# vpc-ccg/tksm

Hardware: AMD Instinct MI355X
Metric: sequenced reads/s (higher is better)
Workload: dtype u8; 1 GPU; Bulk molecules, Badread error+qual model (nanopore2020, identity 84,99,5.5), 24 x 128 Mb random genome, FASTQ; kind=bulk, mean_len=1000, length_distribution=normal(1000, 200), compute_qual=True, contexts_in_flight_per_gpu=3

## Files before the change

### tksm_amd/csrc/api.cpp

```cpp
#include "../../include/tksmseq.h"

#include <hip/hip_runtime.h>

#include <algorithm>
#include <cstdio>
#include <cstring>
#include <cstdlib>
#include <memory>
#include <string>

#include "ctx.h"
#include "loop_filter.h"

static thread_local std::string g_create_error;
void set_contextless_error(const std::string& e) { g_create_error = e; }


template <class T>
static int upload(tksmseq_ctx* ctx, DevBuf& b, const std::vector<T>& v) {
    HIPCHK(ctx, b.ensure(v.size() * sizeof(T) + 16));
    if (!v.empty()) HIPCHK(ctx, hipMemcpyAsync(b.p, v.data(), v.size() * sizeof(T), hipMemcpyHostToDevice, ctx->stream));
    HIPCHK(ctx, hipStreamSynchronize(ctx->stream));
    return TKSMSEQ_OK;
}

extern "C" {

const char* tksmseq_version(void) { return "tksm-amd seq 0.1 (gfx950)"; }

int tksmseq_create(int device, tksmseq_ctx** out) {
    if (!out) return TKSMSEQ_EINVAL;
    *out = nullptr;
    int n = 0;
    hipError_t e = hipGetDeviceCount(&n);
    if (e != hipSuccess || n <= 0) { g_create_error = "no HIP device available (this library has no CPU fallback)"; return TKSMSEQ_EDEVICE; }
    if (device < 0 || device >= n) { g_create_error = "device index out of range"; return TKSMSEQ_EINVAL; }
    e = hipSetDevice(device);
    if (e != hipSuccess) { g_create_error = hipGetErrorString(e); return TKSMSEQ_EDEVICE; }
    std::unique_ptr<tksmseq_ctx> c(new tksmseq_ctx());
    c->device = device;
    if (const char* fs = getenv("TKSMSEQ_FORCE_SLOW")) c->force_slow = fs[0] == '1';
    if (const char* tc = getenv("TKSMSEQ_TAIL_CUT")) c->tail_cut = (uint32_t)atoi(tc);
    if (const char* tc = getenv("TKSMSEQ_SMALL_ALN")) c->small_aln = (uint32_t)atoi(tc);
    if (const char* fr = getenv("TKSMSEQ_FULL_ROWS_CAP")) c->full_rows_cap = (uint32_t)std::max(0, atoi(fr));
    if (const char* tc = getenv("TKSMSEQ_WAVE_LOOP")) c->wave_loop = (uint32_t)atoi(tc);
    if (const char* tc = getenv("TKSMSEQ_TAIL_WAVE")) c->tail_wave = (uint32_t)atoi(tc);
    if (const char* tc = getenv("TKSMSEQ_TAIL_WCAP")) c->tail_wcap = atoi(tc);
    if (const char* tc = getenv("TKSMSEQ_EARLY_TAIL")) c->early_tail = (uint32_t)std::min(4096, std::max(0, atoi(tc)));
    if (const char* hl = getenv("TKSMSEQ_HBM_STATE_LEN")) c->hbm_state_len = atoi(hl);
    if (const char* dl = getenv("TKSMSEQ_DEFER_LEN")) c->defer_len = atoi(dl);
    if (const char* fp = getenv("TKSMSEQ_FULL_POOL_MB")) c->full_pool_bytes = (unsigned long long)atoll(fp) << 20;
    if (const char* nbk = getenv("TKSMSEQ_BUCKETS")) c->n_buckets = (uint32_t)std::max(1, atoi(nbk));
    hipDeviceProp_t prop;
    if (hipGetDeviceProperties(&prop, device) == hipSuccess) c->n_cus = prop.multiProcessorCount;
    e = hipStreamCreateWithFlags(&c->stream, hipStreamNonBlocking);
    if (e != hipSuccess) { g_create_error = hipGetErrorString(e); return TKSMSEQ_EDEVICE; }
    c->own_stream = true;
    for (auto& ev : c->ev) (void)hipEventCreate(&ev);
    *out = c.release();
    DevCache::get().context_created();
    return TKSMSEQ_OK;
}

int tksmseq_clone(const tksmseq_ctx* src, tksmseq_ctx** out) {
    if (!src || !out) return TKSMSEQ_EINVAL;
    int rc = tksmseq_create(src->device, out);
    if (rc != TKSMSEQ_OK) return rc;
    tksmseq_ctx* c = *out;
    c->contig_names = src->contig_names; c->contig_index = src->contig_index; c->contigs = src->contigs;
    c->total_alloc = src->total_alloc; c->total_bases = src->total_bases; c->pool_blocks = src->pool_blocks;
    c->contig_declared = src->contig_declared; c->n_declared = src->n_declared;
    c->tsb = src->tsb;
    c->d_packed.borrow(src->d_packed); c->d_blocktab.borrow(src->d_blocktab); c->d_pool.borrow(src->d_pool); c->d_contigs.borrow(src->d_contigs);
    c->em = src->em; c->qm = src->qm; c->idm = src->idm; c->em_uniform = src->em_uniform; c->em_alt0 = src->em_alt0;
    c->d_pself.borrow(src->d_pself); c->d_pseg.borrow(src->d_pseg); c->d_pt0.borrow(src->d_pt0); c->d_pt0b.borrow(src->d_pt0b); c->d_cdf32.borrow(src->d_cdf32); c->d_cdf.borrow(src->d_cdf); c->d_alts.borrow(src->d_alts); c->d_altenc.borrow(src->d_altenc);
    c->d_nalts.borrow(src->d_nalts); c->d_qkeys.borrow(src->d_qkeys); c->d_qoff.borrow(src->d_qoff); c->d_qcnt.borrow(src->d_qcnt);
    c->d_qcdf.borrow(src->d_qcdf); c->d_qq.borrow(src->d_qq); c->d_qtab.borrow(src->d_qtab); c->d_qent.borrow(src->d_qent);
    c->d_qpairs.borrow(src->d_qpairs); c->d_qguide.borrow(src->d_qguide);
    c->tail = src->tail; c->tail_version = src->tail_version; c->host_threads = src->host_threads;
    c->d_tail_lx.borrow(src->d_tail_lx); c->d_tail_ly.borrow(src->d_tail_ly); c->d_tail_cdf.borrow(src->d_tail_cdf); c->d_tail_chain.borrow(src->d_tail_chain);
    return TKSMSEQ_OK;
}

int tksmseq_host_alloc(uint64_t bytes, void** out) {
    if (!out) return TKSMSEQ_EINVAL;
    *out = nullptr;
    return hipHostMalloc(out, bytes ? bytes : 1, hipHostMallocDefault) == hipSuccess ? TKSMSEQ_OK : TKSMSEQ_ENOMEM;
}

void tksmseq_host_free(void* p) { if (p) (void)hipHostFree(p); }

int tksmseq_device_alloc(tksmseq_ctx* ctx, uint64_t bytes, void** out) {
    if (!ctx || !out) return TKSMSEQ_EINVAL;
    *out = nullptr;
    HIPCHK(ctx, hipSetDevice(ctx->device));
    HIPCHK(ctx, hipMalloc(out, bytes ? bytes : 1));
    return TKSMSEQ_OK;
}
void tksmseq_device_free(tksmseq_ctx* ctx, void* p) { if (ctx && p) { (void)hipSetDevice(ctx->device); (void)hipFree(p); } }
int tksmseq_copy_to_host(tksmseq_ctx* ctx, void* dst_host, const void* src_device, uint64_t bytes, int async) {
    if (!ctx || ((!dst_host || !src_device) && bytes)) return TKSMSEQ_EINVAL;
    HIPCHK(ctx, hipSetDevice(ctx->device));
    if (bytes) HIPCHK(ctx, hipMemcpyAsync(dst_host, src_device, bytes, hipMemcpyDeviceToHost, ctx->stream));
    if (!async) HIPCHK(ctx, hipStreamSynchronize(ctx->stream));
    return TKSMSEQ_OK;
}

void tksmseq_destroy(tksmseq_ctx* ctx) {
    if (!ctx) return;
    (void)hipSetDevice(ctx->device);
    (void)hipStreamSynchronize(ctx->stream);
    for (auto& ev : ctx->ev) if (ev) (void)hipEventDestroy(ev);
    for (auto& ev : ctx->evpool) (void)hipEventDestroy(ev);
    if (ctx->own_stream && ctx->stream) (void)hipStreamDestroy(ctx->stream);
    delete ctx;
    DevCache::get().context_destroyed();
}

const char* tksmseq_last_error(const tksmseq_ctx* ctx) { return ctx ? ctx->err.c_str() : g_create_error.c_str(); }

int tksmseq_set_stream(tksmseq_ctx* ctx, void* s) {
    if (!ctx) return TKSMSEQ_EINVAL;
    HIPCHK(ctx, hipStreamSynchronize(ctx->stream));
    if (ctx->own_stream && ctx->stream) (void)hipStreamDestroy(ctx->stream);
    if (s) { ctx->stream = (hipStream_t)s; ctx->own_stream = false; }
    else { HIPCHK(ctx, hipStreamCreateWithFlags(&ctx->stream, hipStreamNonBlocking)); ctx->own_stream = true; }
    return TKSMSEQ_OK;
}

int tksmseq_synchronize(tksmseq_ctx* ctx) {
    if (!ctx) return TKSMSEQ_EINVAL;
    HIPCHK(ctx, hipStreamSynchronize(ctx->stream));
    return TKSMSEQ_OK;
}

int tksmseq_set_host_threads(tksmseq_ctx* ctx, int n) { if (!ctx || n < 1) return TKSMSEQ_EINVAL; ctx->host_threads = std::min(n, 64); return TKSMSEQ_OK; }

int tksmseq_model_available(const char* name, const char* kind) { return (name && kind && model_available(name, kind)) ? 1 : 0; }

int tksmseq_set_timing(tksmseq_ctx* ctx, int enable) { if (!ctx) return TKSMSEQ_EINVAL; ctx->timing = enable != 0; return TKSMSEQ_OK; }

int tksmseq_reference_add_contig(tksmseq_ctx* ctx, const char* name, const uint8_t* ascii, uint64_t len, int on_device) {
    if (!ctx || !name || (!ascii && len)) return TKSMSEQ_EINVAL;
    HIPCHK(ctx, hipSetDevice(ctx->device));
    const uint64_t BLK = 1ull << tk::BLOCK_SHIFT;
    const uint64_t gstart = ctx->total_alloc;
    const uint64_t nblk = (len + BLK - 1) / BLK;
    if (gstart + nblk * BLK > (1ull << 44)) { ctx->err = "reference larger than 2^44 bases"; return TKSMSEQ_ELIMIT; }
    HIPCHK(ctx, ctx->d_packed.ensure(((gstart + nblk * BLK) >> 4) * 4 + 64, true, ctx->stream));
    HIPCHK(ctx, ctx->d_blocktab.ensure(((gstart >> tk::BLOCK_SHIFT) + nblk) * 4 + 64, true, ctx->stream));
    uint32_t* blocktab = ctx->d_blocktab.as<uint32_t>() + (gstart >> tk::BLOCK_SHIFT);
    const uint64_t CH = 64ull << 20;
    std::vector<uint32_t> flags;
    for (uint64_t off = 0; off < len; off += CH) {
        const uint64_t n = std::min(CH, len - off);
        const uint64_t cb = (n + BLK - 1) / BLK;
        const uint8_t* dsrc;
        if (on_device) dsrc = ascii + off;
        else {
            HIPCHK(ctx, ctx->d_stage.ensure(CH));
            HIPCHK(ctx, hipMemcpyAsync(ctx->d_stage.p, ascii + off, n, hipMemcpyHostToDevice, ctx->stream));
            dsrc = ctx->d_stage.as<uint8_t>();
        }
        uint32_t* bt = blocktab + (off >> tk::BLOCK_SHIFT);
        HIPCHK(ctx, hipMemsetAsync(bt, 0, cb * 4, ctx->stream));
        HIPCHK(ctx, tk::launch_pack(dsrc, n, gstart + off, ctx->d_packed.as<uint32_t>(), ctx->d_blocktab.as<uint32_t>(), ctx->stream));
        flags.resize(cb);
        HIPCHK(ctx, hipMemcpyAsync(flags.data(), bt, cb * 4, hipMemcpyDeviceToHost, ctx->stream));
        HIPCHK(ctx, hipStreamSynchronize(ctx->stream));
        uint32_t newblocks = 0;
        for (auto& f : flags) { if (f) { f = ctx->pool_blocks + newblocks; newblocks++; } else f = tk::NO_BLOCK; }
        HIPCHK(ctx, hipMemcpyAsync(bt, flags.data(), cb * 4, hipMemcpyHostToDevice, ctx->stream));
        if (newblocks) {
            HIPCHK(ctx, ctx->d_pool.ensure((uint64_t)(ctx->pool_blocks + newblocks) * BLK, true, ctx->stream));
            HIPCHK(ctx, tk::launch_fill_pool(dsrc, n, gstart + off, ctx->d_blocktab.as<uint32_t>(), ctx->d_pool.as<uint8_t>(), ctx->stream));
            ctx->pool_blocks += newblocks;
        }
        HIPCHK(ctx, hipStreamSynchronize(ctx->stream));
    }
    std::string nm(name);
    auto it = ctx->contig_index.find(nm);
    if (it == ctx->contig_index.end()) {
        ctx->contig_index[nm] = (int)ctx->contig_names.size();
        ctx->contig_names.push_back(nm);
        ctx->contigs.push_back(gstart); ctx->contigs.push_back(len);
        ctx->contig_declared.push_back(0);
    } else {
        ctx->total_bases -= ctx->contigs[2 * it->second + 1];
        ctx->contigs[2 * it->second] = gstart; ctx->contigs[2 * it->second + 1] = len;
        if (ctx->contig_declared[(size_t)it->second]) { ctx->contig_declared[(size_t)it->second] = 0; ctx->n_declared--; }
    }
    ctx->total_alloc = gstart + nblk * BLK;
    ctx->total_bases += len;
    ctx->ref_version++;
    HIPCHK(ctx, ctx->d_contigs.ensure(ctx->contigs.size() * 8 + 16));
    HIPCHK(ctx, hipMemcpyAsync(ctx->d_contigs.p, ctx->contigs.data(), ctx->contigs.size() * 8, hipMemcpyHostToDevice, ctx->stream));
    HIPCHK(ctx, hipStreamSynchronize(ctx->stream));
    return TKSMSEQ_OK;
}

int tksmseq_reference_declare_contig(tksmseq_ctx* ctx, const char* name, uint64_t len) {
    if (!ctx || !name) return TKSMSEQ_EINVAL;
    HIPCHK(ctx, hipSetDevice(ctx->device));
    if (len > (1ull << 44)) { ctx->err = "reference larger than 2^44 bases"; return TKSMSEQ_ELIMIT; }
    std::string nm(name);
    auto it = ctx->contig_index.find(nm);
    if (it == ctx->contig_index.end()) {
        ctx->contig_index[nm] = (int)ctx->contig_names.size();
        ctx->contig_names.push_back(nm);
        ctx->contigs.push_back(ctx->total_alloc); ctx->contigs.push_back(len);
        ctx->contig_declared.push_back(1);
        ctx->n_declared++;
    } else {
        ctx->total_bases -= ctx->contigs[2 * it->second + 1];
        ctx->contigs[2 * it->second + 1] = len;
        if (!ctx->contig_declared[(size_t)it->second]) { ctx->contig_declared[(size_t)it->second] = 1; ctx->n_declared++; }
    }
    ctx->total_bases += len;
    ctx->ref_version++;
    HIPCHK(ctx, ctx->d_contigs.ensure(ctx->contigs.size() * 8 + 16));
    HIPCHK(ctx, hipMemcpyAsync(ctx->d_contigs.p, ctx->contigs.data(), ctx->contigs.size() * 8, hipMemcpyHostToDevice, ctx->stream));
    HIPCHK(ctx, hipStreamSynchronize(ctx->stream));
    return TKSMSEQ_OK;
}

int tksmseq_reference_add_fasta(tksmseq_ctx* ctx, const char* path) {
    if (!ctx || !path) return TKSMSEQ_EINVAL;
    std::vector<FastaRecord> recs;
    if (!read_fasta(path, recs, ctx->err)) return TKSMSEQ_EIO;
    for (auto& r : recs) {
        int rc = tksmseq_reference_add_contig(ctx, r.name.c_str(), (const uint8_t*)r.seq.data(), r.seq.size(), 0);
        if (rc) return rc;
    }
    return TKSMSEQ_OK;
}

int tksmseq_reference_contig_id(const tksmseq_ctx* ctx, const char* name) { return (!ctx || !name) ? -1 : ctx->find(name); }

int tksmseq_reference_info(const tksmseq_ctx* ctx, uint64_t* n_contigs, uint64_t* total_bases, uint64_t* device_bytes) {
    if (!ctx) return TKSMSEQ_EINVAL;
    if (n_contigs) *n_contigs = ctx->contig_names.size();
    if (total_bases) *total_bases = ctx->total_bases;
    if (device_bytes) *device_bytes = (ctx->total_alloc >> 2) + (ctx->total_alloc >> tk::BLOCK_SHIFT) * 4 + ((uint64_t)ctx->pool_blocks << tk::BLOCK_SHIFT);
    return TKSMSEQ_OK;
}

int tksmseq_load_error_model(tksmseq_ctx* ctx, const char* name_or_path) {
    if (!ctx || !name_or_path) return TKSMSEQ_EINVAL;
    HIPCHK(ctx, hipSetDevice(ctx->device));
    ErrorModelHost m;
    if (!load_error_model(name_or_path, m, ctx->err)) return TKSMSEQ_EIO;
    ctx->em = std::move(m);
    ctx->em_alt0 = ctx->em.type == 1;
    for (size_t i = 0; i < ctx->em.nalts.size() && ctx->em_alt0; i++)
        if (ctx->em.nalts[i] && !(ctx->em.alts[i * (size_t)ctx->em.max_alts] >> 63)) ctx->em_alt0 = false;
    ctx->em_uniform = ctx->em.type == 1;
    for (uint8_t v : ctx->em.nalts) if ((int)v != ctx->em.max_alts) { ctx->em_uniform = false; break; }
    int rc;
    if ((rc = upload(ctx, ctx->d_cdf, ctx->em.cdf))) return rc;
    {
        if (ctx->em.max_alts > 32) { ctx->err = "error models with more than 32 alternatives per k-mer are not supported"; return TKSMSEQ_ELIMIT; }
        const size_t nk = ctx->em.nalts.size(), A = (size_t)ctx->em.max_alts;
        std::vector<uint32_t> c32(nk * 32, 0xFFFFFFFFu);
        for (size_t i = 0; i < nk; i++) for (size_t a = 0; a < A; a++) c32[i * 32 + a] = ctx->em.cdf[i * A + a];
        if (ctx->em.type == 0) std::fill(c32.begin(), c32.end(), 0u);
        if ((rc = upload(ctx, ctx->d_cdf32, c32))) return rc;
        std::vector<uint32_t> ps(nk * 2);
        for (size_t i = 0; i < nk; i++) { ps[2 * i] = c32[i * 32]; ps[2 * i + 1] = ctx->em.nalts[i] ? c32[i * 32 + ctx->em.nalts[i] - 1] : 0u; }
        if ((rc = upload(ctx, ctx->d_pself, ps))) return rc;
        std::vector<uint32_t> sg(nk * 4);
        for (size_t i = 0; i < nk; i++) for (int q = 0; q < 4; q++) sg[4 * i + q] = c32[i * 32 + 8 * q];
        if ((rc = upload(ctx, ctx->d_pseg, sg))) return rc;
        std::vector<uint32_t> t0(nk);
        for (size_t i = 0; i < nk; i++) t0[i] = c32[i * 32];
        if ((rc = upload(ctx, ctx->d_pt0, t0))) return rc;
        std::vector<uint16_t> t0b(tklf::LOOP_FILTER_KEYS);
        tklf::loop_filter_build(t0.data(), nk, t0b.data());
        if ((rc = upload(ctx, ctx->d_pt0b, t0b))) return rc;
    }
    if ((rc = upload(ctx, ctx->d_alts, ctx->em.alts))) return rc;
    {
        const size_t nk = ctx->em.nalts.size(), A = (size_t)ctx->em.max_alts;
        const int k = ctx->em.k;
        std::vector<uint32_t> enc(nk * A * 4, 0u);
        for (size_t i = 0; i < nk && ctx->em.type == 1; i++)
            for (size_t a = 0; a < A; a++) {
                const uint64_t alt = ctx->em.alts[i * A + a];
                uint32_t e[8] = {0, 0, 0, 0, 0, 0, 0, 0};
                int boff = 0;
                for (int j = 0; j < k; j++) {
                    const uint32_t kc = (uint32_t)(i >> (2 * (k - 1 - j))) & 3u;
                    if (alt >> 63) { e[j] = (1u << 12) | (kc & 1u) | ((kc >> 1) << 5); continue; }
                    const uint32_t len = (uint32_t)(alt >> (3 * j)) & 7u;
                    const uint32_t codes = (uint32_t)(alt >> (24 + 2 * boff)) & ((1u << (2 * len)) - 1u);
                    boff += (int)len;
                    uint32_t planar = 0;
                    for (uint32_t x = 0; x < len && x < 5; x++) planar |= (((codes >> (2 * x)) & 1u) << x) | (((codes >> (2 * x + 1)) & 1u) << (5 + x));
                    e[j] = ((len == 1 && codes == kc) ? 0u : 0x8000u) | (len << 12) | planar;
                }
                for (int q = 0; q < 4; q++) enc[(i * A + a) * 4 + q] = e[2 * q] | (e[2 * q + 1] << 16);
            }
        if ((rc = upload(ctx, ctx->d_altenc, enc))) return rc;
    }
    return upload(ctx, ctx->d_nalts, ctx->em.nalts);
}

int tksmseq_load_qscore_model(tksmseq_ctx* ctx, const char* name_or_path) {
    if (!ctx || !name_or_path) return TKSMSEQ_EINVAL;
    HIPCHK(ctx, hipSetDevice(ctx->device));
    QScoreModelHost m;
    if (!load_qscore_model(name_or_path, m, ctx->err)) return TKSMSEQ_EIO;
    ctx->qm = std::move(m);
    int rc;
    if ((rc = upload(ctx, ctx->d_qkeys, ctx->qm.keys))) return rc;
    if ((rc = upload(ctx, ctx->d_qoff, ctx->qm.row_off))) return rc;
    if ((rc = upload(ctx, ctx->d_qcnt, ctx->qm.row_cnt))) return rc;
    if ((rc = upload(ctx, ctx->d_qcdf, ctx->qm.cdf_pool))) return rc;
    if ((rc = upload(ctx, ctx->d_qq, ctx->qm.q_pool))) return rc;
    {
        const QScoreModelHost& m2 = ctx->qm;
        const size_t ns = (size_t)m2.n_slots;
        std::vector<uint32_t> ent(ns * 4, 0), pairs(m2.q_pool.size() * 2, 0);
        std::vector<uint8_t> guide(ns * 64, 0);
        bool direct = true;
        for (size_t s2 = 0; s2 < ns; s2++) if (m2.keys[s2] && m2.row_cnt[s2] > 128) direct = false;
        for (uint8_t qv : m2.q_pool) if (qv > 127) direct = false;
        for (size_t i = 0; i < m2.q_pool.size(); i++) { pairs[2 * i] = m2.cdf_pool[i]; pairs[2 * i + 1] = m2.q_pool[i]; }
        for (size_t s2 = 0; s2 < ns; s2++) {
            ent[4 * s2] = (uint32_t)m2.keys[s2]; ent[4 * s2 + 1] = (uint32_t)(m2.keys[s2] >> 32);
            ent[4 * s2 + 2] = m2.row_off[s2]; ent[4 * s2 + 3] = m2.row_cnt[s2];
            if (!m2.keys[s2]) continue;
            const uint32_t off = m2.row_off[s2], cnt = m2.row_cnt[s2];
            if (cnt > 255) { ctx->err = "q-score rows with more than 255 entries are not supported"; return TKSMSEQ_ELIMIT; }
            uint32_t a = 0;
            for (uint32_t bkt = 0; bkt < 64; bkt++) {
                const uint32_t wmin = bkt << 26, wmax = wmin | 0x3ffffffu;
                while (a + 1 < cnt && m2.cdf_pool[off + a] <= wmin) a++;
                uint32_t ah = a;
                while (ah + 1 < cnt && m2.cdf_pool[off + ah] <= wmax) ah++;
                guide[s2 * 64 + bkt] = (direct && ah == a) ? (uint8_t)(0x80u | m2.q_pool[off + a]) : (uint8_t)a;
            }
        }
        ctx->qm.guide_direct = direct;
        if ((rc = upload(ctx, ctx->d_qent, ent))) return rc;
        if ((rc = upload(ctx, ctx->d_qpairs, pairs))) return rc;
        return upload(ctx, ctx->d_qguide, guide);
    }
}

static int install_tail_model(tksmseq_ctx* ctx, TailModelHost&& m) {
    ctx->tail = std::move(m);
    ctx->tail_version++;
    if (!ctx->tail.enabled) return TKSMSEQ_OK;
    int rc;
    if ((rc = upload(ctx, ctx->d_tail_lx, ctx->tail.lx))) return rc;
    if ((rc = upload(ctx, ctx->d_tail_ly, ctx->tail.ly))) return rc;
    if ((rc = upload(ctx, ctx->d_tail_cdf, ctx->tail.cdf))) return rc;
    std::vector<tk::TailChain> ch(1);
    memcpy(ch[0].cum, ctx->tail.cum, sizeof(ch[0].cum));
    ch[0].bases = (uint32_t)ctx->tail.bases[0] | ((uint32_t)ctx->tail.bases[1] << 8) | ((uint32_t)ctx->tail.bases[2] << 16) | ((uint32_t)ctx->tail.bases[3] << 24);
    ch[0].pad = 0;
    return upload(ctx, ctx->d_tail_chain, ch);
}

int tksmseq_load_tail_model(tksmseq_ctx* ctx, const char* name_or_path) {
    if (!ctx || !name_or_path) return TKSMSEQ_EINVAL;
    HIPCHK(ctx, hipSetDevice(ctx->device));
    TailModelHost m;
    if (!load_tail_model(name_or_path, m, ctx->err)) return TKSMSEQ_EINVAL;
    return install_tail_model(ctx, std::move(m));
}

int tksmseq_set_tail_model(tksmseq_ctx* ctx, const tksmseq_tail_model* t) {
    if (!ctx) return TKSMSEQ_EINVAL;
    HIPCHK(ctx, hipSetDevice(ctx->device));
    TailModelHost m;
    if (t) {
        if (!t->lx || !t->ly || !t->grid) { ctx->err = "tail model: null table"; return TKSMSEQ_EINVAL; }
        if (!make_tail_model(t->lx, t->n_lx, t->ly, t->n_ly, t->grid, t->trans, t->ratio, t->bases, m, ctx->err)) return TKSMSEQ_EINVAL;
    }
    return install_tail_model(ctx, std::move(m));
}

int tksmseq_set_identity(tksmseq_ctx* ctx, double mean, double max, double stdev) {
    if (!ctx) return TKSMSEQ_EINVAL;
    HIPCHK(ctx, hipSetDevice(ctx->device));
    IdentityHost id;
    if (!make_identity(mean, max, stdev, id, ctx->err)) return TKSMSEQ_EINVAL;
    id.set = true;
    ctx->idm = std::move(id);
    if (!ctx->idm.constant) return upload(ctx, ctx->d_qtab, ctx->idm.qtab);
    return TKSMSEQ_OK;
}

int tksmseq_prefetch_model(const char* name_or_path, const char* kind) {
    if (!name_or_path || !kind) return TKSMSEQ_EINVAL;
    std::string err;
    if (!strcmp(kind, "error")) { ErrorModelHost m; if (load_error_model(name_or_path, m, err)) return TKSMSEQ_OK; g_create_error = err; return TKSMSEQ_EIO; }
    if (!strcmp(kind, "qscore")) { QScoreModelHost m; if (load_qscore_model(name_or_path, m, err)) return TKSMSEQ_OK; g_create_error = err; return TKSMSEQ_EIO; }
    g_create_error = std::string("unknown model kind: ") + kind;
    return TKSMSEQ_EINVAL;
}

int tksmseq_prefetch_identity(double mean, double max, double stdev) {
    IdentityHost id; std::string err;
    return make_identity(mean, max, stdev, id, err) ? TKSMSEQ_OK : TKSMSEQ_EINVAL;
}

int tksmseq_get_error_model(const tksmseq_ctx* ctx, int32_t* type, int32_t* k, int32_t* max_alts, uint32_t* cdf, uint64_t* alts, uint8_t* nalts) {
    if (!ctx || ctx->em.type < 0) return TKSMSEQ_ESTATE;
    if (type) *type = ctx->em.type;
    if (k) *k = ctx->em.k;
    if (max_alts) *max_alts = ctx->em.max_alts;
    if (cdf) memcpy(cdf, ctx->em.cdf.data(), ctx->em.cdf.size() * 4);
    if (alts) memcpy(alts, ctx->em.alts.data(), ctx->em.alts.size() * 8);
    if (nalts) memcpy(nalts, ctx->em.nalts.data(), ctx->em.nalts.size());
    return TKSMSEQ_OK;
}

int tksmseq_get_qscore_model(const tksmseq_ctx* ctx, int32_t* n_slots, int32_t* kmer_size, uint64_t* pool_len, uint64_t* keys,
                             uint32_t* row_off, uint32_t* row_cnt, uint32_t* cdf_pool, uint8_t* q_pool) {
    if (!ctx || ctx->qm.n_slots == 0) return TKSMSEQ_ESTATE;
    if (n_slots) *n_slots = ctx->qm.n_slots;
    if (kmer_size) *kmer_size = ctx->qm.kmer_size;
    if (pool_len) *pool_len = ctx->qm.q_pool.size();
    if (keys) memcpy(keys, ctx->qm.keys.data(), ctx->qm.keys.size() * 8);
    if (row_off) memcpy(row_off, ctx->qm.row_off.data(), ctx->qm.row_off.size() * 4);
    if (row_cnt) memcpy(row_cnt, ctx->qm.row_cnt.data(), ctx->qm.row_cnt.size() * 4);
    if (cdf_pool) memcpy(cdf_pool, ctx->qm.cdf_pool.data(), ctx->qm.cdf_pool.size() * 4);
    if (q_pool) memcpy(q_pool, ctx->qm.q_pool.data(), ctx->qm.q_pool.size());
    return TKSMSEQ_OK;
}

int tksmseq_get_identity(const tksmseq_ctx* ctx, int32_t* constant, double* value, double* beta_a, double* beta_b, double* qtab) {
    if (!ctx || !ctx->idm.set) return TKSMSEQ_ESTATE;
    if (constant) *constant = ctx->idm.constant ? 1 : 0;
    if (value) *value = ctx->idm.value;
    if (beta_a) *beta_a = ctx->idm.beta_a;
    if (beta_b) *beta_b = ctx->idm.beta_b;
    if (qtab && !ctx->idm.constant) memcpy(qtab, ctx->idm.qtab.data(), 65537 * sizeof(double));
    return TKSMSEQ_OK;
}

static int batch_from_host(tksmseq_ctx* ctx, const tksmseq_batch_desc* d, tksmseq_batch** out, bool check_mods = true) {
    *out = nullptr;
    HIPCHK(ctx, hipSetDevice(ctx->device));
    if (d->n_intervals >= 0x7fffffffull || d->n_mods >= 0x7fffffffull || d->n_reads >= 0xffffffffull) {
        ctx->err = "batch too large (split it: < 2^31 intervals/mods per batch)"; return TKSMSEQ_ELIMIT;
    }
    std::unique_ptr<tksmseq_batch> b(new tksmseq_batch());
    b->n_reads = d->n_reads; b->n_intervals = d->n_intervals; b->n_mods = d->n_mods; b->n_literals = d->n_literals;
    std::vector<uint32_t> ilen(d->n_intervals);
    const uint64_t nc = ctx->contig_names.size();
    uint32_t prev_mod = 0;
    for (uint64_t i = 0; i < d->n_intervals; i++) {
        const uint32_t* iv = d->intervals + 4 * i;
        uint64_t clen;
        if (iv[0] >> 31) {
            uint32_t li = iv[0] & 0x7fffffffu;
            if (li >= d->n_literals) { ctx->err = "interval refers to a literal that does not exist"; return TKSMSEQ_EINVAL; }
            clen = d->literals[2 * li + 1];
            if (d->literals[2 * li] + clen > d->literal_bytes) { ctx->err = "literal outside the literal pool"; return TKSMSEQ_EINVAL; }
        } else {
            if (iv[0] >= nc) { ctx->err = "interval refers to a contig that does not exist"; return TKSMSEQ_EINVAL; }
            clen = ctx->contigs[2 * (uint64_t)iv[0] + 1];
        }
        const uint64_t s = std::min<uint64_t>(iv[1], clen), e = std::min<uint64_t>(iv[2], clen);
        ilen[i] = e > s ? (uint32_t)(e - s) : 0;
        const uint32_t mb = iv[3] & 0x7fffffffu;
        if (mb < prev_mod || mb > d->n_mods) { ctx->err = "interval modification offsets are not monotone"; return TKSMSEQ_EINVAL; }
        prev_mod = mb;
    }
    for (uint64_t i = 0; i < d->n_intervals && check_mods; i++) {
        const uint32_t mb = d->intervals[4 * i + 3] & 0x7fffffffu;
        const uint32_t me = i + 1 < d->n_intervals ? (d->intervals[4 * (i + 1) + 3] & 0x7fffffffu) : (uint32_t)d->n_mods;
        for (uint32_t m = mb; m < me; m++)
            if (d->mods[2 * (uint64_t)m] >= ilen[i]) { ctx->err = "modification position outside its interval (the reference raises IndexError)"; return TKSMSEQ_EINVAL; }
    }
    b->raw_len.resize(d->n_reads);
    for (uint64_t r = 0; r < d->n_reads; r++) {
        const uint32_t ib = d->reads[2 * r], ic = d->reads[2 * r + 1];
        if ((uint64_t)ib + ic > d->n_intervals) { ctx->err = "read refers to intervals that do not exist"; return TKSMSEQ_EINVAL; }
        uint64_t t = 0;
        for (uint32_t i = 0; i < ic; i++) t += ilen[ib + i];
        if (t > 0x7fffff00ull) { ctx->err = "molecule longer than 2^31 bases"; return TKSMSEQ_ELIMIT; }
        b->raw_len[r] = (uint32_t)t;
        b->max_raw = std::max(b->max_raw, (uint32_t)t);
        b->total_raw += t;
        if ((uint64_t)d->ids[2 * r] + d->ids[2 * r + 1] > d->id_bytes) { ctx->err = "molecule id outside the id pool"; return TKSMSEQ_EINVAL; }
    }
    order_by_length(b->raw_len, b->order);
    auto up = [&](DevBuf& buf, const void* src, size_t bytes) -> int {
        HIPCHK(ctx, buf.ensure(bytes + 64));
        if (bytes) HIPCHK(ctx, hipMemcpyAsync(buf.p, src, bytes, hipMemcpyHostToDevice, ctx->stream));
        return TKSMSEQ_OK;
    };
    int rc;
    if ((rc = up(b->reads, d->reads, d->n_reads * 8))) return rc;
    std::vector<uint32_t> iv(d->intervals, d->intervals + 4 * d->n_intervals);
    iv.push_back(0); iv.push_back(0); iv.push_back(0); iv.push_back((uint32_t)d->n_mods);
// ... 139 lines not shown
```

### tksm_amd/csrc/ctx.h

```cpp
#pragma once
#include <hip/hip_runtime.h>
#include <chrono>

#include <algorithm>
#include <cstdlib>
#include <map>
#include <memory>
#include <mutex>
#include <string>
#include <unordered_map>
#include <vector>

#include "../../include/tksmseq.h"
#include "abund_kernels.h"
#include "host.h"
#include "kernels.h"
#include "tsb_host.h"

using namespace tkh;

#define HIPCHK(ctx, call)                                                                         \
    do {                                                                                          \
        hipError_t e_ = (call);                                                                   \
        if (e_ != hipSuccess) {                                                                   \
// ... 52 lines not shown
    void* p = nullptr;
    size_t cap = 0;
    bool owned = true;
    bool pooled = false;
    hipStream_t pool_stream = nullptr;
    int dev = -1;
    DevBuf() = default;
    DevBuf(const DevBuf&) = delete;
    DevBuf& operator=(const DevBuf&) = delete;
    DevBuf(DevBuf&& o) noexcept : p(o.p), cap(o.cap), owned(o.owned), pooled(o.pooled), pool_stream(o.pool_stream), dev(o.dev) { o.p = nullptr; o.cap = 0; }
    void release() {
        if (p && owned) {
            if (pooled) { if (pool_stream) (void)hipStreamSynchronize(pool_stream); DevCache::get().give(dev, p, cap); }
            else (void)hipFree(p);
        }
        p = nullptr; cap = 0;
    }
    ~DevBuf() { release(); }
    void borrow(const DevBuf& o) { release(); p = o.p; cap = o.cap; owned = false; }
    hipError_t ensure(size_t bytes, bool keep = false, hipStream_t s = nullptr) {
        if (bytes <= cap && owned) return hipSuccess;
        size_t ncap = std::max(bytes > (64u << 20) ? bytes + bytes / 8 : bytes, owned ? cap + cap / 2 : cap);
        ncap = (ncap + 255) & ~(size_t)255;
        void* np = nullptr;
        int ndev = dev;
        if (pooled) {
            ncap = DevCache::size_class(std::max<size_t>(bytes, 1));
            if (hipGetDevice(&ndev) != hipSuccess) ndev = -1;
            np = DevCache::get().take(ndev, ncap);
        }
        if (!np) {
            const auto t_alloc = std::chrono::steady_clock::now();
            hipError_t e = hipMalloc(&np, ncap);
            alloc_seconds() += std::chrono::duration<double>(std::chrono::steady_clock::now() - t_alloc).count();
            alloc_calls()++;
            if (e != hipSuccess) return e;
        }
        if (keep && p && cap) {
            hipError_t e = hipMemcpyAsync(np, p, std::min(cap, ncap), hipMemcpyDeviceToDevice, s);
            if (e == hipSuccess) e = hipStreamSynchronize(s);
            if (e != hipSuccess) { if (pooled) DevCache::get().give(ndev, np, ncap); else (void)hipFree(np); return e; }
        }
        const bool was_owned = owned;
        if (was_owned) release(); else { p = nullptr; cap = 0; }
        p = np; cap = ncap; owned = true; dev = ndev;
        return hipSuccess;
    }
    template <class T> T* as() const { return (T*)p; }
};

struct TmpBuf : DevBuf {
    explicit TmpBuf(hipStream_t s) { pooled = true; pool_stream = s; }
};

struct PinnedBuf {
    void* p = nullptr;
    size_t cap = 0;
    hipError_t ensure(size_t bytes) {
        if (bytes <= cap) return hipSuccess;
        release();
        const hipError_t e = hipHostMalloc(&p, bytes * 2, hipHostMallocDefault);
        if (e != hipSuccess) { p = nullptr; return e; }
        cap = bytes * 2;
        return hipSuccess;
    }
    void release() { if (p) (void)hipHostFree(p); p = nullptr; cap = 0; }
    ~PinnedBuf() { release(); }
    template <class T> T* as() const { return (T*)p; }
};

struct HelperStream {
    hipStream_t stream = nullptr;
    hipEvent_t start = nullptr, done = nullptr;
    bool used = false;
    hipError_t fork_from(hipStream_t main) {
        hipError_t e = stream ? hipSuccess : hipStreamCreateWithFlags(&stream, hipStreamNonBlocking);
        for (hipEvent_t* ev : {&start, &done}) if (e == hipSuccess && !*ev) e = hipEventCreateWithFlags(ev, hipEventDisableTiming);
        if (e == hipSuccess) e = hipEventRecord(start, main);
        if (e == hipSuccess) e = hipStreamWaitEvent(stream, start, 0);
        return e;
    }
    hipError_t launched() { const hipError_t e = hipEventRecord(done, stream); used = used || e == hipSuccess; return e; }
    hipError_t wait_done() { return hipEventSynchronize(done); }
    hipError_t join_into(hipStream_t main) { return hipStreamWaitEvent(main, done, 0); }
    bool idle() const { return !used || hipEventQuery(done) == hipSuccess; }
    hipError_t synchronize() { return stream ? hipStreamSynchronize(stream) : hipSuccess; }
    ~HelperStream() {
        if (stream) { (void)hipStreamSynchronize(stream); (void)hipStreamDestroy(stream); }
        for (hipEvent_t ev : {start, done}) if (ev) (void)hipEventDestroy(ev);
    }
};

enum RunDiag {
    DIAG_ROUNDS, DIAG_EXACT_KERNEL_READS, DIAG_PREDICTED_STRAGGLERS, DIAG_JOBS_14_ROW_ROUNDS, DIAG_JOBS_REDONE_FULL_WIDTH, DIAG_FALLBACKS,
    DIAG_FALLBACK_REASONS, DIAG_FALLBACKS_QSCORE_JOBS, DIAG_FALLBACKS_LIST_PASS, DIAG_JOBS_ALL_ROUNDS, DIAG_BAND_EXITS,
    DIAG_WORDS = 16
};

struct tksmseq_batch {
    uint64_t n_reads = 0, n_intervals = 0, n_mods = 0, n_literals = 0;
    DevBuf reads, intervals, mods, literals, litpool, ids, idpool;
    tksmseq_batch() { for (DevBuf* b : {&reads, &intervals, &mods, &literals, &litpool, &ids, &idpool, &d_dup, &d_order, &d_tail}) b->pooled = true; }
    std::vector<uint32_t> h_dup;
    DevBuf d_dup;
    std::vector<uint32_t> h_comments;
    std::vector<char> h_comment_pool;
    std::vector<uint32_t> raw_len;
    std::vector<uint32_t> order;
    DevBuf d_order;
    uint32_t max_raw = 0;
    uint64_t total_raw = 0;
    std::vector<uint32_t> splice_len;
    DevBuf d_tail;
    bool tail_on = false;
    uint64_t tail_key[4] = {};
    int cache_k = -1, cache_num = 0, cache_den = 0, cache_add = 0;
    uint64_t cache_scratch = 0;
};

struct tksmseq_ctx : ContigLookup {
    int device = 0;
    int n_cus = 256;
    hipStream_t stream = nullptr;
    static constexpr int N_SIDE = 4, SIDE_WAVES = 512;
    HelperStream side[N_SIDE];
    HelperStream early;
    uint32_t early_tail = 1024;
    DevBuf f_early;
    bool own_stream = false;
    std::string err;

    std::vector<std::string> contig_names;
    std::unordered_map<std::string, int> contig_index;
    std::vector<uint64_t> contigs;
    uint64_t total_alloc = 0;
    uint64_t total_bases = 0;
    uint32_t pool_blocks = 0;
    std::vector<uint8_t> contig_declared; uint32_t n_declared = 0;
    uint64_t ref_version = 0, wgs_version = ~0ull;
    DevBuf d_wgs_sofar, d_wgs_nameoff, d_wgs_namelen, d_wgs_names;
    DevBuf d_packed, d_blocktab, d_pool, d_contigs, d_stage;
    std::shared_ptr<const tsb::Transcripts> tsb;
    uint64_t tsb_dev_serial = 0, tsb_ref_version = ~0ull;
    DevBuf d_tsb_first, d_tsb_exons, d_tsb_lits, d_tsb_litpool;
    uint64_t tsb_n_lits = 0, tsb_lit_bytes = 0;
    float tsb_plan_ms = 0.f, tsb_write_ms = 0.f;
    uint64_t mut_serial = 0, mut_ref_version = ~0ull;
    DevBuf d_mut_refctg, d_mut_nameoff, d_mut_names, d_mut_delfirst, d_mut_ptfirst, d_mut_delfrom, d_mut_delto, d_mut_ptpos, d_mut_ptinfo, d_mut_insent, d_mut_inspool;

    ErrorModelHost em; QScoreModelHost qm; IdentityHost idm;
    bool em_uniform = false, em_alt0 = false;
    TailModelHost tail; uint64_t tail_version = 0;
    DevBuf d_tail_lx, d_tail_ly, d_tail_cdf, d_tail_chain;
    DevBuf d_pself, d_pseg, d_pt0, d_pt0b, d_cdf32, d_cdf, d_alts, d_altenc, d_nalts, d_qkeys, d_qoff, d_qcnt, d_qcdf, d_qq, d_qtab, d_qent, d_qpairs, d_qguide;

    DevBuf w_rawlen, w_slotcap, w_slotoff, w_outlen, w_ident, w_reclen, w_recoff, w_status, w_scan, w_trace, w_counter,
        w_scratch, w_records, w_istats, w_dstats, w_sums, w_fullpool, w_biglist, w_bigscratch, w_bigtrace;
    unsigned long long full_pool_bytes = 1ull << 30;
    DevBuf f_state, f_frag, f_nb, f_fplanes, f_jmeta[2], f_redo, f_jpopd, f_trace, f_tracefull, f_slow, f_defer, f_defercnt, f_frag2, f_row64;
    std::vector<uint32_t> h_row64;
    DevBuf f_round, f_geoall;
    PinnedBuf h_round, h_geo;
    bool force_slow = false;
    uint32_t tail_cut = 0;
    int tail_wcap = 2048;
    uint32_t tail_wave = 4096;
    uint32_t wave_loop = 16384;
    uint32_t full_rows_cap = 0;
    uint32_t small_aln = 131072;
    uint32_t n_buckets = 16;
    int defer_len = 0;
    int hbm_state_len = 2304;
    std::vector<hipEvent_t> evpool;
    uint32_t last_diag[DIAG_WORDS] = {};
    void* user_out = nullptr; uint64_t user_out_cap = 0;
    bool timing = false;
    int host_threads = 1;
    hipEvent_t ev[6] = {};
    tksmseq_result last{};
    bool have_last = false, have_stats = false;
    DevBuf g_counts, g_nlscan, g_sizes, g_offs, g_plans, g_out;
    tksmseq_gzip_result last_gzip{};
    bool have_gzip = false, last_fastq = false;

    int find(const std::string& name) const override {
        auto it = contig_index.find(name);
        return it == contig_index.end() ? -1 : it->second;
    }
};

template <class K, class Sort>
int sort_pairs(tksmseq_ctx* ctx, Sort sort, const K* keys, K* keys_sorted, uint32_t* perm, uint32_t n, int end_bit) {
    hipStream_t s = ctx->stream;
    TmpBuf d_iota(s), d_temp(s);
    HIPCHK(ctx, d_iota.ensure((size_t)n * 4));
    HIPCHK(ctx, tk::launch_abund_iota(d_iota.as<uint32_t>(), n, s));
    size_t bytes = 0;
    HIPCHK(ctx, sort(nullptr, &bytes, keys, keys_sorted, d_iota.as<uint32_t>(), perm, n, end_bit, s));
    HIPCHK(ctx, d_temp.ensure(bytes + 256));
    HIPCHK(ctx, sort(d_temp.p, &bytes, keys, keys_sorted, d_iota.as<uint32_t>(), perm, n, end_bit, s));
    return TKSMSEQ_OK;
}

int finalize_device_batch(tksmseq_ctx* ctx, tksmseq_batch* b);

void set_contextless_error(const std::string& e);

inline int verbose_level() { const char* v = getenv("TKSMSEQ_VERBOSE"); return v ? std::max(1, atoi(v)) : 0; }
```

### tksm_amd/csrc/host.h

```cpp
#pragma once
#include <stdint.h>

#include <algorithm>
#include <string>
#include <unordered_map>
#include <vector>

namespace tkh {

struct ErrorModelHost {
    int type = -1, k = 0, max_alts = 0;
    std::vector<uint32_t> cdf;
    std::vector<uint64_t> alts;
    std::vector<uint8_t> nalts;
};

struct QScoreModelHost {
    int n_slots = 0, kmer_size = 1;
    bool guide_direct = false;
    std::vector<uint64_t> keys;
    std::vector<uint32_t> row_off, row_cnt, cdf_pool;
    std::vector<uint8_t> q_pool;
};

struct IdentityHost {
    bool set = false, constant = true;
    double mean = 0, stdev = 0, max_identity = 0, value = 0, beta_a = 0, beta_b = 0;
    std::vector<double> qtab;
};

inline void order_by_length(const std::vector<uint32_t>& len, std::vector<uint32_t>& order) {
    const size_t n = len.size();
    order.resize(n);
    std::vector<uint32_t> tmp(n);
    std::vector<uint32_t> cnt(65537);
    auto pass = [&](int shift, const uint32_t* src, uint32_t* dst, bool first) {
        std::fill(cnt.begin(), cnt.end(), 0u);
        for (size_t i = 0; i < n; i++) cnt[((len[first ? i : src[i]] >> shift) & 0xffffu) + 1]++;
        for (size_t d = 0; d < 65536; d++) cnt[d + 1] += cnt[d];
        for (size_t i = 0; i < n; i++) { const uint32_t r = first ? (uint32_t)i : src[i]; dst[cnt[(len[r] >> shift) & 0xffffu]++] = r; }
    };
    uint32_t mx = 0;
    for (uint32_t v : len) mx = std::max(mx, v);
    if (mx < 65536u) { pass(0, nullptr, order.data(), true); return; }
    pass(0, nullptr, tmp.data(), true);
    pass(16, tmp.data(), order.data(), false);
}

struct BatchHost {
    std::vector<uint32_t> reads;
    std::vector<uint32_t> intervals;
    std::vector<uint32_t> mods;
    std::vector<uint64_t> literals;
    std::vector<uint8_t> literal_pool;
    std::vector<uint32_t> ids;
    std::vector<uint8_t> id_pool;
    std::vector<uint32_t> dup;
    std::vector<uint32_t> comments;
    std::vector<char> comment_pool;
};

struct TrcModelHost {
    std::vector<long long> xlab, ylab;
    std::vector<double> cdf;
    std::vector<int> row_n;
    bool have_sider = false;
    std::vector<double> slab, scdf;
};
bool load_trc_model(const std::string& path, TrcModelHost& m, std::string& err);

struct TailModelHost {
    bool enabled = false;
    std::vector<double> lx, ly;
    std::vector<double> cdf;
    double cum[16] = {};
    double ratio = 0.0;
    uint8_t bases[4] = {'A', 'G', 'T', 'C'};
};

bool read_text_file(const std::string& path, std::string& out, std::string& err);
std::string resolve_model(const std::string& name, const char* kind);
void cdf_thresholds(const std::vector<double>& probs, bool residual_to_one, std::vector<uint32_t>& out);
bool load_error_model(const std::string& name_or_path, ErrorModelHost& m, std::string& err);
bool load_qscore_model(const std::string& name_or_path, QScoreModelHost& m, std::string& err);
bool load_tail_model(const std::string& name_or_path, TailModelHost& m, std::string& err);
bool make_tail_model(const double* lx, size_t n_lx, const double* ly, size_t n_ly, const double* grid, const double* trans16,
                     double ratio, const uint8_t* bases4, TailModelHost& m, std::string& err);
bool make_identity(double mean, double max, double stdev, IdentityHost& id, std::string& err);

struct FastaRecord { std::string name, seq; };
bool read_fasta(const std::string& path, std::vector<FastaRecord>& out, std::string& err);

struct ContigLookup { virtual int find(const std::string& name) const = 0; virtual ~ContigLookup() {} };
bool parse_mdf(const char* text, uint64_t len, const ContigLookup& contigs, BatchHost& out, std::string& err);
bool parse_mdf_mt(const char* text, uint64_t len, const ContigLookup& contigs, BatchHost& out, std::string& err, int n_threads);
bool model_available(const std::string& name, const char* kind);

}
```

### tksm_amd/csrc/kernels.h

```cpp
#pragma once
#include <hip/hip_runtime.h>
#include <stdint.h>

namespace tk {

constexpr uint32_t NO_BLOCK = 0xFFFFFFFFu;
constexpr int BLOCK_SHIFT = 12;
constexpr int WAVES_PER_WG = 4;

struct RefView {
    const uint32_t* packed;
    const uint32_t* blocktab;
    const uint8_t* pool;
    const uint64_t* contigs;
    uint32_t n_contigs;
};

struct BatchView {
    const uint32_t* reads;
    const uint32_t* intervals;
    const uint32_t* mods;
    const uint64_t* literals;
    const uint8_t* litpool;
    const uint32_t* ids;
    const uint8_t* idpool;
    uint64_t n_reads;
    uint32_t n_literals;
};

struct ErrModelView {
    int type, k, max_alts;
    int alt0_noop;
    int uniform_nalts;
    const uint32_t* cdf;
    const uint64_t* alts;
    const uint8_t* nalts;
    const uint2* pself2;
    const uint32_t* cdf32;
    const uint4* pseg;
    const uint32_t* pt0;
    const uint4* pt0b;
    const uint4* alts_enc;
};

struct QsModelView {
    int n_slots, kmer_size;
    const uint64_t* keys;
    const uint32_t* row_off;
    const uint32_t* row_cnt;
    const uint32_t* cdf_pool;
    const uint8_t* q_pool;
    const uint4* ent;
    const uint2* pairs;
    const uint8_t* guide;
    int guide_direct;
};

struct IdentView {
    int constant;
    double value;
    const double* qtab;
};

struct TailView {
    int n_lx, n_ly;
    double ratio;
    const double* lx;
    const double* ly;
    const double* cdf;
};
struct TailChain {
    double cum[16];
    uint32_t bases;
    uint32_t pad;
};

struct SimParams {
    uint64_t seed, first_read, stride;
    int mode, compute_q, fastq, quirk_perfect;
    int lcap;
    int ncap;
    int trace_words;
    int s_lcap, s_ncap;
    int ablate;
    int cap_num, cap_den, cap_add;
};

struct SimBuffers {
    const uint32_t* raw_len;
    const uint64_t* slot_off;
    uint8_t* scratch;
    uint32_t* out_len;
    double* identity;
    uint64_t* rec_len;
    uint32_t* status;
    uint32_t* trace;
    unsigned long long* work_counter;
    int32_t* istats;
    double* dstats;
    uint8_t* full_pool; unsigned long long full_pool_bytes; unsigned long long* full_pool_used;
    const uint32_t* tail_len;
    const TailChain* tail_chain;
    uint8_t* big_scratch; size_t big_per_wave; unsigned long long* big_trace;
    const uint32_t* read_list;
    uint64_t n_work;
};

struct ReadState {
    double errors, target, est;
    int32_t change_count;
    uint32_t n_base, aln_no;
    int16_t resume_src, resume_j;
    uint8_t stage;
    uint8_t pending, slow, early;
    int32_t st_draws, st_aligns;
    uint32_t job;
    int32_t raw_len;
    uint32_t res_mt, res_cols, res_fail, pad3;
};

struct RangeGeo {
    uint64_t trace_off;
    uint64_t jc_off;
    uint64_t popd_off;
    uint64_t unused;
    uint32_t tstride;
    uint32_t cw;
    uint32_t ncap;
    uint32_t pad;
};

enum Counter {
    CNT_JOBS = 0,
    CNT_DEFERRED = 1,
    CNT_SLOW = 2,
    CNT_FULL_ROWS = 3,
    CNT_EXIT = 4,
    CNT_REDO_JOBS = 8,
    CNT_REDO_WAVES = 9,
    CNT_REDO_LIST = 10,
    CNT_FAIL = 12,
    CNT_FAIL_OR = 13,
    CNT_FAIL_LAST = 14,
    CNT_FAIL_NM = 15,
    CNT_FAIL_REASON = 16,
    CNT_FAIL_QJOB = 24,
    CNT_FAIL_LIST = 25,
    CNT_EARLY_SLOW = 26,
    CNT_EARLY = 27,
    CNT_WORDS = 32
};
enum ExitCause { EXIT_BAND_LOOP = 0, EXIT_SHIFT_LOOP = 1, EXIT_SHIFT_ERR = 2, EXIT_BAND_ERR = 3 };
enum FailBit { FAIL_QUEUE = 0, FAIL_NOROW = 1, FAIL_SHIFT31 = 3, FAIL_SHIFT14 = 4, FAIL_END_CELL = 5, FAIL_WALK = 6 };

struct FastBuffers {
    ReadState* state;
    const uint32_t* row64;
    uint8_t* st_frag;
    uint16_t* st_nb;
    unsigned long long* st_fplanes;
    uint32_t* st_frag2;
    uint32_t* job_meta;
    uint8_t* job_popd;
    void* trace;
    uint32_t* redo_list;
    void* trace_full;
    uint32_t full_rows, full_tg;
    uint32_t full_cl;
    uint32_t* counters;
    uint32_t* job_cnt;
    uint32_t rs, n_ranges;
    const uint32_t* prev_meta; const uint8_t* prev_popd;
    const uint32_t* prefix;
    const uint32_t* base_cur; const uint32_t* base_prev;
    const RangeGeo* geo_cur; const RangeGeo* geo_prev;
    uint32_t* slow_list;
    uint32_t* early_hist;
    uint2* early_list;
    uint32_t* early_slow;
    uint2* defer_list;
    uint32_t* defer_cnt;
    int defer_len;
};

hipError_t launch_pack(const uint8_t* ascii, uint64_t n, uint64_t gstart, uint32_t* packed, uint32_t* blockflag,
                       hipStream_t s);
hipError_t launch_fill_pool(const uint8_t* ascii, uint64_t n, uint64_t gstart, const uint32_t* blocktab,
                            uint8_t* pool, hipStream_t s);
hipError_t launch_read_lengths(const BatchView& b, const RefView& r, int k, int cap_num, int cap_den, int cap_add,
                               const uint32_t* tail_len, uint32_t* raw_len, uint64_t* slot_cap, uint32_t* status, hipStream_t s);
hipError_t launch_tail_lengths(const BatchView& B, const RefView& R, const TailView& T, uint64_t seed, uint64_t first_read,
                               uint64_t stride, uint32_t* tail_len, hipStream_t s);
hipError_t launch_simulate(const BatchView& b, const RefView& r, const ErrModelView& em, const QsModelView& qm,
                           const IdentView& im, const SimParams& p, const SimBuffers& o, int n_wgs,
                           int waves_per_wg, hipStream_t s);
size_t simulate_big_bytes(int lcap, int ncap);
hipError_t launch_simulate_big(const BatchView& b, const RefView& r, const ErrModelView& em, const QsModelView& qm,
                               const IdentView& im, const SimParams& p, const SimBuffers& o, int n_waves, hipStream_t s);
hipError_t launch_init(const BatchView& b, const RefView& r, const ErrModelView& em, const IdentView& im, const SimParams& p,
                       const SimBuffers& o, const FastBuffers& fb, int waves_per_wg, hipStream_t s);
int err_lds_bytes(int lcap, int ncap, int waves_per_wg, bool state_in_hbm);
int loop_lds_words(int lcap);
hipError_t launch_loopw(const ErrModelView& em, const SimParams& p, const FastBuffers& fb, const uint32_t* order, uint32_t begin,
                        uint32_t count, int lcap, int from_jobs, uint32_t c0, uint32_t c1, hipStream_t s);
hipError_t launch_tail(const ErrModelView& em, const SimParams& p, const FastBuffers& fb, const uint32_t* order, uint32_t begin,
                        uint32_t count, int lcap, int from_jobs, uint32_t c0, uint32_t c1, int wcap, hipStream_t s);
size_t tail_lds_bytes(int lcap);
hipError_t launch_mark_early(const FastBuffers& fb, const uint32_t* order, uint64_t n_reads, int k, uint32_t min_bin, hipStream_t s);
hipError_t launch_tail_early(const ErrModelView& em, const SimParams& p, const FastBuffers& fb, uint32_t max_count, int lcap, int wcap, hipStream_t s);
hipError_t launch_merge_early_slow(const FastBuffers& fb, hipStream_t s);
hipError_t launch_loop(const ErrModelView& em, const SimParams& p, const FastBuffers& fb, const uint32_t* order, uint32_t begin,
                       uint32_t count, int lcap, int from_jobs, uint32_t c0, uint32_t c1, hipStream_t s);
hipError_t launch_err(const BatchView& b, const ErrModelView& em, const QsModelView& qm, const SimParams& p, const SimBuffers& o,
                      const FastBuffers& fb, const uint32_t* order, uint32_t begin, uint32_t count, int lds_lcap, int lds_ncap,
                      int from_jobs, uint32_t c0, uint32_t c1, int waves_per_wg, bool state_in_hbm, hipStream_t s);
hipError_t launch_qjobs(const FastBuffers& fb, int k, uint32_t count, hipStream_t s);
hipError_t launch_round_reset(const FastBuffers& fb, hipStream_t s);
hipError_t launch_collect_unfinished(const FastBuffers& fb, uint64_t n_reads, hipStream_t s);
hipError_t launch_alnf(const SimParams& p, const FastBuffers& fb, const SimBuffers& o, uint32_t n_jobs, bool full_only, int mode, hipStream_t s);
hipError_t launch_perfect_lengths(const BatchView& b, const RefView& r, const SimParams& p, const SimBuffers& o, hipStream_t s);
hipError_t launch_perfect(const BatchView& b, const RefView& r, const SimParams& p, const SimBuffers& o, const uint64_t* rec_off, uint8_t* records,
                          uint32_t max_raw, int n_cus, hipStream_t s);
hipError_t launch_emit(const BatchView& b, const SimParams& p, const SimBuffers& o, const uint64_t* rec_off,
                       uint8_t* records, hipStream_t s);
hipError_t launch_interleave_lens(int n_ranks, const uint64_t* const* offsets, const uint64_t* n_per_rank,
                                  uint64_t n_total, uint64_t* lens, hipStream_t s);
hipError_t launch_interleave_copy(int n_ranks, const uint8_t* const* streams, const uint64_t* const* offsets,
                                  uint64_t n_total, const uint64_t* dst_off, uint8_t* dst, hipStream_t s);
size_t scan_temp_bytes(uint64_t n);
hipError_t launch_scan(const uint64_t* in, uint64_t* out, uint64_t n, void* temp, size_t temp_bytes, hipStream_t s);
hipError_t launch_sum_u32(const uint32_t* in, uint64_t n, unsigned long long* out, hipStream_t s);
int simulate_lds_bytes(int lcap, int ncap, int waves_per_wg);
int simulate_max_wgs(int lds_bytes);

}
```

### tksm_amd/csrc/kernels.hip

```cpp
#include "kernels.h"
#include "loop_filter.h"
#include <type_traits>

namespace tk {

#define DEV __device__ __forceinline__

constexpr int BIG = 1 << 28;
DEV bool is_inf(int v) { return v >= (1 << 27); }

struct Ph4 { uint32_t x, y, z, w; };
enum { ST_ID = 0, ST_PAD = 1, ST_IDENT = 2, ST_DRAW = 3, ST_ALNPOS = 4, ST_QUAL = 5, ST_TAIL = 6 };

DEV Ph4 philox(uint64_t seed, uint64_t read, uint32_t stream, uint32_t n) {
    uint32_t c0 = (uint32_t)read, c1 = (uint32_t)(read >> 32), c2 = stream, c3 = n;
    uint32_t k0 = (uint32_t)seed, k1 = (uint32_t)(seed >> 32);
#pragma unroll
    for (int r = 0; r < 10; r++) {
        const unsigned long long p0 = (unsigned long long)0xD2511F53u * c0, p1 = (unsigned long long)0xCD9E8D57u * c2;
        const uint32_t h0 = (uint32_t)(p0 >> 32), l0 = (uint32_t)p0, h1 = (uint32_t)(p1 >> 32), l1 = (uint32_t)p1;
        uint32_t n0 = h1 ^ c1 ^ k0, n2 = h0 ^ c3 ^ k1;
        c0 = n0; c1 = l1; c2 = n2; c3 = l0;
        k0 += 0x9E3779B9u; k1 += 0xBB67AE85u;
    }
    return Ph4{c0, c1, c2, c3};
}

DEV uint8_t base_char(int code) { return (uint8_t)((0x54474341u >> (8 * (code & 3))) & 0xff); }
DEV int code_of(uint8_t c) { return c == 'A' ? 0 : c == 'C' ? 1 : c == 'G' ? 2 : c == 'T' ? 3 : -1; }
DEV uint8_t upper(uint8_t c) { return (c >= 'a' && c <= 'z') ? (uint8_t)(c - 32) : c; }
DEV uint8_t comp(uint8_t c) {
    return c == 'A' ? 'T' : c == 'C' ? 'G' : c == 'G' ? 'C' : c == 'T' ? 'A' : c;
}

template <int CTRL, int ROW_MASK> DEV int dpp_mov(int old, int src) { return __builtin_amdgcn_update_dpp(old, src, CTRL, ROW_MASK, 0xf, false); }
constexpr int DPP_WAVE_SHL1 = 0x130, DPP_WAVE_SHR1 = 0x138;
#define TKSM_DPP_SCAN(OP, IDENT, x)                         \
    x = OP(x, dpp_mov<0x111, 0xf>(IDENT, x));               \
    x = OP(x, dpp_mov<0x112, 0xf>(IDENT, x));               \
    x = OP(x, dpp_mov<0x114, 0xf>(IDENT, x));               \
    x = OP(x, dpp_mov<0x118, 0xf>(IDENT, x));               \
    x = OP(x, dpp_mov<0x142, 0xa>(IDENT, x));               \
    x = OP(x, dpp_mov<0x143, 0xc>(IDENT, x));
DEV int scan_min_incl(int x, int) { TKSM_DPP_SCAN(min, 0x7fffffff, x) return x; }
DEV int scan_max_incl(int x, int) { TKSM_DPP_SCAN(max, (int)0x80000000, x) return x; }
DEV int add_i32(int a, int b) { return a + b; }
DEV int scan_add_incl(int x, int) { TKSM_DPP_SCAN(add_i32, 0, x) return x; }
DEV uint32_t scan_umax_incl(uint32_t x) {
#define TKSM_UMAX_STEP(C, R) x = max(x, (uint32_t)dpp_mov<C, R>(0, (int)x));
    TKSM_UMAX_STEP(0x111, 0xf) TKSM_UMAX_STEP(0x112, 0xf) TKSM_UMAX_STEP(0x114, 0xf) TKSM_UMAX_STEP(0x118, 0xf) TKSM_UMAX_STEP(0x142, 0xa) TKSM_UMAX_STEP(0x143, 0xc)
#undef TKSM_UMAX_STEP
    return x;
}
DEV int prefix_small(int v, int& total) {
    const unsigned long long b0 = __ballot(v & 1), b1 = __ballot(v & 2), b2 = __ballot(v & 4);
    const int e0 = (int)__builtin_amdgcn_mbcnt_hi((uint32_t)(b0 >> 32), __builtin_amdgcn_mbcnt_lo((uint32_t)b0, 0u));
    const int e1 = (int)__builtin_amdgcn_mbcnt_hi((uint32_t)(b1 >> 32), __builtin_amdgcn_mbcnt_lo((uint32_t)b1, 0u));
    const int e2 = (int)__builtin_amdgcn_mbcnt_hi((uint32_t)(b2 >> 32), __builtin_amdgcn_mbcnt_lo((uint32_t)b2, 0u));
    total = __popcll(b0) + 2 * __popcll(b1) + 4 * __popcll(b2);
    return e0 + 2 * e1 + 4 * e2;
}

DEV void wave_sync() {
    __builtin_amdgcn_fence(__ATOMIC_RELEASE, "wavefront");
    __builtin_amdgcn_wave_barrier();
    __builtin_amdgcn_fence(__ATOMIC_ACQUIRE, "wavefront");
}

DEV uint32_t lo32(unsigned long long v) { return (uint32_t)v; }
DEV uint32_t hi32(unsigned long long v) { return (uint32_t)(v >> 32); }
DEV unsigned long long mk64(uint32_t hi, uint32_t lo) { return ((unsigned long long)hi << 32) | lo; }
DEV uint32_t alignbit(uint32_t hi, uint32_t lo, uint32_t s) { return __builtin_amdgcn_alignbit(hi, lo, s); }
constexpr uint32_t TA = 0xF0u, TB = 0xCCu, TC = 0xAAu;
#define BOOL3(expr) ((uint32_t)((expr) & 0xFFu))
template <uint32_t TT> DEV uint32_t bool3(uint32_t x, uint32_t y, uint32_t z) { return __builtin_amdgcn_bitop3_b32(x, y, z, TT); }
template <uint32_t TT> DEV unsigned long long bool3(unsigned long long x, unsigned long long y, unsigned long long z) {
    return mk64(bool3<TT>(hi32(x), hi32(y), hi32(z)), bool3<TT>(lo32(x), lo32(y), lo32(z)));
}
DEV unsigned long long funnel128(unsigned long long x0, unsigned long long x1, int s) {
    const bool a = (s & 32) != 0;
    const uint32_t b = (uint32_t)s & 31u;
    const uint32_t y0 = a ? hi32(x0) : lo32(x0), y1 = a ? lo32(x1) : hi32(x0), y2 = a ? hi32(x1) : lo32(x1);
    return mk64(alignbit(y2, y1, b), alignbit(y1, y0, b));
}

DEV double sqrt_inrange(double x) {
    const double y = __builtin_amdgcn_rsq(x);
    double g = x * y, h = 0.5 * y;
    const double r = __builtin_fma(-h, g, 0.5);
    g = __builtin_fma(g, r, g); h = __builtin_fma(h, r, h);
    double d = __builtin_fma(-g, g, x);
    g = __builtin_fma(d, h, g);
    d = __builtin_fma(-g, g, x);
    return __builtin_fma(d, h, g);
}
DEV double rcp_refined(double b) {
    double y = __builtin_amdgcn_rcp(b);
    double r = __builtin_fma(-b, y, 1.0);
    y = __builtin_fma(y, r, y);
    r = __builtin_fma(-b, y, 1.0);
    return __builtin_fma(y, r, y);
}
DEV double div_inrange(double a, double b, double yb) {
    const double q = a * yb;
    const double r = __builtin_fma(-b, q, a);
    return __builtin_fma(r, yb, q);
}

DEV uint8_t ref_base(const RefView& R, uint64_t g) {
    uint32_t ex = R.blocktab[g >> BLOCK_SHIFT];
    if (ex != NO_BLOCK) return R.pool[((uint64_t)ex << BLOCK_SHIFT) + (g & ((1u << BLOCK_SHIFT) - 1))];
    uint32_t w = R.packed[g >> 4];
    return base_char((int)(w >> ((g & 15) * 2)));
}

DEV int slot_len(uint32_t code) { return code ? (int)((code >> 12) & 7) : 1; }
DEV uint8_t slot_sym(uint32_t code, int x, uint8_t orig) {
    if (!code) return orig;
    if ((int)((code >> 10) & 3) == x + 1) return orig;
    return base_char((int)(code >> (2 * x)));
}

__global__ void k_pack(const uint8_t* __restrict__ ascii, uint64_t n, uint64_t gstart, uint32_t* __restrict__ packed,
                       uint32_t* __restrict__ blockflag) {
    uint64_t w = (uint64_t)blockIdx.x * blockDim.x + threadIdx.x;
    uint64_t nw = (n + 15) >> 4;
    for (; w < nw; w += (uint64_t)gridDim.x * blockDim.x) {
        uint64_t b0 = w << 4;
        uint32_t word = 0; bool exc = false;
        if (b0 + 16 <= n && ((uintptr_t)(ascii + b0) & 15) == 0) {
            uint4 v = *reinterpret_cast<const uint4*>(ascii + b0);
            uint32_t q[4] = {v.x, v.y, v.z, v.w};
#pragma unroll
            for (int i = 0; i < 16; i++) {
                int c = code_of(upper((uint8_t)(q[i >> 2] >> (8 * (i & 3)))));
                exc |= c < 0; word |= (uint32_t)(c & 3) << (2 * i);
            }
        } else {
            for (int i = 0; i < 16 && b0 + i < n; i++) {
                int c = code_of(upper(ascii[b0 + i]));
                exc |= c < 0; word |= (uint32_t)(c & 3) << (2 * i);
            }
        }
        packed[(gstart >> 4) + w] = word;
        if (exc) blockflag[(gstart + b0) >> BLOCK_SHIFT] = 1;
    }
}

__global__ void k_fill_pool(const uint8_t* __restrict__ ascii, uint64_t n, uint64_t gstart,
                            const uint32_t* __restrict__ blocktab, uint8_t* __restrict__ pool) {
    uint64_t i = (uint64_t)blockIdx.x * blockDim.x + threadIdx.x;
    for (; i < n; i += (uint64_t)gridDim.x * blockDim.x) {
        uint64_t g = gstart + i;
        uint32_t ex = blocktab[g >> BLOCK_SHIFT];
// ... 1348 lines not shown
            const Ph4 d = philox(P.seed, g, ST_DRAW, nl);
            const int di = (int)__umulhi(d.x, kmer_range);
            const int w = di >> 4, o = di & 15;
            const int kidx = (int)((uint32_t)(mk64(f2[w], f2[w + 1]) >> (64 - 2 * o - 2 * k)) & kmask);
            const uint4 seg = EM.pseg[kidx];
            const int na = EM.uniform_nalts ? EM.max_alts : (int)EM.nalts[kidx];
            int cls = EM.type == 0 ? 2 : (d.y < seg.x ? (EM.alt0_noop ? 0 : 3) : 1);
            const int sbase = 8 * ((d.y < seg.y ? 0 : 1) + (d.y < seg.z ? 0 : 1) + (d.y < seg.w ? 0 : 1));
            const uint4* c4 = reinterpret_cast<const uint4*>(EM.cdf32 + (cls == 1 ? (size_t)kidx * 32 + sbase : (size_t)0));
            const uint4 th0 = c4[0], th1 = c4[1];
            size_t at = 0;
            if (cls == 1 || cls == 3) {
                int a = 0;
                if (cls == 1) {
                    const uint32_t wv = d.y;
                    a = sbase;
                    a += !(wv < th0.x) ? 1 : 0; a += !(wv < th0.y) ? 1 : 0; a += !(wv < th0.z) ? 1 : 0; a += !(wv < th0.w) ? 1 : 0;
                    a += !(wv < th1.x) ? 1 : 0; a += !(wv < th1.y) ? 1 : 0; a += !(wv < th1.z) ? 1 : 0; a += !(wv < th1.w) ? 1 : 0;
                    a = min(a, na);
                }
                if (a == na) cls = 2;
                else if (a == 0 && EM.alt0_noop) cls = 0;
                else at = (size_t)kidx * EM.max_alts + a;
            }
            uint4 A = EM.alts_enc[at];
            if (cls == 2) {
                const uint32_t type = __umulhi(d.z, 3u), pos = __umulhi(d.w, (uint32_t)k);
                const uint32_t base4 = d.w & 3u, side = (d.w >> 2) & 1u;
                const uint32_t r3 = (((d.z & 0xffffu) * 3u) >> 16) + 1u;
                const uint32_t kc = ((uint32_t)kidx >> (2 * (k - 1 - (int)pos))) & 3u;
                const uint32_t v = type == 0 ? 0x8000u | (1u << 12) | planar1((kc + r3) & 3u)
                                 : type == 1 ? 0x8000u | (2u << 12) | (side ? planar2(kc, base4) : planar2(base4, kc))
                                             : 0x8000u;
                const uint32_t wv = v << (16 * (pos & 1u)), which = pos >> 1;
                A = make_uint4(which == 0 ? wv : 0u, which == 1 ? wv : 0u, which == 2 ? wv : 0u, which == 3 ? wv : 0u);
            }
            uint32_t dm = ((A.x >> 15) & 1u) | ((A.x >> 31) << 1) | (((A.y >> 15) & 1u) << 2) | ((A.y >> 31) << 3) |
                          (((A.z >> 15) & 1u) << 4) | ((A.z >> 31) << 5) | (((A.w >> 15) & 1u) << 6) | ((A.w >> 31) << 7);
            dm &= (1u << k) - 1u;
            if (!live || cls == 0) dm = 0u;
            unsigned long long mask = __ballot(dm != 0u);
            const unsigned long long dead = __ballot(!live);
            while (mask) {
                const int src = __builtin_ctzll(mask);
                mask &= mask - 1ull;
                const int ai = __builtin_amdgcn_readlane(di, src);
                uint4 As;
                As.x = (uint32_t)__builtin_amdgcn_readlane((int)A.x, src); As.y = (uint32_t)__builtin_amdgcn_readlane((int)A.y, src);
                As.z = (uint32_t)__builtin_amdgcn_readlane((int)A.z, src); As.w = (uint32_t)__builtin_amdgcn_readlane((int)A.w, src);
                uint32_t dms = (uint32_t)__builtin_amdgcn_readlane((int)dm, src);
                double est = est_cur;
                if (resume_j > 0) { dms &= ~((1u << resume_j) - 1u); est = est_keep; }
                const double f15 = est * sqrt_inrange(est);
                int stop_at = -1;
                while (dms) {
                    const int jj = __builtin_ctz(dms);
                    dms &= dms - 1u;
                    const int ps = ai + jj;
                    if (TAIL ? ((bml[ps >> 5] >> (ps & 31)) & 1u) == 0u : (nbl[ps] & 0x8000u) == 0) {
                        const uint32_t e = draw_slot(As, jj);
                        if (lane == 0) {
                            if (TAIL) bml[ps >> 5] |= 1u << (ps & 31); else nbl[ps] = (uint16_t)(e | 0x8000u);
                            gnb[ps] = (uint16_t)(e | 0x8000u);
                        }
                        change_count++;
                        const int len_j = (int)((e >> 12) & 7u);
                        errors += (double)(len_j < 2 ? 1 : len_j - 1) * f15;
                        if (++cc25 == 25) { cc25 = 0; stop_at = jj; break; }
                    }
                }
                wave_sync();
                if (stop_at >= 0) {
                    st = NEED_ALN;
                    if (stop_at + 1 < k) { resume_j = stop_at + 1; est_keep = est; n += (uint32_t)src; }
                    else { resume_j = 0; n += (uint32_t)src + 1u; }
                    break;
                }
                resume_j = 0;
                est_cur = 1.0 - div_inrange(errors, frag_len, rcp_len);
                if ((double)change_count > 0.9 * frag_len || est_cur <= target) { st = DONE; st_draws = (int)n + src + 1; break; }
            }
            if (st != RUN) break;
            resume_j = 0;
            if (dead) { st = DONE; st_draws = (int)loop_limit; break; }
            n += 64u;
        }
        if (!TAIL || st != NEED_ALN) break;
        {
            int p0 = 0, nrows = L;
            if (L > 1000) {
                p0 = (int)__umulhi(philox(P.seed, g, ST_ALNPOS, aln_no).x, (uint32_t)(L - 1000 + 1));
                nrows = 1000;
                wave_sync();
                for (int t = lane; t < nrows; t += 64) Fw[t] = gfrag[p0 + t];
            }
            wave_sync();
            const int m = join_window_planar(gnb, p0, nrows, Nw, ownw, wcap, lane);
            wave_sync();
            if (m > wcap) {
                if (early_mode) { to_exact_kernel(); return; }
                break;
            }
            const AlnOut a = band_align<0, false>(Fw, nrows, Nw, ownw, m, lane, nullptr);
            st_aligns++;
            if (is_inf(a.dist)) {
                to_exact_kernel();
                return;
            }
            const int cols = (int)(a.stat & 0xffffu), mt = (int)(a.stat >> 16);
            const double ident = cols ? (double)mt / (double)cols : 0.0;
            if (L <= 1000) errors = (1.0 - ident) * frag_len;
            else {
                const double estimated = (1.0 - ident) * frag_len;
                const double weight = 1000.0 / frag_len;
                errors = estimated * weight + errors * (1.0 - weight);
            }
            aln_no++;
            st = RUN;
        }
    }
    if (lane == 0) {
        uint32_t job = 0;
        if (st == NEED_ALN) {
            job = FB.base_cur[rc] + atomicAdd(&FB.job_cnt[rc * 32u], 1u);
            st_aligns++;
            uint32_t p0 = 0, nrows = (uint32_t)L;
            if (L > 1000) {
                p0 = __umulhi(philox(P.seed, g, ST_ALNPOS, aln_no).x, (uint32_t)(L - 1000 + 1));
                nrows = 1000u;
            }
            *reinterpret_cast<uint4*>(FB.job_meta + 4ull * job) = make_uint4(r, p0, nrows, 0u);
        }
        sp->errors = errors; sp->est = est_keep; sp->change_count = change_count; sp->n_base = n; sp->aln_no = aln_no;
        sp->resume_src = -1; sp->resume_j = (int16_t)resume_j; sp->st_draws = st_draws; sp->st_aligns = st_aligns;
        sp->pending = st == NEED_ALN ? 1 : 0;
        sp->job = job;
        sp->stage = st == NEED_ALN ? 0 : 3;
        if (st == DONE) {
            atomicAdd(&FB.defer_cnt[rc * 32u], 1u);
            FB.defer_list[atomicAdd(&FB.counters[CNT_DEFERRED], 1u)] = make_uint2(r, rc);
        }
    }
}

template <bool STATE_IN_HBM>
__global__ __launch_bounds__(256, 8) void k_err(BatchView B, ErrModelView EM, QsModelView QM, SimParams P, SimBuffers O,
                                              FastBuffers FB, const uint32_t* __restrict__ order, uint32_t begin, uint32_t count,
                                              int lds_lcap, int lds_ncap, int from_jobs, uint32_t c0, uint32_t c1) {
#ifndef TKSM_ABLATE
    __builtin_amdgcn_s_setprio(2);
#endif
    const int lane = threadIdx.x & 63, wave = __builtin_amdgcn_readfirstlane(threadIdx.x >> 6), wpw = blockDim.x >> 6;
    const uint32_t widx = blockIdx.x * (uint32_t)wpw + (uint32_t)wave;
    if (widx >= count) return;
    uint64_t r; uint32_t pos;
    if (!from_jobs) { pos = begin + widx; r = (uint64_t)__builtin_amdgcn_readfirstlane((int)order[pos]) & 0xffffffffull; }
    else if (from_jobs == 2) {
        const uint2 e = FB.defer_list[widx];
        r = (uint64_t)__builtin_amdgcn_readfirstlane((int)e.x) & 0xffffffffull;
        pos = (uint32_t)__builtin_amdgcn_readfirstlane((int)e.y) * FB.rs;
    } else {
        const uint32_t target = FB.prefix[c0] + widx;
        uint32_t lo2 = c0, hi2 = c1 - 1;
        while (lo2 < hi2) { const uint32_t mid = (lo2 + hi2 + 1) >> 1; if (FB.prefix[mid] <= target) lo2 = mid; else hi2 = mid - 1; }
        const uint32_t pjob = FB.base_prev[lo2] + (target - FB.prefix[lo2]);
        r = (uint64_t)__builtin_amdgcn_readfirstlane((int)FB.prev_meta[4ull * pjob]) & 0xffffffffull;
        pos = lo2 * FB.rs;
    }
    ReadState S = FB.state[r];
    if (S.stage == 2 || S.slow) return;
    if (S.stage == 0) return;
    uint16_t* gnb = nb_row(FB, r);
    const int per_wave = STATE_IN_HBM ? lds_ncap + 128 : lds_lcap * 3 + lds_ncap + 128;
    uint8_t* lds_wave = lds_raw + (size_t)wave * per_wave;
    uint8_t* frag = STATE_IN_HBM ? frag_row(FB, r) : lds_wave;
    uint16_t* nb = STATE_IN_HBM ? gnb : reinterpret_cast<uint16_t*>(lds_wave + lds_lcap);
    uint8_t* aux = STATE_IN_HBM ? lds_wave : lds_wave + 3 * (size_t)lds_lcap;
    const int k = EM.k;
    const uint64_t g = P.first_read + r * P.stride;
    const int raw_len = __builtin_amdgcn_readfirstlane(S.raw_len);
    const int L = raw_len + 2 * k;
    const uint64_t slot = O.slot_off[r];
    const int cap = __builtin_amdgcn_readfirstlane((int)((O.slot_off[r + 1] - slot) >> 1));
    uint8_t* out_seq = O.scratch + slot;
    uint8_t* out_qual = out_seq + cap;
    if (!STATE_IN_HBM) {
        const uint8_t* gfrag0 = frag_row(FB, r);
        for (int t = lane * 4; t < L; t += 256) *reinterpret_cast<uint32_t*>(frag + t) = *reinterpret_cast<const uint32_t*>(gfrag0 + t);
        for (int t = lane * 2; t < L; t += 128) *reinterpret_cast<uint32_t*>(nb + t) = *reinterpret_cast<const uint32_t*>(gnb + t);
    }
    wave_sync();
    uint32_t status = 0;
    const double frag_len = (double)L;
    const double errors = S.errors;
    const double target = S.target;
    const int change_count = __builtin_amdgcn_readfirstlane(S.change_count), st_draws = __builtin_amdgcn_readfirstlane(S.st_draws);
    int st_aligns = __builtin_amdgcn_readfirstlane(S.st_aligns);
    double identity = 1.0;

    int start_trim, end_trim;
    {
        int v1 = lane < k ? slot_len(nb[lane]) : 0, v2 = lane < k ? slot_len(nb[L - k + lane]) : 0;
        (void)prefix_small(v1, start_trim);
        (void)prefix_small(v2, end_trim);
    }
    const int jcap = min(lds_ncap, cap);
    const int m = joined_len(nb, 0, L, lane);
    int lo = start_trim, hi = end_trim == 0 ? 0 : m - end_trim;
    lo = min(lo, m); hi = max(hi, lo);
    if (m > jcap) { status |= 1; lo = hi = 0; }
    const int out_len = hi - lo;
    const bool want_q = P.compute_q && m > 0 && !(status & 1);
    if (want_q) {
        const uint32_t mt = S.res_mt, cols = S.res_cols, fail = S.res_fail;
        if (fail) { go_slow(FB, r, lane, EXIT_BAND_ERR); return; }
        identity = cols ? (double)mt / (double)cols : 0.0;
        const uint32_t rc1 = pos / FB.rs;
        const uint8_t* gp = FB.prev_popd + FB.geo_prev[rc1].popd_off + (size_t)(S.job - FB.base_prev[rc1]) * FB.geo_prev[rc1].ncap;
        wave_sync();
        uint8_t* popd = aux + 16;
        for (int t = lane; t < m; t += 64) popd[t] = gp[t];
        wave_sync();
        const int margins = (QM.kmer_size - 1) / 2;
        const uint32_t hmask = (uint32_t)QM.n_slots - 1u;
        for (int i2 = lo + lane; i2 < hi; i2 += 64) {
#ifdef TKSM_ABLATE
            if (P.ablate == 40) { out_qual[i2 - lo] = 40; continue; }
#endif
            const int d = max(0, max(margins - i2, i2 + margins - (m - 1)));
            int row = -1; uint32_t roff = 0, rcnt = 0;
            auto probe = [&](uint64_t key) {
                uint32_t sl = (uint32_t)qs_hash(key) & hmask;
#ifdef TKSM_ABLATE
                if (P.ablate == 41) { row = (int)(sl & 1023u); roff = 0u; rcnt = 1u; return; }
#endif
                for (;;) {
                    const uint4 e = QM.ent[sl];
                    const uint64_t kk = ((uint64_t)e.y << 32) | e.x;
                    if (kk == key) { row = (int)sl; roff = e.z; rcnt = e.w; break; }
                    if (kk == 0) break;
                    sl = (sl + 1) & hmask;
                }
            };
            if (margins <= 4) {
                const int ob = 16 + i2 - 4, sh = ob & 3;
                const uint32_t* aw = reinterpret_cast<const uint32_t*>(aux) + (ob >> 2);
                const uint32_t w0 = aw[0], w1 = aw[1], w2 = aw[2];
                const uint32_t b0 = __builtin_amdgcn_alignbyte(w1, w0, sh), b1 = __builtin_amdgcn_alignbyte(w2, w1, sh), b2 = w2 >> (8 * sh);
                auto byte_at = [&](int j) -> uint32_t { return j < 4 ? (b0 >> (8 * j)) & 255u : j < 8 ? (b1 >> (8 * (j - 4))) & 255u : b2 & 255u; };
                uint64_t K[5]; int ln[5];
                K[0] = byte_at(4) & 3u; ln[0] = 1;
#pragma unroll
                for (int h = 1; h <= 4; h++) {
                    const uint32_t bl = byte_at(4 - h);
                    const int ddl = (int)(bl >> 2), ddr = (int)(byte_at(3 + h) >> 2);
                    ln[h] = ln[h - 1] + 2 + ddl + ddr;
                    const bool fits = ln[h] <= 29;
                    const int sl_ = fits ? 2 * (1 + ddl) : 0, sr_ = fits ? 2 * (1 + ddl + ln[h - 1]) : 0, so_ = fits ? 2 * (ln[h] - 1) : 0;
                    const int dl2 = fits ? 2 * ddl : 0, dr2 = fits ? 2 * ddr : 0;
                    K[h] = (uint64_t)(bl & 3u) | (((1ull << dl2) - 1ull) << 2) | (K[h - 1] << sl_) | (((1ull << dr2) - 1ull) << sr_) |
                           ((uint64_t)(byte_at(4 + h) & 3u) << so_);
                }
                const int hmax = margins - d;
                bool pend = true;
#pragma unroll
                for (int h = 4; h >= 0; h--) {
                    const bool tryit = pend && h <= hmax;
                    if (__ballot(tryit) == 0ull) continue;
                    if (tryit && ln[h] <= 29) { probe(K[h] | ((uint64_t)ln[h] << 58)); pend = row < 0; }
#ifdef TKSM_ABLATE
                    if (P.ablate == 44) { if (row < 0) row = (int)(K[h] & 1023u); pend = false; }
                    if (P.ablate == 45 && h == 3) { if (row < 0) row = (int)(K[h] & 1023u); pend = false; }
#endif
                }
            } else {
                int s0 = i2 - margins + d, e0 = i2 + margins - d;
                for (;;) {
                    uint64_t key = 0; int len = 0; bool ok = true;
                    for (int x2 = s0; x2 <= e0; x2++) {
                        if (x2 > s0) {
                            const int dd = popd[x2 - 1] >> 2;
                            if (len + dd > 29) { ok = false; break; }
                            key |= ((1ull << (2 * dd)) - 1ull) << (2 * len); len += dd;
                        }
                        if (len >= 29) { ok = false; break; }
                        key |= (uint64_t)(popd[x2] & 3) << (2 * len); len++;
                    }
                    if (ok) probe(key | ((uint64_t)len << 58));
                    if (row >= 0 || s0 == e0) break;
                    s0++; e0--;
                }
            }
            uint8_t q = 0;
#ifdef TKSM_ABLATE
            if (P.ablate == 42) { out_qual[i2 - lo] = (uint8_t)(33 + (row & 31)); continue; }
            if (P.ablate == 43 && row >= 0) {
                const uint32_t w = (uint32_t)i2 * 2654435761u;
                const uint32_t a2 = QM.guide[(size_t)row * 64 + (w >> 26)] & 0x7fu;
                out_qual[i2 - lo] = (uint8_t)(33 + QM.pairs[roff + min(a2, rcnt - 1u)].y); continue;
            }
#endif
            if (row >= 0) {
                const uint32_t w = philox(P.seed, g, ST_QUAL, (uint32_t)i2).x;
                uint32_t a2 = QM.guide[(size_t)row * 64 + (w >> 26)];
                if (QM.guide_direct && (a2 & 0x80u)) q = (uint8_t)(a2 & 0x7fu);
                else {
                    uint2 pr = QM.pairs[roff + a2];
                    while (a2 + 1 < rcnt && !(w < pr.x)) { a2++; pr = QM.pairs[roff + a2]; }
                    q = (uint8_t)pr.y;
                }
            }
            out_qual[i2 - lo] = (uint8_t)(q + 33);
        }
    } else {
        identity = 1.0 - errors / frag_len;
    }
    join_out(frag, nb, L, out_seq, lo, hi, lane);
    if (P.quirk_perfect) identity = 1.0;
    finish_read(B, P, O, r, P.quirk_perfect ? out_len : raw_len, out_len, identity, status, st_draws, change_count, st_aligns, L, m,
                start_trim, end_trim, errors, target, lane);
    if (lane == 0) FB.state[r].stage = 2;
}

__global__ void k_collect_unfinished(FastBuffers FB, uint64_t n_reads) {
    const uint64_t r = (uint64_t)blockIdx.x * blockDim.x + threadIdx.x;
    if (r >= n_reads) return;
    ReadState S = FB.state[r];
    if (S.stage != 2 && !S.slow) {
        FB.state[r].slow = 1;
        const uint32_t idx = atomicAdd(&FB.counters[CNT_SLOW], 1u);
        FB.slow_list[idx] = (uint32_t)r;
    }
}

DEV uint32_t range_of_job(const FastBuffers& FB, uint32_t job0) {
    uint32_t rng = 0, hi2 = FB.n_ranges - 1;
    while (rng < hi2) { const uint32_t mid = (rng + hi2 + 1) >> 1; if (FB.base_cur[mid] <= job0) rng = mid; else hi2 = mid - 1; }
    return rng;
}
__global__ __launch_bounds__(64) void k_qjobs(FastBuffers FB, int k, uint32_t count) {
    const int lane = threadIdx.x;
    const uint32_t widx = blockIdx.x * 64u + (uint32_t)lane;
    bool need = widx < count;
    uint32_t r = 0, rc = 0, job = 0;
    if (need) { const uint2 e = FB.defer_list[widx]; r = e.x; rc = e.y; }
    need = need && FB.state[r].stage == 3 && !FB.state[r].slow;
    const bool mine = need;
    unsigned long long todo = __ballot(need);
    while (todo) {
        const int leader = __builtin_ctzll(todo);
        const uint32_t lrc = (uint32_t)__shfl((int)rc, leader, 64);
        const unsigned long long grp = __ballot(need && rc == lrc);
        uint32_t base = 0;
        if (lane == leader) base = FB.base_cur[lrc] + atomicAdd(&FB.job_cnt[lrc * 32u], (uint32_t)__popcll(grp));
        base = (uint32_t)__shfl((int)base, leader, 64);
        if (need && rc == lrc) { job = base + (uint32_t)__popcll(grp & ((1ull << lane) - 1ull)); need = false; }
        todo &= ~grp;
    }
    if (mine) {
        ReadState* sp = FB.state + r;
        const uint32_t L = (uint32_t)(sp->raw_len + 2 * k);
        *reinterpret_cast<uint4*>(FB.job_meta + 4ull * job) = make_uint4(r, 0u, L | 0x80000000u, 0u);
        sp->resume_src = -1; sp->pending = 1; sp->stage = 1; sp->job = job;
    }
}

DEV int wave_max(int v) {
#pragma unroll
    for (int o = 32; o > 0; o >>= 1) v = max(v, __shfl_xor(v, o, 64));
    return v;
}
DEV void list_append(uint32_t* list, uint32_t* counter, bool want, uint32_t job, int lane) {
    const unsigned long long wm = __ballot(want);
    if (!wm) return;
    uint32_t base = 0;
    if (lane == 0) base = atomicAdd(counter, (uint32_t)__popcll(wm));
    base = __shfl(base, 0, 64);
    if (want) list[base + (uint32_t)__popcll(wm & ((1ull << lane) - 1ull))] = job;
}


constexpr uint32_t ENT_EMPTY = 0xF0000000u;
constexpr int BACKLOG_DRAIN = 20;
struct AlnJobF {
    bool act; int p0, n;
    const uint16_t* nb;
    const ulonglong2* fp; int wlast;
    unsigned long long* popd8;
};
struct AlnResF { uint32_t mt, cols; int m; bool fail, needfull, overflow; uint32_t why; };

template <int MODE, int ROWS>
DEV AlnResF aln_fused(const AlnJobF& J, uint4* trl, int tg, int cl, uint32_t ls, int mcap) {
    static_assert(ROWS == 14 || ROWS == 64, "14 stored rows, or all of them");
    constexpr int NC = ROWS == 14 ? 16 : 4;
    constexpr int ST = ROWS == 14 ? 24 : 0;
    constexpr int RAMP0 = 31 - ST;
    const bool act = J.act;
    const int n = act ? J.n : 0;
    const int base = J.p0 & ~1, skip = J.p0 - base;
    const int nmax = __builtin_amdgcn_readfirstlane(wave_max(act ? n + skip : 0));
    tg = __builtin_amdgcn_readfirstlane(tg); cl = __builtin_amdgcn_readfirstlane(cl);
    const int wb = base >> 6, bsh = base & 63;
    auto fpw = [&](int w) { return J.fp[min(max(w, 0), J.wlast)]; };
    auto aligned = [&](const ulonglong2& a, const ulonglong2& b) { ulonglong2 v; v.x = funnel128(a.x, b.x, bsh); v.y = funnel128(a.y, b.y, bsh); return v; };
    ulonglong2 Wn;
    unsigned long long A, B;
    {
        const ulonglong2 r0 = fpw(wb), r1 = fpw(wb + 1), r2 = fpw(wb + 2);
        const ulonglong2 W0 = aligned(r0, r1);
        Wn = aligned(r1, r2);
        A = ~funnel128(W0.x, Wn.x, skip); B = ~funnel128(W0.y, Wn.y, skip);
    }
    int jc = 0;
    unsigned long long EA = 0ull, EB = 0ull;
    int app = 0;
    unsigned long long Pv = ~0ull, Mv = 0ull;
    int t = 1, t32 = 1;
    uint32_t qlo = 0u, qhi = 0u;
    unsigned long long U = 0ull;
    int npend = 0, upos = 0, pcol = -1 - skip, col = 0, col32 = 0, shmax = 0;
    bool bad = false;
    struct __attribute__((packed, aligned(4))) U4b { uint32_t x, y, z, w; };
    uint32_t cw[8], cwn[8];
    auto load_codes = [&](int s, uint32_t (&d)[8]) {
        const int src = (s <= n + skip) ? base + s : base;
        const U4b* cp = reinterpret_cast<const U4b*>(J.nb + src);
        const U4b c0 = cp[0], c1 = cp[1];
        d[0] = c0.x; d[1] = c0.y; d[2] = c0.z; d[3] = c0.w; d[4] = c1.x; d[5] = c1.y; d[6] = c1.z; d[7] = c1.w;
    };
    load_codes(0, cw);
    constexpr int HS = 16;
    constexpr int LPH = HS / NC;
    uint32_t tw[16], shw[4] = {0u, 0u, 0u, 0u};
    int ql = 0;
    bool ovf = false;
    int s0 = 0;
    for (;;) {
        const bool more = s0 < nmax;
        const bool drain = __ballot(npend > (more ? BACKLOG_DRAIN : 0)) != 0ull;
        if (!more && !drain) break;
        if (ql + LPH > (ROWS == 64 ? cl : tg - 1)) { ovf = true; break; }
        if (!drain) load_codes(s0 + HS, cwn);
        const int inc = drain ? 0 : 1;
        uint4* const dl = trl + (size_t)(act ? ql : tg - 1) * ls;
        const int it0 = __builtin_amdgcn_readfirstlane(ql * NC);
        int mxn = 0, mxu = 0;
#pragma unroll
        for (int q = 0; q < HS; q++) {
            const int p = s0 + q - skip;
            const bool on = !drain && act && (uint32_t)p < (uint32_t)n;
            const uint32_t code = (cw[q >> 1] >> (16 * (q & 1))) & 0xffffu;
            const int len = on ? (int)((code >> 12) & 7u) : 0;
            const uint32_t m5 = (1u << len) - 1u;
            const uint32_t lo5 = code & m5, hi5 = (code >> 5) & m5;
            mxn = max(mxn, npend); mxu = max(mxu, upos);
            qlo |= lo5 << npend; qhi |= hi5 << npend;
            U |= (unsigned long long)(m5 << 1) << upos;
            upos += len + inc; npend += len;
            const uint32_t zz = U ? (uint32_t)__builtin_ctzll(U) : 64u;
            const int zc = (int)min(zz, (uint32_t)upos);
            pcol += zc;
            const bool have = npend > 0;
            const int used = zc + (have ? 1 : 0);
            U >>= used; upos -= used;
            uint32_t ent0 = ENT_EMPTY, ent1 = 0u, ent2 = 0u, ent3 = 0u, shb = 0xffu;
            if (have) {
                const int tn = max(1, pcol - 30);
// ... 573 lines not shown
                if (mp < e.len) bimg[e.o + ((e.flags & 2u) ? e.len - 1 - mp : mp)] = (e.flags & 2u) ? comp((uint8_t)mc) : (uint8_t)mc;
            }
        }
        if (lane == 0) {
            bimg[L] = '\n';
            if (P.fastq) { bimg[L + 1] = '+'; bimg[L + 2] = '\n'; bimg[L + 3 + L] = '\n'; }
        }
        if (P.fastq) {
            uint8_t* kq = bimg + L + 3;
            const uint32_t head = (uint32_t)((16 - (reinterpret_cast<uintptr_t>(kq) & 15)) & 15);
            for (uint32_t t = lane; t < min(head, L); t += 64) kq[t] = 'K';
            if (L > head) {
                const uint32_t body = (L - head) & ~15u;
                for (uint32_t t = 16u * lane; t < body; t += 1024u)
                    *reinterpret_cast<uint4*>(kq + head + t) = make_uint4(0x4b4b4b4bu, 0x4b4b4b4bu, 0x4b4b4b4bu, 0x4b4b4b4bu);
                for (uint32_t t = head + body + lane; t < L; t += 64) kq[t] = 'K';
            }
        }
        wave_sync();
        flush_image(img, a, (uint32_t)rec_len, records + off - a, lane);
    }
}

struct PtrPack { const void* p[16]; uint64_t n[16]; };

__global__ void k_interleave_lens(int P_, PtrPack offs, uint64_t n_total, uint64_t* __restrict__ lens) {
    uint64_t gi = (uint64_t)blockIdx.x * blockDim.x + threadIdx.x;
    if (gi >= n_total) return;
    const int p = (int)(gi % P_); const uint64_t i = gi / P_;
    const uint64_t* o = (const uint64_t*)offs.p[p];
    lens[gi] = o[i + 1] - o[i];
}

__global__ __launch_bounds__(256) void k_interleave_copy(int P_, PtrPack streams, PtrPack offs, uint64_t n_total,
                                                          const uint64_t* __restrict__ dst_off, uint8_t* __restrict__ dst) {
    const int lane = threadIdx.x & 63, wave = threadIdx.x >> 6;
    const uint64_t gi = (uint64_t)blockIdx.x * WAVES_PER_WG + wave;
    if (gi >= n_total) return;
    const int p = (int)(gi % P_); const uint64_t i = gi / P_;
    const uint64_t* o = (const uint64_t*)offs.p[p];
    const uint8_t* s = (const uint8_t*)streams.p[p] + o[i];
    const uint64_t len = o[i + 1] - o[i];
    uint8_t* d = dst + dst_off[gi];
    struct __attribute__((packed, aligned(1))) U16 { uint32_t x, y, z, w; };
    const uint64_t body = len & ~15ull;
    for (uint64_t t = 16ull * lane; t < body; t += 1024) *reinterpret_cast<U16*>(d + t) = *reinterpret_cast<const U16*>(s + t);
    if (body + lane < len) d[body + lane] = s[body + lane];
}

constexpr int SCAN_T = 256, SCAN_V = 8, SCAN_B = SCAN_T * SCAN_V;

__global__ __launch_bounds__(SCAN_T) void k_scan_sums(const uint64_t* __restrict__ in, uint64_t n, uint64_t* __restrict__ sums) {
    __shared__ uint64_t sh[SCAN_T];
    const uint64_t base = (uint64_t)blockIdx.x * SCAN_B + (uint64_t)threadIdx.x * SCAN_V;
    uint64_t a = 0;
    for (int i = 0; i < SCAN_V; i++) if (base + i < n) a += in[base + i];
    sh[threadIdx.x] = a;
    __syncthreads();
    for (int o = SCAN_T / 2; o > 0; o >>= 1) { if ((int)threadIdx.x < o) sh[threadIdx.x] += sh[threadIdx.x + o]; __syncthreads(); }
    if (threadIdx.x == 0) sums[blockIdx.x] = sh[0];
}

__global__ __launch_bounds__(SCAN_T) void k_scan_apply(const uint64_t* __restrict__ in, uint64_t n, const uint64_t* __restrict__ block_off,
                                                        uint64_t* __restrict__ out) {
    __shared__ uint64_t sh[SCAN_T];
    const uint64_t base = (uint64_t)blockIdx.x * SCAN_B + (uint64_t)threadIdx.x * SCAN_V;
    uint64_t v[SCAN_V], a = 0;
    for (int i = 0; i < SCAN_V; i++) { v[i] = base + i < n ? in[base + i] : 0; a += v[i]; }
    sh[threadIdx.x] = a;
    __syncthreads();
    for (int o = 1; o < SCAN_T; o <<= 1) {
        uint64_t y = (int)threadIdx.x >= o ? sh[threadIdx.x - o] : 0;
        __syncthreads();
        sh[threadIdx.x] += y;
        __syncthreads();
    }
    uint64_t run = (block_off ? block_off[blockIdx.x] : 0) + sh[threadIdx.x] - a;
    for (int i = 0; i < SCAN_V; i++) { if (base + i < n) out[base + i] = run; run += v[i]; }
    if (base <= n - 1 && n - 1 < base + SCAN_V) out[n] = run;
}

__global__ void k_set_u64(uint64_t* p, uint64_t v) { *p = v; }

__global__ void k_sum_u32(const uint32_t* __restrict__ in, uint64_t n, unsigned long long* out) {
    uint64_t i = (uint64_t)blockIdx.x * blockDim.x + threadIdx.x;
    unsigned long long a = 0;
    for (; i < n; i += (uint64_t)gridDim.x * blockDim.x) a += in[i];
    for (int o = 32; o > 0; o >>= 1) a += __shfl_down((long long)a, o, 64);
    if ((threadIdx.x & 63) == 0 && a) atomicAdd(out, a);
}

static inline unsigned grid_for(uint64_t n, unsigned threads, unsigned cap = 256 * 16) {
    uint64_t b = (n + threads - 1) / threads;
    if (b < 1) b = 1;
    return (unsigned)(b > cap ? cap : b);
}

hipError_t launch_pack(const uint8_t* ascii, uint64_t n, uint64_t gstart, uint32_t* packed, uint32_t* blockflag, hipStream_t s) {
    if (!n) return hipSuccess;
    hipLaunchKernelGGL(k_pack, dim3(grid_for((n + 15) >> 4, 256)), dim3(256), 0, s, ascii, n, gstart, packed, blockflag);
    return hipGetLastError();
}
hipError_t launch_fill_pool(const uint8_t* ascii, uint64_t n, uint64_t gstart, const uint32_t* blocktab, uint8_t* pool, hipStream_t s) {
    if (!n) return hipSuccess;
    hipLaunchKernelGGL(k_fill_pool, dim3(grid_for(n, 256)), dim3(256), 0, s, ascii, n, gstart, blocktab, pool);
    return hipGetLastError();
}
hipError_t launch_read_lengths(const BatchView& b, const RefView& r, int k, int cap_num, int cap_den, int cap_add,
                               const uint32_t* tail_len, uint32_t* raw_len, uint64_t* slot_cap, uint32_t* status, hipStream_t s) {
    if (!b.n_reads) return hipSuccess;
    hipLaunchKernelGGL(k_read_lengths, dim3((unsigned)((b.n_reads + 255) / 256)), dim3(256), 0, s, b, r, k, cap_num, cap_den,
                       cap_add, tail_len, raw_len, slot_cap, status);
    return hipGetLastError();
}
hipError_t launch_tail_lengths(const BatchView& b, const RefView& r, const TailView& t, uint64_t seed, uint64_t first_read,
                               uint64_t stride, uint32_t* tail_len, hipStream_t s) {
    if (!b.n_reads) return hipSuccess;
    hipLaunchKernelGGL(k_tail_lengths, dim3((unsigned)((b.n_reads + 255) / 256)), dim3(256), 0, s, b, r, t, seed, first_read, stride,
                       tail_len);
    return hipGetLastError();
}
int simulate_lds_bytes(int lcap, int ncap, int wpw) { return wpw * (lcap * 3 + ncap * 4); }
int simulate_max_wgs(int lds_bytes) {
    int per_cu = lds_bytes > 0 ? (160 * 1024) / lds_bytes : 8;
    if (per_cu > 8) per_cu = 8;
    if (per_cu < 1) per_cu = 1;
    return per_cu;
}
hipError_t launch_simulate(const BatchView& b, const RefView& r, const ErrModelView& em, const QsModelView& qm,
                           const IdentView& im, const SimParams& p, const SimBuffers& o, int n_wgs, int wpw, hipStream_t s) {
    if (!b.n_reads) return hipSuccess;
    const int lds = simulate_lds_bytes(p.s_lcap, p.s_ncap, wpw);
    hipError_t e = hipFuncSetAttribute(reinterpret_cast<const void*>(k_simulate<false>), hipFuncAttributeMaxDynamicSharedMemorySize, lds);
    if (e != hipSuccess) return e;
    hipLaunchKernelGGL(k_simulate<false>, dim3(n_wgs), dim3(64 * wpw), lds, s, b, r, em, qm, im, p, o);
    return hipGetLastError();
}
size_t simulate_big_bytes(int lcap, int ncap) { return ((size_t)lcap * 3 + (size_t)ncap * 6 + 255) & ~(size_t)255; }
hipError_t launch_simulate_big(const BatchView& b, const RefView& r, const ErrModelView& em, const QsModelView& qm,
                               const IdentView& im, const SimParams& p, const SimBuffers& o, int n_waves, hipStream_t s) {
    if (!b.n_reads || !n_waves) return hipSuccess;
    hipLaunchKernelGGL(k_simulate<true>, dim3(n_waves), dim3(64), 0, s, b, r, em, qm, im, p, o);
    return hipGetLastError();
}
hipError_t launch_init(const BatchView& b, const RefView& r, const ErrModelView& em, const IdentView& im, const SimParams& p,
                       const SimBuffers& o, const FastBuffers& fb, int wpw, hipStream_t s) {
    if (!b.n_reads) return hipSuccess;
    const int lds = wpw * p.lcap;
    hipError_t e = hipFuncSetAttribute(reinterpret_cast<const void*>(k_init), hipFuncAttributeMaxDynamicSharedMemorySize, lds);
    if (e != hipSuccess) return e;
    hipLaunchKernelGGL(k_init, dim3((unsigned)((b.n_reads + wpw - 1) / wpw)), dim3(64 * wpw), lds, s, b, r, em, im, p, o, fb);
    return hipGetLastError();
}
int err_lds_bytes(int lcap, int ncap, int wpw, bool state_in_hbm) { return wpw * ((state_in_hbm ? 0 : lcap * 3) + ncap + 128); }
hipError_t launch_err(const BatchView& b, const ErrModelView& em, const QsModelView& qm, const SimParams& p, const SimBuffers& o,
                      const FastBuffers& fb, const uint32_t* order, uint32_t begin, uint32_t count, int lds_lcap, int lds_ncap,
                      int from_jobs, uint32_t c0, uint32_t c1, int wpw, bool state_in_hbm, hipStream_t s) {
    if (!count) return hipSuccess;
    const int lds = err_lds_bytes(lds_lcap, lds_ncap, wpw, state_in_hbm);
    auto kern = state_in_hbm ? k_err<true> : k_err<false>;
    hipError_t e = hipFuncSetAttribute(reinterpret_cast<const void*>(kern), hipFuncAttributeMaxDynamicSharedMemorySize, 160 * 1024);
    if (e != hipSuccess) return e;
    hipLaunchKernelGGL(kern, dim3((count + wpw - 1) / wpw), dim3(64 * wpw), lds, s, b, em, qm, p, o, fb, order, begin, count, lds_lcap,
                       lds_ncap, from_jobs, c0, c1);
    return hipGetLastError();
}
constexpr int LOOP_WL_MAX = 64;
int loop_lds_words(int lcap) {
    static const int wl_max = [] { const char* e = getenv("TKSMSEQ_LOOP_WL"); return e ? std::max(4, atoi(e) & ~3) : LOOP_WL_MAX; }();
    return std::min(wl_max, (((lcap + 15) / 16 + 1) + 3) & ~3);
}
hipError_t launch_loop(const ErrModelView& em, const SimParams& p, const FastBuffers& fb, const uint32_t* order, uint32_t begin,
                       uint32_t count, int lcap, int from_jobs, uint32_t c0, uint32_t c1, hipStream_t s) {
    if (!count) return hipSuccess;
    const int Wl = loop_lds_words(lcap);
    hipLaunchKernelGGL(k_loop, dim3((count + 63) / 64), dim3(64), (size_t)Wl * 256 + tklf::LOOP_FILTER_BYTES, s, em, p, fb, order, begin, count, Wl, from_jobs, c0, c1);
    return hipGetLastError();
}
hipError_t launch_loopw(const ErrModelView& em, const SimParams& p, const FastBuffers& fb, const uint32_t* order, uint32_t begin,
                        uint32_t count, int lcap, int from_jobs, uint32_t c0, uint32_t c1, hipStream_t s) {
    if (!count) return hipSuccess;
    hipLaunchKernelGGL(k_loopw<false>, dim3(count), dim3(64), (size_t)lcap * 2 + 16, s, em, p, fb, order, begin, count, from_jobs, c0, c1, lcap, 0);
    return hipGetLastError();
}
size_t tail_lds_bytes(int lcap) { return tail_bitmap_bytes(lcap) + TAIL_FCAP + TAIL_WCAP * 3; }
__global__ void k_mark_early(FastBuffers FB, const uint32_t* __restrict__ order, uint64_t n_reads, int k, uint32_t min_bin) {
    const uint64_t pos = (uint64_t)blockIdx.x * blockDim.x + threadIdx.x;
    if (pos >= n_reads) return;
    const uint32_t r = order[pos];
    ReadState* sp = FB.state + r;
    if (sp->stage != 0 || sp->slow) return;
    if (early_bin(sp->raw_len + 2 * k, sp->target) < min_bin) return;
    sp->early = 1;
    FB.early_list[atomicAdd(&FB.counters[CNT_EARLY], 1u)] = make_uint2(r, (uint32_t)(pos / FB.rs));
}
__global__ void k_merge_early_slow(FastBuffers FB) {
    const uint32_t n = FB.counters[CNT_EARLY_SLOW];
    for (uint32_t i = threadIdx.x; i < n; i += blockDim.x) FB.slow_list[FB.counters[CNT_SLOW] + i] = FB.early_slow[i];
    __syncthreads();
    if (threadIdx.x == 0) { FB.counters[CNT_SLOW] += n; FB.counters[CNT_EXIT + EXIT_BAND_LOOP] += n; FB.counters[CNT_EARLY_SLOW] = 0u; }
}
hipError_t launch_mark_early(const FastBuffers& fb, const uint32_t* order, uint64_t n_reads, int k, uint32_t min_bin, hipStream_t s) {
    hipLaunchKernelGGL(k_mark_early, dim3((unsigned)((n_reads + 255) / 256)), dim3(256), 0, s, fb, order, n_reads, k, min_bin);
    return hipGetLastError();
}
hipError_t launch_tail_early(const ErrModelView& em, const SimParams& p, const FastBuffers& fb, uint32_t max_count, int lcap, int wcap, hipStream_t s) {
    if (!max_count) return hipSuccess;
    hipLaunchKernelGGL(k_loopw<true>, dim3(max_count), dim3(64), tail_lds_bytes(lcap), s, em, p, fb, nullptr, 0u, max_count, 3, 0u, 0u, lcap, std::min(std::max(wcap, 1), TAIL_WCAP));
    return hipGetLastError();
}
hipError_t launch_merge_early_slow(const FastBuffers& fb, hipStream_t s) {
    hipLaunchKernelGGL(k_merge_early_slow, dim3(1), dim3(256), 0, s, fb);
    return hipGetLastError();
}
hipError_t launch_tail(const ErrModelView& em, const SimParams& p, const FastBuffers& fb, const uint32_t* order, uint32_t begin,
                       uint32_t count, int lcap, int from_jobs, uint32_t c0, uint32_t c1, int wcap, hipStream_t s) {
    if (!count) return hipSuccess;
    hipLaunchKernelGGL(k_loopw<true>, dim3(count), dim3(64), tail_lds_bytes(lcap), s, em, p, fb, order, begin, count, from_jobs, c0, c1, lcap, std::min(std::max(wcap, 1), TAIL_WCAP));
    return hipGetLastError();
}
hipError_t launch_qjobs(const FastBuffers& fb, int k, uint32_t count, hipStream_t s) {
    if (!count) return hipSuccess;
    hipLaunchKernelGGL(k_qjobs, dim3((count + 63) / 64), dim3(64), 0, s, fb, k, count);
    return hipGetLastError();
}
__global__ void k_round_reset(uint32_t* __restrict__ job_cnt, uint32_t n_words, uint32_t* __restrict__ counters) {
    const uint32_t i = blockIdx.x * blockDim.x + threadIdx.x;
    if (i < n_words) job_cnt[i] = 0u;
    if (i == 0) { counters[CNT_FULL_ROWS] = 0u; counters[CNT_REDO_LIST] = 0u; }
}
hipError_t launch_round_reset(const FastBuffers& fb, hipStream_t s) {
    const uint32_t n_words = fb.n_ranges * 32u;
    hipLaunchKernelGGL(k_round_reset, dim3((n_words + 255) / 256), dim3(256), 0, s, fb.job_cnt, n_words, fb.counters);
    return hipGetLastError();
}
hipError_t launch_collect_unfinished(const FastBuffers& fb, uint64_t n_reads, hipStream_t s) {
    if (!n_reads) return hipSuccess;
    hipLaunchKernelGGL(k_collect_unfinished, dim3((unsigned)((n_reads + 255) / 256)), dim3(256), 0, s, fb, n_reads);
    return hipGetLastError();
}
hipError_t launch_alnf(const SimParams& p, const FastBuffers& fb, const SimBuffers& o, uint32_t n_jobs, bool full_only, int mode, hipStream_t s) {
    if (!n_jobs) return hipSuccess;
    const uint32_t waves = (n_jobs + 63) / 64;
    if (full_only) {
        if (mode) hipLaunchKernelGGL((k_alnf<1, 64, false>), dim3(waves), dim3(64), 0, s, p, fb, o, n_jobs);
        else hipLaunchKernelGGL((k_alnf<0, 64, false>), dim3(waves), dim3(64), 0, s, p, fb, o, n_jobs);
        return hipGetLastError();
    }
    const uint32_t g2 = std::max<uint32_t>(1u, std::min<uint32_t>((waves + 7) / 8, std::max<uint32_t>(1u, fb.full_rows / 64)));
    if (mode) {
        hipLaunchKernelGGL((k_alnf<1, 14, false>), dim3(waves), dim3(64), 0, s, p, fb, o, n_jobs);
        hipLaunchKernelGGL((k_alnf<1, 64, true>), dim3(g2), dim3(64), 0, s, p, fb, o, n_jobs);
    } else {
        hipLaunchKernelGGL((k_alnf<0, 14, false>), dim3(waves), dim3(64), 0, s, p, fb, o, n_jobs);
        hipLaunchKernelGGL((k_alnf<0, 64, true>), dim3(g2), dim3(64), 0, s, p, fb, o, n_jobs);
    }
    return hipGetLastError();
}
hipError_t launch_emit(const BatchView& b, const SimParams& p, const SimBuffers& o, const uint64_t* rec_off, uint8_t* records, hipStream_t s) {
    if (!b.n_reads) return hipSuccess;
    hipLaunchKernelGGL(k_emit, dim3((unsigned)((b.n_reads + WAVES_PER_WG - 1) / WAVES_PER_WG)), dim3(256), 0, s, b, p, o, rec_off, records);
    return hipGetLastError();
}
hipError_t launch_perfect_lengths(const BatchView& b, const RefView& r, const SimParams& p, const SimBuffers& o, hipStream_t s) {
    if (!b.n_reads) return hipSuccess;
    hipLaunchKernelGGL(k_perfect_lengths, dim3((unsigned)((b.n_reads + 255) / 256)), dim3(256), 0, s, b, r, p, o);
    return hipGetLastError();
}
hipError_t launch_perfect(const BatchView& b, const RefView& r, const SimParams& p, const SimBuffers& o, const uint64_t* rec_off, uint8_t* records,
                          uint32_t max_raw, int n_cus, hipStream_t s) {
    if (!b.n_reads) return hipSuccess;
    hipError_t e = hipFuncSetAttribute(reinterpret_cast<const void*>(k_perfect), hipFuncAttributeMaxDynamicSharedMemorySize, 160 * 1024);
    if (e != hipSuccess) return e;
    const uint64_t need = ((p.fastq ? 2ull : 1ull) * max_raw + 512 + 255) & ~255ull;
    const int img[2] = {(int)std::min<uint64_t>(PERFECT_IMG_MAX, need), (int)std::min<uint64_t>(PERFECT_IMG_LONG, need)};
    const int n_launch = need > (uint64_t)PERFECT_IMG_MAX ? 2 : 1;
    for (int k = 0; k < n_launch; k++) {
        const int lds = perfect_lds_bytes(img[k]);
        int wgs_per_cu = 0;
        e = hipOccupancyMaxActiveBlocksPerMultiprocessor(&wgs_per_cu, reinterpret_cast<const void*>(k_perfect), 64 * WAVES_PER_WG, (size_t)lds);
        if (e != hipSuccess) return e;
        wgs_per_cu = std::max(1, wgs_per_cu);
        const uint64_t want = (b.n_reads + WAVES_PER_WG - 1) / WAVES_PER_WG;
        hipLaunchKernelGGL(k_perfect, dim3((unsigned)std::min<uint64_t>(want, (uint64_t)n_cus * wgs_per_cu)), dim3(64 * WAVES_PER_WG), lds, s, b, r, p, o,
                           rec_off, records, img[k], k ? img[0] : 0, k == n_launch - 1 ? 1 : 0);
        if ((e = hipGetLastError()) != hipSuccess) return e;
    }
    return hipSuccess;
}
hipError_t launch_interleave_lens(int n_ranks, const uint64_t* const* offsets, const uint64_t* n_per_rank, uint64_t n_total,
                                  uint64_t* lens, hipStream_t s) {
    if (!n_total) return hipSuccess;
    PtrPack o{};
    for (int i = 0; i < n_ranks; i++) { o.p[i] = offsets[i]; o.n[i] = n_per_rank[i]; }
    hipLaunchKernelGGL(k_interleave_lens, dim3((unsigned)((n_total + 255) / 256)), dim3(256), 0, s, n_ranks, o, n_total, lens);
    return hipGetLastError();
}
hipError_t launch_interleave_copy(int n_ranks, const uint8_t* const* streams, const uint64_t* const* offsets, uint64_t n_total,
                                  const uint64_t* dst_off, uint8_t* dst, hipStream_t s) {
    if (!n_total) return hipSuccess;
    PtrPack st{}, o{};
    for (int i = 0; i < n_ranks; i++) { st.p[i] = streams[i]; o.p[i] = offsets[i]; }
    hipLaunchKernelGGL(k_interleave_copy, dim3((unsigned)((n_total + WAVES_PER_WG - 1) / WAVES_PER_WG)), dim3(256), 0, s, n_ranks,
                       st, o, n_total, dst_off, dst);
    return hipGetLastError();
}

size_t scan_temp_bytes(uint64_t n) {
    size_t total = 0;
    while (n > 1) { uint64_t nb = (n + SCAN_B - 1) / SCAN_B; total += (nb + 1) * sizeof(uint64_t) * 2; n = nb; if (nb == 1) break; }
    return total + 64;
}
hipError_t launch_scan(const uint64_t* in, uint64_t* out, uint64_t n, void* temp, size_t temp_bytes, hipStream_t s) {
    if (n == 0) { hipLaunchKernelGGL(k_set_u64, dim3(1), dim3(1), 0, s, out, 0ull); return hipGetLastError(); }
    const uint64_t nb = (n + SCAN_B - 1) / SCAN_B;
    if (nb == 1) {
// ... 22 lines not shown
```

### tksm_amd/csrc/models.cpp

```cpp
#include "host.h"

#include <zlib.h>
#include <dlfcn.h>
#include <sys/stat.h>

#include <cmath>
#include <cstdlib>
#include <cstring>
#include <cstdio>
#include <map>
#include <memory>
#include <mutex>

namespace tkh {

static bool file_exists(const std::string& p) { struct stat st; return stat(p.c_str(), &st) == 0 && S_ISREG(st.st_mode); }

bool read_text_file(const std::string& path, std::string& out, std::string& err) {
    gzFile f = gzopen(path.c_str(), "rb");
    if (!f) { err = "cannot open " + path; return false; }
    gzbuffer(f, 1 << 20);
    out.clear();
    std::vector<char> buf(1 << 22);
    for (;;) {
// ... 46 lines not shown
            int d = at(i - 1, j - 1) + (q[i - 1] != t[j - 1]), u = at(i - 1, j) + 1, l = at(i, j - 1) + 1;
            at(i, j) = std::min(d, std::min(u, l));
        }
    }
    std::string ops;
    int i = n, j = m;
    while (i > 0 || j > 0) {
        int cur = at(i, j);
        if (i > 0 && at(i - 1, j) + 1 == cur) { ops.push_back('I'); i--; }
        else if (j > 0 && at(i, j - 1) + 1 == cur) { ops.push_back('D'); j--; }
        else { ops.push_back(at(i - 1, j - 1) == cur ? '=' : 'X'); i--; j--; }
    }
    return std::string(ops.rbegin(), ops.rend());
}

static bool align_kmers(const std::string& kmer_in, const std::string& alt_in, std::vector<std::string>& result) {
    if (kmer_in.size() <= 2 || alt_in.size() <= 1) return false;
    if (kmer_in.front() != alt_in.front() || kmer_in.back() != alt_in.back()) return false;
    const size_t k = kmer_in.size();
    result.assign(k, std::string());
    result[0] = std::string(1, kmer_in.front());
    result[k - 1] = std::string(1, kmer_in.back());
    std::vector<bool> set(k, false);
    std::string kmer = kmer_in.substr(1, k - 2), alt = alt_in.substr(1, alt_in.size() - 2);
    std::string ops = alt.empty() ? std::string(kmer.size(), 'D') : nw_ops(alt, kmer);
    size_t kp = 0, ap = 0;
    for (char c : ops) {
        if (c == '=' || c == 'X') { result[kp + 1] = std::string(1, alt[ap]); ap++; kp++; }
        else if (c == 'D') { result[kp + 1] = ""; kp++; }
        else { result[kp] += alt[ap]; ap++; }
    }
    if (result[0].size() == 2) {
        std::string ins(1, result[0][1]);
        result[0] = result[0].substr(0, 1);
        result[1] = ins + result[1];
    }
    return true;
}

static int base_code(char c) { return c == 'A' ? 0 : c == 'C' ? 1 : c == 'G' ? 2 : c == 'T' ? 3 : -1; }

void cdf_thresholds(const std::vector<double>& probs, bool residual_to_one, std::vector<uint32_t>& out) {
    double s = 0.0;
    for (double p : probs) s += p;
    const double total = (residual_to_one && s < 1.0) ? 1.0 : s;
    double cum = 0.0;
    for (double p : probs) {
        cum += p;
        double x = cum / total * 4294967296.0;
        out.push_back(x >= 4294967295.0 ? 0xFFFFFFFFu : (uint32_t)x);
    }
}

static void split(const std::string& s, char sep, std::vector<std::string>& out) {
    out.clear();
    size_t a = 0;
    for (;;) { size_t b = s.find(sep, a); if (b == std::string::npos) { out.push_back(s.substr(a)); break; } out.push_back(s.substr(a, b - a)); a = b + 1; }
}
static std::string strip(const std::string& s) {
    size_t a = 0, b = s.size();
    while (a < b && isspace((unsigned char)s[a])) a++;
    while (b > a && isspace((unsigned char)s[b - 1])) b--;
    return s.substr(a, b - a);
}

static bool parse_error_model(const std::string& name_or_path, ErrorModelHost& m, std::string& err) {
    m = ErrorModelHost();
    if (name_or_path == "random") {
        m.type = 0; m.k = 1; m.max_alts = 1;
        m.cdf.assign(4, 0); m.alts.assign(4, 0); m.nalts.assign(4, 0);
        return true;
    }
    std::string text;
    if (!read_text_file(resolve_model(name_or_path, "error"), text, err)) return false;
    struct Row { std::string kmer; std::vector<uint64_t> alts; std::vector<uint32_t> thr; };
    std::vector<Row> rows;
    size_t a = 0; int k = -1; size_t A = 0;
    std::vector<std::string> parts, kv, slots;
    while (a < text.size()) {
        size_t b = text.find('\n', a);
        if (b == std::string::npos) b = text.size();
        std::string line = strip(text.substr(a, b - a));
        a = b + 1;
        if (line.empty()) continue;
        split(line, ';', parts);
        Row row; std::vector<double> probs;
        for (auto& part : parts) {
            if (part.empty()) continue;
            split(part, ',', kv);
            if (kv.size() < 2) { err = "malformed error model line"; return false; }
            if (row.kmer.empty() && row.alts.empty()) {
                row.kmer = kv[0];
                if (k < 0) k = (int)row.kmer.size();
                if ((int)row.kmer.size() != k) { err = "error model k-mers differ in size"; return false; }
                if (k > 8) { err = "error model k-mer longer than 8 is not supported"; return false; }
            }
            if (!align_kmers(row.kmer, kv[0], slots)) { err = "cannot align alternative " + kv[0] + " to " + row.kmer; return false; }
            uint64_t v = 0; int nbases = 0;
            for (size_t j = 0; j < slots.size(); j++) {
                if (slots[j].size() > 5) { err = "alternative slot longer than 5 bases (the slot codes hold 5 symbols)"; return false; }
                v |= (uint64_t)slots[j].size() << (3 * j);
                for (char ch : slots[j]) {
                    int c = base_code(ch);
                    if (c < 0 || nbases >= 19) { err = "alternative not representable: " + kv[0]; return false; }
                    v |= (uint64_t)c << (24 + 2 * nbases); nbases++;
                }
            }
            if (kv[0] == row.kmer) v |= 1ull << 63;
            row.alts.push_back(v);
            char* endp = nullptr;
            probs.push_back(strtod(kv[1].c_str(), &endp));
        }
        if (row.alts.empty()) continue;
        cdf_thresholds(probs, true, row.thr);
        A = std::max(A, row.alts.size());
        rows.push_back(std::move(row));
    }
    if (k < 3) { err = "error model has no usable k-mers"; return false; }
    if (A > 255) { err = "too many alternatives per k-mer"; return false; }
    const size_t n = (size_t)1 << (2 * k);
    m.type = 1; m.k = k; m.max_alts = (int)A;
    m.cdf.assign(n * A, 0); m.alts.assign(n * A, 0); m.nalts.assign(n, 0);
    for (auto& row : rows) {
        size_t idx = 0;
        for (char ch : row.kmer) { int c = base_code(ch); if (c < 0) { err = "non-ACGT k-mer in error model"; return false; } idx = idx * 4 + (size_t)c; }
        m.nalts[idx] = (uint8_t)row.alts.size();
        for (size_t j = 0; j < A; j++) {
            m.alts[idx * A + j] = j < row.alts.size() ? row.alts[j] : 0;
            m.cdf[idx * A + j] = j < row.thr.size() ? row.thr[j] : row.thr.back();
        }
    }
    return true;
}

static uint64_t qs_hash(uint64_t k) {
    k ^= k >> 33; k *= 0xff51afd7ed558ccdull; k ^= k >> 33; k *= 0xc4ceb9fe1a85ec53ull; k ^= k >> 33;
    return k;
}

static bool encode_key(const std::string& cigar, uint64_t& key) {
    if (cigar.empty() || cigar.size() > 29) return false;
    key = 0;
    for (size_t i = 0; i < cigar.size(); i++) {
        int op = cigar[i] == '=' ? 0 : cigar[i] == 'X' ? 1 : cigar[i] == 'I' ? 2 : cigar[i] == 'D' ? 3 : -1;
        if (op < 0) return false;
        key |= (uint64_t)op << (2 * i);
    }
    key |= (uint64_t)cigar.size() << 58;
    return true;
}

static bool parse_qscore_model(const std::string& name_or_path, QScoreModelHost& m, std::string& err) {
    m = QScoreModelHost();
    struct Row { std::string cigar; std::vector<int> scores; std::vector<double> probs; };
    std::vector<Row> rows;
    m.kmer_size = 1;
    auto uniform = [&](const std::string& c, int lo, int hi) {
        Row r; r.cigar = c;
        int cnt = hi - lo + 1;
        for (int q = lo; q <= hi; q++) { r.scores.push_back(q); r.probs.push_back(1.0 / cnt); }
        rows.push_back(r);
    };
    if (name_or_path == "random") {
        uniform("=", 1, 20); uniform("X", 1, 20); uniform("I", 1, 20);
    } else if (name_or_path == "ideal") {
        m.kmer_size = 9;
        uniform("X", 1, 3); uniform("I", 1, 3); uniform("=", 4, 7); uniform("===", 8, 20); uniform("=====", 21, 30);
        uniform("=======", 31, 40); uniform("=========", 41, 50);
    } else {
        std::string text;
        if (!read_text_file(resolve_model(name_or_path, "qscore"), text, err)) return false;
        size_t a = 0;
        std::vector<std::string> parts, sp, qp;
        while (a < text.size()) {
            size_t b = text.find('\n', a);
            if (b == std::string::npos) b = text.size();
            std::string line = strip(text.substr(a, b - a));
            a = b + 1;
            if (line.empty()) continue;
            split(line, ';', parts);
            if (parts[0] == "overall") continue;
            if (parts.size() < 3) { err = name_or_path + " does not seem to be a valid qscore model file"; return false; }
            Row r; r.cigar = parts[0];
            int kk = 0;
            for (char c : r.cigar) kk += c != 'D';
            m.kmer_size = std::max(m.kmer_size, kk);
            split(parts[2], ',', sp);
            for (auto& x : sp) {
                if (x.empty()) continue;
                split(x, ':', qp);
                if (qp.size() < 2) { err = name_or_path + " does not seem to be a valid qscore model file"; return false; }
                r.scores.push_back(atoi(qp[0].c_str()));
                r.probs.push_back(strtod(qp[1].c_str(), nullptr));
            }
            bool replaced = false;
            for (auto& e : rows) if (e.cigar == r.cigar) { e = r; replaced = true; break; }
            if (!replaced) rows.push_back(std::move(r));
        }
    }
    bool has_eq = false, has_x = false, has_i = false;
    for (auto& r : rows) { has_eq |= r.cigar == "="; has_x |= r.cigar == "X"; has_i |= r.cigar == "I"; }
    if (!(has_eq && has_x && has_i)) { err = "qscore model lacks one of the 1-mer cigars =, X, I"; return false; }
    size_t n_slots = 1;
    while (n_slots < 2 * rows.size()) n_slots *= 2;
    m.n_slots = (int)n_slots;
    m.keys.assign(n_slots, 0); m.row_off.assign(n_slots, 0); m.row_cnt.assign(n_slots, 0);
    for (auto& r : rows) {
        uint64_t key;
        if (!encode_key(r.cigar, key)) { err = "q-score key not representable (longer than 29 ops): " + r.cigar; return false; }
        size_t s = (size_t)(qs_hash(key) & (n_slots - 1));
        while (m.keys[s] != 0) s = (s + 1) & (n_slots - 1);
        m.keys[s] = key;
        m.row_off[s] = (uint32_t)m.q_pool.size();
        m.row_cnt[s] = (uint32_t)r.scores.size();
        cdf_thresholds(r.probs, false, m.cdf_pool);
        for (int q : r.scores) m.q_pool.push_back((uint8_t)q);
    }
    return true;
}

namespace {
struct JVal {
    enum Kind { Null, Bool, Num, Str, Arr, Obj } kind = Null;
    double num = 0.0; bool b = false; std::string str;
    std::vector<JVal> arr;
    std::vector<std::pair<std::string, JVal>> obj;
    const JVal* get(const char* key) const { for (auto& kv : obj) if (kv.first == key) return &kv.second; return nullptr; }
};
struct JParser {
    const char* p; const char* e; std::string err;
    void ws() { while (p < e && (*p == ' ' || *p == '\n' || *p == '\t' || *p == '\r')) p++; }
    bool fail(const char* m) { if (err.empty()) err = m; return false; }
    bool str(std::string& out) {
        if (p >= e || *p != '"') return fail("expected a string");
        p++; out.clear();
        while (p < e && *p != '"') {
            if (*p == '\\') {
                if (++p >= e) return fail("bad escape");
                switch (*p) { case 'n': out += '\n'; break; case 't': out += '\t'; break; case 'r': out += '\r'; break;
                              case 'b': out += '\b'; break; case 'f': out += '\f'; break;
                              case 'u': if (e - p < 5) return fail("bad escape"); out += (char)strtol(std::string(p + 1, 4).c_str(), nullptr, 16); p += 4; break;
                              default: out += *p; }
                p++;
            } else out += *p++;
        }
        if (p >= e) return fail("unterminated string");
        p++;
        return true;
    }
    bool value(JVal& v, int depth) {
        if (depth > 32) return fail("nesting too deep");
        ws();
        if (p >= e) return fail("unexpected end");
        if (*p == '{') {
            v.kind = JVal::Obj; p++; ws();
            if (p < e && *p == '}') { p++; return true; }
            for (;;) {
                ws(); std::string k; if (!str(k)) return false;
                ws(); if (p >= e || *p != ':') return fail("expected ':'");
                p++;
                v.obj.emplace_back(k, JVal());
                if (!value(v.obj.back().second, depth + 1)) return false;
                ws(); if (p < e && *p == ',') { p++; continue; }
                if (p < e && *p == '}') { p++; return true; }
                return fail("expected ',' or '}'");
            }
        }
        if (*p == '[') {
            v.kind = JVal::Arr; p++; ws();
            if (p < e && *p == ']') { p++; return true; }
            for (;;) {
                v.arr.emplace_back();
                if (!value(v.arr.back(), depth + 1)) return false;
                ws(); if (p < e && *p == ',') { p++; continue; }
                if (p < e && *p == ']') { p++; return true; }
                return fail("expected ',' or ']'");
            }
        }
        if (*p == '"') { v.kind = JVal::Str; return str(v.str); }
        if (e - p >= 4 && !strncmp(p, "true", 4)) { v.kind = JVal::Bool; v.b = true; p += 4; return true; }
        if (e - p >= 5 && !strncmp(p, "false", 5)) { v.kind = JVal::Bool; p += 5; return true; }
        if (e - p >= 4 && !strncmp(p, "null", 4)) { p += 4; return true; }
        if (e - p >= 3 && !strncmp(p, "NaN", 3)) { v.kind = JVal::Num; v.num = NAN; p += 3; return true; }
        char* end = nullptr;
        v.num = strtod(p, &end);
        if (end == p) return fail("unexpected character");
        v.kind = JVal::Num; p = end;
        return true;
    }
};
bool num_list(const JVal* v, std::vector<double>& out) {
    if (!v || v->kind != JVal::Arr) return false;
    for (auto& x : v->arr) { if (x.kind != JVal::Num) return false; out.push_back(x.num); }
    return true;
}
}

bool make_tail_model(const double* lx, size_t n_lx, const double* ly, size_t n_ly, const double* grid, const double* trans16,
                     double ratio, const uint8_t* bases4, TailModelHost& m, std::string& err) {
    if (!n_lx || !n_ly) { err = "tail model: empty lx or ly"; return false; }
    if (n_lx > (1u << 24) || n_ly > (1u << 24)) { err = "tail model: grid too large"; return false; }
    m = TailModelHost();
    m.lx.assign(lx, lx + n_lx); m.ly.assign(ly, ly + n_ly);
    for (size_t i = 0; i < n_lx; i++) if (!std::isfinite(lx[i])) { err = "tail model: lx is not finite"; return false; }
    for (size_t i = 0; i < n_ly; i++)
        if (!std::isfinite(ly[i]) || (i && ly[i] < ly[i - 1])) { err = "tail model: ly must be finite and sorted (np.searchsorted)"; return false; }
    if (!(ly[n_ly - 1] != 0.0)) { err = "tail model: last ly label is zero"; return false; }
    m.cdf.resize(n_lx * n_ly);
    for (size_t r = 0; r < n_ly; r++) {
        const double* pdf = grid + r * n_lx;
        double sum = 0.0;
        for (size_t i = 0; i < n_lx; i++) {
            if (!(pdf[i] >= 0.0) || !std::isfinite(pdf[i])) { err = "tail model: grid entries must be finite and >= 0"; return false; }
            sum += pdf[i];
        }
        if (!(sum > 0.0)) { err = "tail model: a grid row sums to zero"; return false; }
        double c = 0.0;
        for (size_t i = 0; i < n_lx; i++) { c = pdf[i] / sum + c; m.cdf[r * n_lx + i] = c; }
    }
    for (int s = 0; s < 4; s++) {
        double c = 0.0;
        for (int j = 0; j < 4; j++) {
            const double w = trans16[4 * s + j];
            if (!(w >= 0.0) || !std::isfinite(w)) { err = "tail model: transition weights must be finite and >= 0"; return false; }
            c += w; m.cum[4 * s + j] = c;
        }
        if (!(c > 0.0)) { err = "tail model: Total of weights must be greater than zero"; return false; }
    }
    if (!std::isfinite(ratio)) { err = "tail model: ratio is not finite"; return false; }
    m.ratio = ratio;
    memcpy(m.bases, bases4, 4);
    m.enabled = true;
    return true;
}

bool load_tail_model(const std::string& name_or_path, TailModelHost& m, std::string& err) {
    if (name_or_path == "no_noise") { m = TailModelHost(); return true; }
    std::string text;
    if (!read_text_file(resolve_model(name_or_path, "tail"), text, err)) return false;
    JParser jp{text.c_str(), text.c_str() + text.size(), {}};
    JVal root;
    if (!jp.value(root, 0) || root.kind != JVal::Obj) { err = "tail model: not a JSON object" + (jp.err.empty() ? std::string() : " (" + jp.err + ")"); return false; }
    std::vector<double> lx, ly, grid, trans;
    if (!num_list(root.get("lx"), lx) || !num_list(root.get("ly"), ly)) { err = "tail model: lx / ly missing or not numeric lists"; return false; }
    const JVal* g = root.get("grid");
    if (!g || g->kind != JVal::Arr || g->arr.size() != ly.size()) { err = "tail model: grid must hold one row per ly label"; return false; }
    for (auto& row : g->arr) {
        const size_t before = grid.size();
        if (!num_list(&row, grid) || grid.size() - before != lx.size()) { err = "tail model: grid rows must hold one number per lx entry"; return false; }
    }
    const JVal* t = root.get("trans");
    if (!t || t->kind != JVal::Arr || t->arr.size() != 4) { err = "tail model: trans must be 4 x 4"; return false; }
    for (auto& row : t->arr) {
        const size_t before = trans.size();
        if (!num_list(&row, trans) || trans.size() - before != 4) { err = "tail model: trans must be 4 x 4"; return false; }
    }
    const JVal* r = root.get("ratio");
    if (!r || r->kind != JVal::Num) { err = "tail model: ratio missing"; return false; }
    const JVal* bs = root.get("bases");
    uint8_t bases[4];
    if (!bs || bs->kind != JVal::Arr || bs->arr.size() != 4) { err = "tail model: bases must list 4 symbols"; return false; }
    for (int i = 0; i < 4; i++) {
        if (bs->arr[i].kind != JVal::Str || bs->arr[i].str.size() != 1) { err = "tail model: bases must be single characters"; return false; }
        bases[i] = (uint8_t)bs->arr[i].str[0];
    }
    if (!root.get("begin")) { err = "tail model: begin missing"; return false; }
    return make_tail_model(lx.data(), lx.size(), ly.data(), ly.size(), grid.data(), trans.data(), r->num, bases, m, err);
}

bool load_trc_model(const std::string& path, TrcModelHost& m, std::string& err) {
// ... 168 lines not shown
```

### tksm_amd/csrc/run.cpp

```cpp
#include "../../include/tksmseq.h"

#include <hip/hip_runtime.h>

#include <algorithm>
#include <cstdio>
#include <cstring>
#include <cstdlib>
#include <string>

#include "ctx.h"

#define TRY(call) do { const int rc_ = (call); if (rc_ != TKSMSEQ_OK) return rc_; } while (0)

static tk::BatchView batch_view(const tksmseq_batch* b) {
    return tk::BatchView{b->reads.as<uint32_t>(), b->intervals.as<uint32_t>(), b->mods.as<uint32_t>(), b->literals.as<uint64_t>(),
                         b->litpool.as<uint8_t>(), b->ids.as<uint32_t>(), b->idpool.as<uint8_t>(), b->n_reads, (uint32_t)b->n_literals};
}
static tk::RefView ref_view(const tksmseq_ctx* ctx) {
    return tk::RefView{ctx->d_packed.as<uint32_t>(), ctx->d_blocktab.as<uint32_t>(), ctx->d_pool.as<uint8_t>(),
                       ctx->d_contigs.as<uint64_t>(), (uint32_t)ctx->contig_names.size()};
}

static int apply_tail(tksmseq_ctx* ctx, tksmseq_batch* b, const tksmseq_run_params* p) {
    const bool want = p->mode == TKSMSEQ_MODE_BADREAD && ctx->tail.enabled && b->n_reads > 0;
    const uint64_t key[4] = {p->seed, p->first_read_index, p->read_index_stride ? p->read_index_stride : 1, ctx->tail_version};
    if (want == b->tail_on && (!want || !memcmp(key, b->tail_key, sizeof(key)))) return TKSMSEQ_OK;
    if (b->splice_len.empty()) b->splice_len = b->raw_len;
    const uint64_t n = b->n_reads;
    if (want) {
        HIPCHK(ctx, b->d_tail.ensure(n * 4 + 16));
        tk::TailView T{(int)ctx->tail.lx.size(), (int)ctx->tail.ly.size(), ctx->tail.ratio, ctx->d_tail_lx.as<double>(),
                       ctx->d_tail_ly.as<double>(), ctx->d_tail_cdf.as<double>()};
        HIPCHK(ctx, tk::launch_tail_lengths(batch_view(b), ref_view(ctx), T, key[0], key[1], key[2], b->d_tail.as<uint32_t>(), ctx->stream));
        std::vector<uint32_t> tl(n);
        HIPCHK(ctx, hipMemcpyAsync(tl.data(), b->d_tail.p, n * 4, hipMemcpyDeviceToHost, ctx->stream));
        HIPCHK(ctx, hipStreamSynchronize(ctx->stream));
        for (uint64_t r = 0; r < n; r++) {
            const uint64_t t = (uint64_t)b->splice_len[r] + tl[r];
            if (t > 0x7fffff00ull) { ctx->err = "molecule plus tail noise longer than 2^31 bases"; return TKSMSEQ_ELIMIT; }
            b->raw_len[r] = (uint32_t)t;
        }
    } else b->raw_len = b->splice_len;
    b->max_raw = 0;
    for (uint32_t v : b->raw_len) b->max_raw = std::max(b->max_raw, v);
    order_by_length(b->raw_len, b->order);
    HIPCHK(ctx, hipMemcpyAsync(b->d_order.p, b->order.data(), n * 4, hipMemcpyHostToDevice, ctx->stream));
    HIPCHK(ctx, hipStreamSynchronize(ctx->stream));
    b->cache_k = -1;
    b->tail_on = want;
    memcpy(b->tail_key, key, sizeof(key));
    return TKSMSEQ_OK;
}

struct RunPlan {
    tksmseq_ctx* ctx; tksmseq_batch* b; const tksmseq_run_params* p;
    int cap_num, cap_den, cap_add;
    int vlevel;
    std::chrono::steady_clock::time_point t_entry = std::chrono::steady_clock::now();
    uint64_t n = 0;
    bool badread = false, direct = false, fast = false;
    int k = 0, lcap = 0, ncap = 0, s_lcap = 0, s_ncap = 0, wpw = 0, lds = 0, n_wgs = 0, trace_words = 0;
    tk::BatchView B{}; tk::RefView R{}; tk::ErrModelView EM{}; tk::QsModelView QM{}; tk::IdentView IM{}; tk::SimParams P{}; tk::SimBuffers O{};

    uint64_t capf(uint64_t raw) const { return ((raw + 2 * (uint64_t)k) * cap_num / cap_den + cap_add + 15) & ~15ull; }
    void mark(const char* what) const {
        if (vlevel >= 2) fprintf(stderr, "[tksmseq] run: %s at %.3f s\n", what, std::chrono::duration<double>(std::chrono::steady_clock::now() - t_entry).count());
    }

    int geometry() {
        n = b->n_reads;
        badread = p->mode == TKSMSEQ_MODE_BADREAD;
        k = badread ? ctx->em.k : 0;
        if (b->cache_k != k || b->cache_num != cap_num || b->cache_den != cap_den || b->cache_add != cap_add) {
            uint64_t t = 0;
            for (uint32_t rl : b->raw_len) t += 2 * capf(rl);
            b->cache_scratch = t; b->cache_k = k; b->cache_num = cap_num; b->cache_den = cap_den; b->cache_add = cap_add;
        }
        lcap = (int)((b->max_raw + 2 * k + 7) & ~7u);
        ncap = badread ? (int)capf(b->max_raw) : 4;
        direct = !badread && !ctx->force_slow && !p->collect_stats;
        fast = badread && !ctx->force_slow && n > 0;
        s_lcap = lcap; s_ncap = ncap;
        if (badread && !ctx->force_slow && tk::simulate_lds_bytes(s_lcap, s_ncap, 1) > 160 * 1024) {
            while (s_lcap > 64 && tk::simulate_lds_bytes(s_lcap, (int)capf((uint64_t)(s_lcap - 2 * k)), 1) > 160 * 1024) s_lcap -= 64;
            s_ncap = (int)capf((uint64_t)(s_lcap - 2 * k));
        }
        wpw = tk::WAVES_PER_WG;
        while (wpw > 1 && tk::simulate_lds_bytes(s_lcap, s_ncap, wpw) > 160 * 1024) wpw >>= 1;
        lds = tk::simulate_lds_bytes(s_lcap, s_ncap, wpw);
        if (!direct && (lds > 160 * 1024 || (badread && !ctx->force_slow ? lcap > 100000 : (ncap >= 65000 || lcap >= 65000)))) {
            ctx->err = "molecule of " + std::to_string(b->max_raw) + " bases exceeds the limit of this build (Badread mode: 100 000 bases)";
            return TKSMSEQ_ELIMIT;
        }
        const int wgs_per_cu = std::min(std::min(32 / wpw, 16), std::max(1, (160 * 1024) / std::max(lds, 1)));
        n_wgs = (int)std::max<uint64_t>(1, std::min<uint64_t>((n + wpw - 1) / wpw, (uint64_t)ctx->n_cus * wgs_per_cu));
        trace_words = (s_ncap + 2) * 4;
        return TKSMSEQ_OK;
    }
    int buffers() {
        hipStream_t s = ctx->stream;
        HIPCHK(ctx, ctx->w_rawlen.ensure(n * 4 + 16));
        HIPCHK(ctx, ctx->w_slotcap.ensure(n * 8 + 16));
        HIPCHK(ctx, ctx->w_slotoff.ensure((n + 1) * 8 + 16));
        HIPCHK(ctx, ctx->w_outlen.ensure(n * 4 + 16));
        HIPCHK(ctx, ctx->w_ident.ensure(n * 8 + 16));
        HIPCHK(ctx, ctx->w_reclen.ensure(n * 8 + 16));
        HIPCHK(ctx, ctx->w_recoff.ensure((n + 1) * 8 + 16));
        HIPCHK(ctx, ctx->w_status.ensure(n * 4 + 16));
        HIPCHK(ctx, ctx->w_scan.ensure(tk::scan_temp_bytes(n) + 64));
        HIPCHK(ctx, ctx->w_trace.ensure(((size_t)n_wgs * wpw + (size_t)tksmseq_ctx::N_SIDE * tksmseq_ctx::SIDE_WAVES) * trace_words * 4 + 64));
        HIPCHK(ctx, ctx->w_counter.ensure(8192));
        HIPCHK(ctx, ctx->w_sums.ensure(64));
        HIPCHK(ctx, ctx->w_scratch.ensure(b->cache_scratch + 64));
        if (p->collect_stats) {
            HIPCHK(ctx, ctx->w_istats.ensure(n * 64 + 16));
            HIPCHK(ctx, ctx->w_dstats.ensure(n * 16 + 16));
            HIPCHK(ctx, hipMemsetAsync(ctx->w_istats.p, 0, n * 64, s));
            HIPCHK(ctx, hipMemsetAsync(ctx->w_dstats.p, 0, n * 16, s));
        }
        B = batch_view(b);
        R = ref_view(ctx);
        EM = tk::ErrModelView{ctx->em.type, k, ctx->em.max_alts, ctx->em_alt0 ? 1 : 0, ctx->em_uniform ? 1 : 0, ctx->d_cdf.as<uint32_t>(), ctx->d_alts.as<uint64_t>(), ctx->d_nalts.as<uint8_t>(), ctx->d_pself.as<uint2>(), ctx->d_cdf32.as<uint32_t>(), ctx->d_pseg.as<uint4>(), ctx->d_pt0.as<uint32_t>(), ctx->d_pt0b.as<uint4>(), ctx->d_altenc.as<uint4>()};
        QM = tk::QsModelView{ctx->qm.n_slots, ctx->qm.kmer_size, ctx->d_qkeys.as<uint64_t>(), ctx->d_qoff.as<uint32_t>(),
                             ctx->d_qcnt.as<uint32_t>(), ctx->d_qcdf.as<uint32_t>(), ctx->d_qq.as<uint8_t>(), ctx->d_qent.as<uint4>(),
                             ctx->d_qpairs.as<uint2>(), ctx->d_qguide.as<uint8_t>(), ctx->qm.guide_direct ? 1 : 0};
        IM = tk::IdentView{ctx->idm.constant ? 1 : 0, ctx->idm.value, ctx->d_qtab.as<double>()};
        P.seed = p->seed; P.first_read = p->first_read_index; P.stride = p->read_index_stride ? p->read_index_stride : 1;
        P.mode = badread ? 1 : 0; P.fastq = p->fastq ? 1 : 0;
        P.quirk_perfect = (badread && p->perfect_of_badread) ? 1 : 0;
        P.compute_q = (badread && p->compute_qual && p->fastq && !P.quirk_perfect) ? 1 : 0;
#ifdef TKSM_ABLATE
        P.ablate = getenv("TKSMSEQ_ABLATE") ? atoi(getenv("TKSMSEQ_ABLATE")) : 0;
#endif
        P.lcap = lcap; P.ncap = ncap; P.s_lcap = s_lcap; P.s_ncap = s_ncap; P.trace_words = trace_words; P.cap_num = cap_num; P.cap_den = cap_den; P.cap_add = cap_add;
        O.raw_len = ctx->w_rawlen.as<uint32_t>(); O.slot_off = ctx->w_slotoff.as<uint64_t>(); O.scratch = ctx->w_scratch.as<uint8_t>();
        O.out_len = ctx->w_outlen.as<uint32_t>(); O.identity = ctx->w_ident.as<double>(); O.rec_len = ctx->w_reclen.as<uint64_t>();
        O.status = ctx->w_status.as<uint32_t>(); O.trace = ctx->w_trace.as<uint32_t>();
        O.work_counter = ctx->w_counter.as<unsigned long long>();
        O.tail_len = (badread && b->tail_on) ? b->d_tail.as<uint32_t>() : nullptr;
        O.tail_chain = ctx->d_tail_chain.as<tk::TailChain>();
        if (badread) {
            HIPCHK(ctx, ctx->w_fullpool.ensure(ctx->full_pool_bytes));
            O.full_pool = ctx->w_fullpool.as<uint8_t>(); O.full_pool_bytes = ctx->full_pool_bytes;
            O.full_pool_used = ctx->w_counter.as<unsigned long long>() + 1023;
        }
        O.istats = p->collect_stats ? ctx->w_istats.as<int32_t>() : nullptr;
        O.dstats = p->collect_stats ? ctx->w_dstats.as<double>() : nullptr;
        O.read_list = nullptr; O.n_work = n;
        return TKSMSEQ_OK;
    }
};

struct FastRun {
    enum Kind { GAP = -1, OTHER = 0, LOOP = 1, ALN = 2, JOB = 3 };
    struct Bucket { uint32_t begin, count; int lcap, ncap, wpw; bool hbm; };
    static constexpr uint32_t EARLY_CAP = 4096;

    RunPlan& pl;
    tksmseq_ctx* const ctx; tksmseq_batch* const b; const hipStream_t s; const uint64_t n;
    tk::FastBuffers FB{};
    std::vector<uint32_t> r_ncap, r_tg;
    uint64_t jcap = 0, tot_trace = 0, tot_popd = 0, nblk = 0;
    size_t nrb = 0, round_bytes = 0, geo_off = 0, geo_bytes = 0;
    uint32_t *hprefix = nullptr, *hbase_prev = nullptr, *hbase_cur = nullptr;
    tk::RangeGeo* hrg = nullptr;
    uint32_t* cnt = nullptr;
    const uint32_t* hcnt = nullptr;
    std::vector<Bucket> buckets;
    uint32_t n_side = 0, side_launches = 0;
    uint32_t full_rows_fit = 0;
    bool late_flushed = false, early_on = false, early_active = false, revive = false, revived = false;
    uint32_t n_early = 0, n_rounds = 0, n_deferred = 0;
    uint64_t jobs_all = 0, jobs_14 = 0;
    std::vector<int> kinds;

    explicit FastRun(RunPlan& plan) : pl(plan), ctx(plan.ctx), b(plan.b), s(plan.ctx->stream), n(plan.n) {
        for (HelperStream& h : ctx->side) h.used = false;
        ctx->early.used = false;
    }
    ~FastRun() {
        for (HelperStream& h : ctx->side) if (h.used) (void)h.synchronize();
        (void)ctx->early.synchronize();
    }

    int tick(Kind kind) {
        if (!ctx->timing) return TKSMSEQ_OK;
        hipEvent_t e;
        const size_t evi = kinds.size();
        if (evi >= ctx->evpool.size()) { if (hipEventCreate(&e) != hipSuccess) { ctx->err = "event"; return TKSMSEQ_EDEVICE; } ctx->evpool.push_back(e); }
        if (hipEventRecord(ctx->evpool[evi], s) != hipSuccess) { ctx->err = "event"; return TKSMSEQ_EDEVICE; }
        kinds.push_back(kind);
        return TKSMSEQ_OK;
    }
    void size_ranges() {
        FB.rs = (uint32_t)((((n + 255) / 256) + 63) & ~63ull);
        FB.n_ranges = (uint32_t)((n + FB.rs - 1) / FB.rs);
        jcap = (uint64_t)FB.n_ranges * FB.rs;
        r_ncap.resize(FB.n_ranges); r_tg.resize(FB.n_ranges);
        for (uint32_t c = 0; c < FB.n_ranges; c++) {
            r_ncap[c] = (uint32_t)pl.capf(b->raw_len[b->order[last_pos(c)]]);
            r_tg[c] = ((r_ncap[c] + 31) & ~31u) / 16 + 1;
            tot_trace += (uint64_t)FB.rs * r_tg[c]; tot_popd += (uint64_t)FB.rs * r_ncap[c];
        }
        ctx->h_row64.resize(n + 1);
        for (uint64_t r = 0; r < n; r++) { ctx->h_row64[r] = (uint32_t)nblk; nblk += ((uint64_t)b->raw_len[r] + 2 * pl.k + 63) / 64 + 1; }
        ctx->h_row64[n] = (uint32_t)nblk;
        nrb = (size_t)FB.n_ranges * 128;
        round_bytes = 2 * nrb + 1024;
        geo_off = (((size_t)(FB.n_ranges + 1) * 12 + 63) & ~(size_t)63);
        geo_bytes = geo_off + (size_t)FB.n_ranges * 2 * sizeof(tk::RangeGeo);
        FB.full_cl = ((((uint32_t)pl.ncap + 31) & ~31u) / 4 + 16 + 3) & ~3u;
        FB.full_tg = FB.full_cl + (FB.full_cl / 4 + 3) / 4 + 1;
        FB.full_rows = (uint32_t)std::max<uint64_t>(64, std::min<uint64_t>(jcap, (4ull << 30) / ((uint64_t)FB.full_tg * 64)) & ~63ull);
        full_rows_fit = FB.full_rows;
        if (ctx->full_rows_cap) FB.full_rows = std::min(FB.full_rows, std::max(64u, ctx->full_rows_cap & ~63u));
        early_on = ctx->early_tail > 0 && ctx->tail_cut == 0 && ctx->tail_wave > 0 && tk::tail_lds_bytes(pl.lcap) <= 65536 && n >= 16ull * ctx->early_tail;
    }
    int grow_buffers() {
        if (nblk >= (1ull << 32)) { ctx->err = "batch too large (split it)"; return TKSMSEQ_ELIMIT; }
        HIPCHK(ctx, ctx->f_state.ensure(n * sizeof(tk::ReadState) + 64));
        HIPCHK(ctx, ctx->f_row64.ensure((n + 1) * 4 + 64));
        HIPCHK(ctx, ctx->f_frag.ensure(nblk * 64 + 256));
        HIPCHK(ctx, ctx->f_nb.ensure(nblk * 128 + 256));
        HIPCHK(ctx, ctx->f_fplanes.ensure((nblk + 8 * n) * 16 + 256));
        HIPCHK(ctx, ctx->f_frag2.ensure((4 * nblk + 4 * n) * 4 + 1024));
        for (DevBuf& m : ctx->f_jmeta) HIPCHK(ctx, m.ensure(jcap * 16 + 64));
        HIPCHK(ctx, ctx->f_jpopd.ensure(tot_popd + 64));
        HIPCHK(ctx, ctx->f_round.ensure(round_bytes + 64));
        HIPCHK(ctx, ctx->f_geoall.ensure(geo_bytes + 64));
        HIPCHK(ctx, ctx->f_trace.ensure(tot_trace * 64 + 64));
        HIPCHK(ctx, ctx->f_redo.ensure(jcap * 4 + 64));
        HIPCHK(ctx, ctx->f_tracefull.ensure((size_t)FB.full_rows * FB.full_tg * 64 + 64));
        HIPCHK(ctx, ctx->f_slow.ensure(n * 4 + 64));
        HIPCHK(ctx, ctx->f_defer.ensure(n * 8 + 64));
        HIPCHK(ctx, ctx->f_defercnt.ensure((size_t)FB.n_ranges * 128 + 64));
        HIPCHK(ctx, ctx->h_round.ensure(round_bytes));
        HIPCHK(ctx, ctx->h_geo.ensure(geo_bytes));
        HIPCHK(ctx, hipMemcpyAsync(ctx->f_row64.p, ctx->h_row64.data(), (n + 1) * 4, hipMemcpyHostToDevice, s));
        FB.state = ctx->f_state.as<tk::ReadState>(); FB.st_frag = ctx->f_frag.as<uint8_t>(); FB.st_nb = ctx->f_nb.as<uint16_t>();
        FB.st_fplanes = ctx->f_fplanes.as<unsigned long long>(); FB.st_frag2 = ctx->f_frag2.as<uint32_t>(); FB.row64 = ctx->f_row64.as<uint32_t>();
        FB.trace = ctx->f_trace.p;
        FB.redo_list = ctx->f_redo.as<uint32_t>();
        FB.trace_full = ctx->f_tracefull.p; FB.counters = reinterpret_cast<uint32_t*>(ctx->f_round.as<uint8_t>() + nrb);
        FB.slow_list = ctx->f_slow.as<uint32_t>();
        FB.early_hist = nullptr; FB.early_list = nullptr; FB.early_slow = nullptr;
        if (early_on) {
            HIPCHK(ctx, ctx->f_early.ensure(65536 + (size_t)EARLY_CAP * 12 + 64));
            FB.early_hist = ctx->f_early.as<uint32_t>();
            FB.early_list = reinterpret_cast<uint2*>(ctx->f_early.as<uint8_t>() + 65536);
            FB.early_slow = reinterpret_cast<uint32_t*>(ctx->f_early.as<uint8_t>() + 65536 + (size_t)EARLY_CAP * 8);
            HIPCHK(ctx, hipMemsetAsync(ctx->f_early.p, 0, 65536, s));
        }
        FB.defer_list = ctx->f_defer.as<uint2>(); FB.defer_cnt = ctx->f_defercnt.as<uint32_t>(); FB.defer_len = ctx->defer_len;
        HIPCHK(ctx, hipMemsetAsync(ctx->f_defercnt.p, 0, (size_t)FB.n_ranges * 128, s));
        FB.prefix = ctx->f_geoall.as<uint32_t>(); FB.base_prev = FB.prefix + (FB.n_ranges + 1); FB.base_cur = FB.prefix + 2 * (FB.n_ranges + 1);
        FB.geo_cur = reinterpret_cast<tk::RangeGeo*>(ctx->f_geoall.as<uint8_t>() + geo_off); FB.geo_prev = FB.geo_cur + FB.n_ranges;
        return TKSMSEQ_OK;
    }
    void select_set(uint32_t round) {
        const int z = round & 1, y = z ^ 1;
        FB.job_meta = ctx->f_jmeta[z].as<uint32_t>(); FB.prev_meta = ctx->f_jmeta[y].as<uint32_t>();
        FB.prev_popd = FB.job_popd = ctx->f_jpopd.as<uint8_t>();
        FB.job_cnt = reinterpret_cast<uint32_t*>(ctx->f_round.as<uint8_t>() + (z ? nrb + 1024 : 0));
        hcnt = ctx->h_round.as<uint32_t>() + (z ? (nrb + 1024) / 4 : 0);
    }
    hipError_t place_ranges() {
        uint64_t ot = 0, op = 0;
        for (uint32_t c = 0; c < FB.n_ranges; c++) {
            hrg[FB.n_ranges + c] = hrg[c];
            const uint64_t slots = hbase_cur[c + 1] - hbase_cur[c];
            tk::RangeGeo g{};
            g.trace_off = ot; g.popd_off = op;
            g.tstride = r_tg[c]; g.ncap = r_ncap[c];
            hrg[c] = g;
            ot += slots * g.tstride; op += slots * g.ncap;
        }
        return hipMemcpyAsync(ctx->f_geoall.p, ctx->h_geo.p, geo_bytes, hipMemcpyHostToDevice, s);
    }
    hipError_t pack_ranges(const uint32_t* counts, bool clear_prefix) {
        uint32_t acc = 0;
        for (uint32_t c = 0; c < FB.n_ranges; c++) {
            hbase_prev[c] = hbase_cur[c]; hbase_cur[c] = acc; acc += (counts[(size_t)c * 32] + 63) & ~63u;
            if (clear_prefix) hprefix[c] = 0;
        }
        hbase_prev[FB.n_ranges] = hbase_cur[FB.n_ranges]; hbase_cur[FB.n_ranges] = acc;
        if (clear_prefix) hprefix[FB.n_ranges] = 0;
        return place_ranges();
    }
    void make_buckets() {
        const uint32_t minr = b->raw_len[b->order.front()], maxr = b->raw_len[b->order.back()];
        const uint32_t step = std::max<uint32_t>(128, ((maxr - minr) / ctx->n_buckets + 63) & ~63u);
        uint64_t i0 = 0;
        while (i0 < n) {
            const uint32_t lim = (b->raw_len[b->order[i0]] / step + 1) * step;
            uint64_t i1 = i0;
            while (i1 < n && b->raw_len[b->order[i1]] < lim) i1++;
            const uint32_t mx = b->raw_len[b->order[i1 - 1]];
            Bucket bk;
            bk.begin = (uint32_t)i0; bk.count = (uint32_t)(i1 - i0);
            bk.lcap = (int)((mx + 2 * pl.k + 7) & ~7u); bk.ncap = (int)pl.capf(mx);
            bk.hbm = bk.lcap > ctx->hbm_state_len;
            bk.wpw = tk::WAVES_PER_WG;
            while (bk.wpw > 1 && tk::err_lds_bytes(bk.lcap, bk.ncap, bk.wpw, bk.hbm) > 64 * 1024) bk.wpw >>= 1;
            buckets.push_back(bk);
            i0 = i1;
        }
    }
    int prepare() {
        size_ranges();
        TRY(grow_buffers());
        select_set(0);
        HIPCHK(ctx, hipStreamSynchronize(s));
        memset(ctx->h_geo.p, 0, geo_bytes);
        const size_t nr1 = FB.n_ranges + 1;
        hprefix = ctx->h_geo.as<uint32_t>(); hbase_prev = hprefix + nr1; hbase_cur = hprefix + 2 * nr1;
        hrg = reinterpret_cast<tk::RangeGeo*>(ctx->h_geo.as<uint8_t>() + geo_off);
        for (uint32_t c = 0; c <= FB.n_ranges; c++) hbase_cur[c] = hbase_prev[c] = c * FB.rs;
        HIPCHK(ctx, place_ranges());
        cnt = ctx->h_round.as<uint32_t>() + nrb / 4;
        make_buckets();
        HIPCHK(ctx, hipMemsetAsync(ctx->f_nb.p, 0, nblk * 128, s));
        HIPCHK(ctx, hipMemsetAsync(ctx->f_round.p, 0, round_bytes, s));
        TRY(tick(GAP));
        pl.mark("buffers ready");
        return TKSMSEQ_OK;
    }
    int launch_side(uint32_t upto) {
        if (upto <= n_side || side_launches + 2 >= 1024) return TKSMSEQ_OK;
        const int k2 = (int)(side_launches % tksmseq_ctx::N_SIDE);
        HelperStream& h = ctx->side[k2];
        tk::SimBuffers O2 = pl.O;
        O2.read_list = ctx->f_slow.as<uint32_t>() + n_side; O2.n_work = upto - n_side;
        O2.work_counter = ctx->w_counter.as<unsigned long long>() + 1 + side_launches;
        O2.trace = pl.O.trace + ((size_t)pl.n_wgs * pl.wpw + (size_t)k2 * tksmseq_ctx::SIDE_WAVES) * pl.trace_words;
        HIPCHK(ctx, h.fork_from(s));
        const uint64_t want = (O2.n_work + pl.wpw - 1) / pl.wpw;
        const int wgs = (int)std::max<uint64_t>(1, std::min<uint64_t>(want, (uint64_t)(tksmseq_ctx::SIDE_WAVES / pl.wpw)));
        HIPCHK(ctx, tk::launch_simulate(pl.B, pl.R, pl.EM, pl.QM, pl.IM, pl.P, O2, wgs, pl.wpw, h.stream));
        HIPCHK(ctx, h.launched());
        n_side = upto; side_launches++;
        return TKSMSEQ_OK;
    }
    int launch_early(const std::vector<uint32_t>& copies) {
        uint32_t hist[256] = {};
        for (size_t i = 0; i < copies.size(); i++) hist[i & 255] += copies[i];
        uint64_t total = 0; for (uint32_t v : hist) total += v;
        uint64_t acc = 0; int median_bin = 0;
        for (int bb = 0; bb < 256; bb++) { acc += hist[bb]; if (2 * acc >= total) { median_bin = bb; break; } }
        int min_bin = 256; uint64_t top = 0;
        while (min_bin > median_bin + 16 && top + hist[min_bin - 1] <= ctx->early_tail) { min_bin--; top += hist[min_bin]; }
        if (!top) return TKSMSEQ_OK;
        n_early = (uint32_t)top;
        HIPCHK(ctx, tk::launch_mark_early(FB, b->d_order.as<uint32_t>(), n, pl.k, (uint32_t)min_bin, s));
        HIPCHK(ctx, ctx->early.fork_from(s));
        HIPCHK(ctx, tk::launch_tail_early(pl.EM, pl.P, FB, n_early, pl.lcap, ctx->tail_wcap, ctx->early.stream));
        HIPCHK(ctx, ctx->early.launched());
        early_active = true;
        return TKSMSEQ_OK;
    }
    int init() {
        const int lcap = pl.lcap;
        HIPCHK(ctx, tk::launch_init(pl.B, pl.R, pl.EM, pl.IM, pl.P, pl.O, FB, lcap * tk::WAVES_PER_WG <= 150 * 1024 ? tk::WAVES_PER_WG : (lcap * 2 <= 150 * 1024 ? 2 : 1), s));
        TRY(tick(OTHER));
        HIPCHK(ctx, hipMemcpyAsync(cnt, FB.counters, 64, hipMemcpyDeviceToHost, s));
        std::vector<uint32_t> early_copies(early_on ? 64 * 256 : 0);
        if (early_on) HIPCHK(ctx, hipMemcpyAsync(early_copies.data(), FB.early_hist, early_copies.size() * 4, hipMemcpyDeviceToHost, s));
        HIPCHK(ctx, hipStreamSynchronize(s));
        pl.mark("fragments spliced (k_init)");
        TRY(launch_side(cnt[tk::CNT_SLOW]));
        if (early_on) TRY(launch_early(early_copies));
        return TKSMSEQ_OK;
    }
    int launch_revive() {
        if (pl.P.compute_q) HIPCHK(ctx, tk::launch_qjobs(FB, pl.k, n_deferred, s));
        else {
            const Bucket& bk = buckets.back();
            HIPCHK(ctx, tk::launch_err(pl.B, pl.EM, pl.QM, pl.P, pl.O, FB, b->d_order.as<uint32_t>(), 0, n_deferred, bk.lcap, bk.ncap, 2, 0, FB.n_ranges, bk.wpw, bk.hbm, s));
        }
        revive = false;
        return TKSMSEQ_OK;
    }
    uint32_t last_pos(uint32_t c) const { return (uint32_t)std::min<uint64_t>((uint64_t)(c + 1) * FB.rs, n) - 1; }
    int launch_last_visits() {
        size_t bi = 0;
        for (uint32_t c = 0, c1; c < FB.n_ranges; c = c1) {
            while (bi + 1 < buckets.size() && last_pos(c) >= buckets[bi].begin + buckets[bi].count) bi++;
            const Bucket& bk = buckets[bi];
            for (c1 = c + 1; c1 < FB.n_ranges && last_pos(c1) < bk.begin + bk.count; c1++) {}
            const uint32_t cntw = hprefix[c1] - hprefix[c];
            if (cntw) HIPCHK(ctx, tk::launch_err(pl.B, pl.EM, pl.QM, pl.P, pl.O, FB, b->d_order.as<uint32_t>(), 0, cntw, bk.lcap, bk.ncap, 1, c, c1, bk.wpw, bk.hbm, s));
        }
        return TKSMSEQ_OK;
    }
    int launch_loops() {
        const uint32_t* order = b->d_order.as<uint32_t>();
        const uint32_t left = hprefix[FB.n_ranges];
        const int lcap = pl.lcap;
        const uint64_t tail_slots = (uint64_t)ctx->n_cus * std::min<uint64_t>(16, (160u * 1024u) / tk::tail_lds_bytes(lcap));
        if (n_rounds == 0) HIPCHK(ctx, tk::launch_loop(pl.EM, pl.P, FB, order, 0, (uint32_t)n, lcap, 0, 0, 0, s));
        else if (left <= std::min<uint64_t>(ctx->tail_wave, tail_slots) && tk::tail_lds_bytes(lcap) <= 65536)
            HIPCHK(ctx, tk::launch_tail(pl.EM, pl.P, FB, order, 0, left, lcap, 1, 0, FB.n_ranges, ctx->tail_wcap, s));
        else if (left <= ctx->wave_loop && lcap <= 32768)
            HIPCHK(ctx, tk::launch_loopw(pl.EM, pl.P, FB, order, 0, left, lcap, 1, 0, FB.n_ranges, s));
        else HIPCHK(ctx, tk::launch_loop(pl.EM, pl.P, FB, order, 0, left, lcap, 1, 0, FB.n_ranges, s));
        return tick(LOOP);
    }
    int exchange() {
        HIPCHK(ctx, hipMemcpyAsync(ctx->h_round.p, ctx->f_round.p, round_bytes, hipMemcpyDeviceToHost, s));
        HIPCHK(ctx, hipStreamSynchronize(s));
        uint32_t jobs = 0;
        for (uint32_t c = 0; c < FB.n_ranges; c++) { hprefix[c] = jobs; jobs += hcnt[(size_t)c * 32]; }
        hprefix[FB.n_ranges] = cnt[tk::CNT_JOBS] = jobs;
        return TKSMSEQ_OK;
    }
    int flush_side() {
        const bool late = cnt[tk::CNT_JOBS] * 16ull < n;
        const uint32_t pending = cnt[tk::CNT_SLOW] - n_side;
        const bool stream_idle = ctx->side[side_launches % tksmseq_ctx::N_SIDE].idle();
        if ((pending >= 128 && (stream_idle || pending >= 2048)) || (pending && late && !late_flushed)) TRY(launch_side(cnt[tk::CNT_SLOW]));
        late_flushed = late_flushed || late;
        return TKSMSEQ_OK;
    }
    int join_early() {
        if (!early_active) return TKSMSEQ_OK;
        HIPCHK(ctx, ctx->early.wait_done());
        HIPCHK(ctx, tk::launch_merge_early_slow(FB, s));
        HIPCHK(ctx, hipMemcpyAsync(cnt, FB.counters, 64, hipMemcpyDeviceToHost, s));
        HIPCHK(ctx, hipStreamSynchronize(s));
        cnt[tk::CNT_JOBS] = 0;
        early_active = false;
        return TKSMSEQ_OK;
    }
    int align(bool qround) {
        const uint32_t jobs = cnt[tk::CNT_JOBS];
        const uint32_t n_jobs = hbase_cur[FB.n_ranges - 1] + ((hcnt[(size_t)(FB.n_ranges - 1) * 32] + 63) & ~63u);
        const bool full_only = jobs <= std::min(ctx->small_aln, full_rows_fit);
        jobs_all += jobs; if (!full_only) jobs_14 += jobs;
        HIPCHK(ctx, tk::launch_alnf(pl.P, FB, pl.O, n_jobs, full_only, qround ? 1 : 0, s));
        return tick(ALN);
    }
    int rounds() {
        for (;; n_rounds++) {
            select_set(n_rounds);
            HIPCHK(ctx, tk::launch_round_reset(FB, s));
            TRY(tick(GAP));
            const bool qround = revive && pl.P.compute_q;
            const bool regular = !revive && !revived;
            TRY(revive ? launch_revive() : revived ? launch_last_visits() : launch_loops());
            TRY(tick(regular ? JOB : OTHER));
            TRY(exchange());
            TRY(flush_side());
            if (cnt[tk::CNT_JOBS] == 0) {
                TRY(join_early());
                if (cnt[tk::CNT_DEFERRED] == 0 || revived) break;
                revived = revive = true; n_deferred = cnt[tk::CNT_DEFERRED];
                std::vector<uint32_t> hd((size_t)FB.n_ranges * 32);
                HIPCHK(ctx, hipMemcpy(hd.data(), ctx->f_defercnt.p, hd.size() * 4, hipMemcpyDeviceToHost));
                HIPCHK(ctx, pack_ranges(hd.data(), true));
                continue;
            }
#ifdef TKSM_ABLATE
            if (pl.P.ablate >= 1 && pl.P.ablate <= 9) break;
#endif
            if (cnt[tk::CNT_JOBS] < ctx->tail_cut && cnt[tk::CNT_JOBS] * 64ull < n) {
                HIPCHK(ctx, tk::launch_collect_unfinished(FB, n, s));
                HIPCHK(ctx, hipMemcpyAsync(cnt, FB.counters, 64, hipMemcpyDeviceToHost, s));
                HIPCHK(ctx, hipStreamSynchronize(s));
                break;
            }
            if (n_rounds > 100000) { ctx->err = "internal: error loop did not terminate"; return TKSMSEQ_EDEVICE; }
            TRY(tick(GAP));
            TRY(align(qround));
            HIPCHK(ctx, pack_ranges(hcnt, false));
        }
        pl.mark("rounds done");
        return TKSMSEQ_OK;
    }
    int finish(float ms[3]) {
        uint32_t* d = ctx->last_diag;
        memset(d, 0, sizeof(ctx->last_diag));
        d[DIAG_ROUNDS] = n_rounds; d[DIAG_EXACT_KERNEL_READS] = cnt[tk::CNT_SLOW]; d[DIAG_PREDICTED_STRAGGLERS] = n_early;
        d[DIAG_JOBS_14_ROW_ROUNDS] = (uint32_t)std::min<uint64_t>(jobs_14, 0xffffffffu); d[DIAG_JOBS_REDONE_FULL_WIDTH] = cnt[tk::CNT_REDO_JOBS];
        d[DIAG_FALLBACKS] = cnt[tk::CNT_FAIL]; d[DIAG_FALLBACK_REASONS] = cnt[tk::CNT_FAIL_OR]; d[DIAG_FALLBACKS_QSCORE_JOBS] = cnt[tk::CNT_FAIL_QJOB];
        d[DIAG_FALLBACKS_LIST_PASS] = cnt[tk::CNT_FAIL_LIST]; d[DIAG_JOBS_ALL_ROUNDS] = (uint32_t)std::min<uint64_t>(jobs_all, 0xffffffffu);
        d[DIAG_BAND_EXITS] = cnt[tk::CNT_EXIT + tk::EXIT_BAND_LOOP] + cnt[tk::CNT_EXIT + tk::EXIT_BAND_ERR];
        if (pl.vlevel) {
            uint32_t cc[tk::CNT_WORDS];
            HIPCHK(ctx, hipMemcpy(cc, FB.counters, sizeof(cc), hipMemcpyDeviceToHost));
            const uint32_t *ex = cc + tk::CNT_EXIT, *why = cc + tk::CNT_FAIL_REASON;
            fprintf(stderr, "[tksmseq] this thread so far: %u device allocations, %.3f s in hipMalloc\n", alloc_calls(), alloc_seconds());
            fprintf(stderr, "[tksmseq] reads %llu rounds %u slow-path reads %u (band exit %u/%u, shift %u/%u), full-width redo: %u jobs in %u waves; predicted stragglers on their own stream: %u\n",
                    (unsigned long long)n, n_rounds, cnt[tk::CNT_SLOW], ex[tk::EXIT_BAND_LOOP], ex[tk::EXIT_BAND_ERR], ex[tk::EXIT_SHIFT_LOOP], ex[tk::EXIT_SHIFT_ERR], cc[tk::CNT_REDO_JOBS], cc[tk::CNT_REDO_WAVES], n_early);
            fprintf(stderr, "[tksmseq] fused alignment failures: %u, reasons or-ed 0x%x, last 0x%x (n %u, m %u)\n", cc[tk::CNT_FAIL], cc[tk::CNT_FAIL_OR], cc[tk::CNT_FAIL_LAST], cc[tk::CNT_FAIL_NM] & 0xffffu, cc[tk::CNT_FAIL_NM] >> 16);
            fprintf(stderr, "[tksmseq]   per reason: queue / reservoir overflow %u no pool rows %u - shift>31 %u shift>14 %u end cell %u walk %u | q-score jobs %u, list pass %u\n", why[tk::FAIL_QUEUE], why[tk::FAIL_NOROW], why[tk::FAIL_SHIFT31], why[tk::FAIL_SHIFT14], why[tk::FAIL_END_CELL], why[tk::FAIL_WALK], cc[tk::CNT_FAIL_QJOB], cc[tk::CNT_FAIL_LIST]);
        }
        for (HelperStream& h : ctx->side) if (h.used) HIPCHK(ctx, h.join_into(s));
        if (cnt[tk::CNT_SLOW] > n_side) {
            pl.O.read_list = ctx->f_slow.as<uint32_t>() + n_side; pl.O.n_work = cnt[tk::CNT_SLOW] - n_side;
            const uint64_t want = (pl.O.n_work + pl.wpw - 1) / pl.wpw;
            TRY(tick(GAP));
            HIPCHK(ctx, tk::launch_simulate(pl.B, pl.R, pl.EM, pl.QM, pl.IM, pl.P, pl.O, (int)std::max<uint64_t>(1, std::min<uint64_t>(want, (uint64_t)pl.n_wgs)), pl.wpw, s));
            TRY(tick(OTHER));
        }
        if (ctx->timing) {
            HIPCHK(ctx, hipStreamSynchronize(s));
            for (size_t i = 1; i < kinds.size(); i++) {
                float t = 0; (void)hipEventElapsedTime(&t, ctx->evpool[i - 1], ctx->evpool[i]);
                if (kinds[i] >= LOOP) ms[kinds[i] - LOOP] += t;
            }
        }
        return TKSMSEQ_OK;
    }
};

static int rerun_in_hbm(const RunPlan& pl, const std::vector<uint32_t>& st) {
    tksmseq_ctx* ctx = pl.ctx;
    hipStream_t s = ctx->stream;
    std::vector<uint32_t> big;
    for (uint64_t i = 0; i < pl.n; i++) if (st[i] & 8) big.push_back((uint32_t)i);
    const int n_waves = (int)std::min<size_t>(big.size(), 64);
    const size_t per_wave = tk::simulate_big_bytes(pl.lcap, pl.ncap);
    HIPCHK(ctx, ctx->w_biglist.ensure(big.size() * 4 + 16));
    HIPCHK(ctx, ctx->w_bigscratch.ensure(per_wave * n_waves + 64));
    HIPCHK(ctx, ctx->w_bigtrace.ensure((size_t)n_waves * 2 * (pl.ncap + 2) * 8 + 64));
    HIPCHK(ctx, hipMemcpyAsync(ctx->w_biglist.p, big.data(), big.size() * 4, hipMemcpyHostToDevice, s));
    HIPCHK(ctx, hipMemsetAsync(ctx->w_counter.p, 0, 8, s));
    tk::SimBuffers O3 = pl.O;
    O3.read_list = ctx->w_biglist.as<uint32_t>(); O3.n_work = big.size();
    O3.work_counter = ctx->w_counter.as<unsigned long long>();
    O3.big_scratch = ctx->w_bigscratch.as<uint8_t>(); O3.big_per_wave = per_wave; O3.big_trace = ctx->w_bigtrace.as<unsigned long long>();
    HIPCHK(ctx, tk::launch_simulate_big(pl.B, pl.R, pl.EM, pl.QM, pl.IM, pl.P, O3, n_waves, s));
    if (pl.vlevel) fprintf(stderr, "[tksmseq] %zu molecules beyond the LDS-resident limit took the exact kernel with HBM working sets\n", big.size());
    return TKSMSEQ_OK;
}

static int check_status(const RunPlan& pl, int pass, bool* again, bool* overflow) {
    tksmseq_ctx* ctx = pl.ctx;
    const uint64_t n = pl.n;
    std::vector<uint32_t> st(n);
    HIPCHK(ctx, hipMemcpy(st.data(), ctx->w_status.p, n * 4, hipMemcpyDeviceToHost));
    uint32_t any = 0; uint64_t first = 0;
    for (uint64_t i = 0; i < n; i++) if (st[i]) { if (!any) first = i; any |= st[i]; }
    if ((any & 16) && pl.vlevel) {
        std::string l;
        int shown = 0;
        for (uint64_t i = 0; i < n && shown < 16; i++) if (st[i] & 16) { l += " " + std::to_string(i); shown++; }
        fprintf(stderr, "[tksmseq] reads with an unbanded alignment (first %d):%s\n", shown, l.c_str());
    }
    if (any & 2) { ctx->err = "modification position outside its interval at read " + std::to_string(first); return TKSMSEQ_EINVAL; }
    if (any & 4) { ctx->err = "out of memory for the unbanded alignment fallback at read " + std::to_string(first) + " (TKSMSEQ_FULL_POOL_MB)"; return TKSMSEQ_ENOMEM; }
    if ((any & 8) && pass == 0 && pl.badread) { *again = true; return rerun_in_hbm(pl, st); }
    if (any & 8) {
        uint64_t f8 = 0;
        for (uint64_t i = 0; i < n; i++) if (st[i] & 8) { f8 = i; break; }
        ctx->err = "read " + std::to_string(f8) + " (" + std::to_string(pl.b->raw_len[f8]) + " bases) exceeds the limits of the exact wave-wide kernel";
        return TKSMSEQ_ELIMIT;
    }
    if (any & 1) *overflow = true;
    return TKSMSEQ_OK;
}

static int close_run(const RunPlan& pl, const float ms[3], tksmseq_result* res, bool* overflow) {
    tksmseq_ctx* ctx = pl.ctx;
    hipStream_t s = ctx->stream;
    const uint64_t n = pl.n;
    const bool T = ctx->timing;
    unsigned long long* sums = ctx->w_sums.as<unsigned long long>();
    unsigned long long hs[2] = {0, 0}; uint64_t total = 0;
    for (int pass = 0;; pass++) {
        HIPCHK(ctx, tk::launch_scan(ctx->w_reclen.as<uint64_t>(), ctx->w_recoff.as<uint64_t>(), n, ctx->w_scan.p, ctx->w_scan.cap, s));
        HIPCHK(ctx, tk::launch_sum_u32(ctx->w_status.as<uint32_t>(), n, sums, s));
        HIPCHK(ctx, tk::launch_sum_u32(ctx->w_outlen.as<uint32_t>(), n, sums + 1, s));
        if (T && pass == 0) HIPCHK(ctx, hipEventRecord(ctx->ev[3], s));
        HIPCHK(ctx, hipMemcpyAsync(hs, sums, 16, hipMemcpyDeviceToHost, s));
        HIPCHK(ctx, hipMemcpyAsync(&total, ctx->w_recoff.as<uint64_t>() + n, 8, hipMemcpyDeviceToHost, s));
        HIPCHK(ctx, hipStreamSynchronize(s));
        if (!hs[0]) break;
        bool again = false;
        TRY(check_status(pl, pass, &again, overflow));
        if (*overflow) return TKSMSEQ_OK;
        if (!again) break;
    }
    uint8_t* records;
    if (ctx->user_out) {
        if (total > ctx->user_out_cap) { ctx->err = "caller-provided output buffer too small: need " + std::to_string(total) + " bytes"; return TKSMSEQ_ENOMEM; }
        records = (uint8_t*)ctx->user_out;
    } else {
        HIPCHK(ctx, ctx->w_records.ensure(total + 64));
        records = ctx->w_records.as<uint8_t>();
    }
    if (pl.direct) HIPCHK(ctx, tk::launch_perfect(pl.B, pl.R, pl.P, pl.O, ctx->w_recoff.as<uint64_t>(), records, pl.b->max_raw, ctx->n_cus, s));
    else HIPCHK(ctx, tk::launch_emit(pl.B, pl.P, pl.O, ctx->w_recoff.as<uint64_t>(), records, s));
    if (T) {
        HIPCHK(ctx, hipEventRecord(ctx->ev[4], s));
        HIPCHK(ctx, hipEventSynchronize(ctx->ev[4]));
        for (int i = 0; i < 4; i++) (void)hipEventElapsedTime(&res->kernel_ms[i], ctx->ev[i], ctx->ev[i + 1]);
        (void)hipEventElapsedTime(&res->kernel_ms[4], ctx->ev[0], ctx->ev[4]);
        for (int i = 0; i < 3; i++) res->kernel_ms[5 + i] = ms[i];
    }
    res->records = records; res->record_offsets = ctx->w_recoff.p; res->records_bytes = total; res->n_reads = n;
    res->bases_in = pl.b->total_raw; res->bases_out = hs[1];
    return TKSMSEQ_OK;
}

static int run_once(tksmseq_ctx* ctx, tksmseq_batch* b, const tksmseq_run_params* p, int cap_num, int cap_den, int cap_add, int vlevel,
                    tksmseq_result* res, bool* overflow) {
    *overflow = false;
    RunPlan pl{ctx, b, p, cap_num, cap_den, cap_add, vlevel};
    TRY(pl.geometry());
    TRY(pl.buffers());
    hipStream_t s = ctx->stream;
    const bool T = ctx->timing;
    float ms[3] = {0, 0, 0};
    if (T) HIPCHK(ctx, hipEventRecord(ctx->ev[0], s));
    HIPCHK(ctx, hipMemsetAsync(ctx->w_counter.p, 0, 8192, s));
    HIPCHK(ctx, tk::launch_read_lengths(pl.B, pl.R, pl.k, cap_num, cap_den, cap_add, pl.O.tail_len, ctx->w_rawlen.as<uint32_t>(), ctx->w_slotcap.as<uint64_t>(),
                                        ctx->w_status.as<uint32_t>(), s));
    HIPCHK(ctx, tk::launch_scan(ctx->w_slotcap.as<uint64_t>(), ctx->w_slotoff.as<uint64_t>(), pl.n, ctx->w_scan.p, ctx->w_scan.cap, s));
    if (T) HIPCHK(ctx, hipEventRecord(ctx->ev[1], s));
    if (pl.direct) HIPCHK(ctx, tk::launch_perfect_lengths(pl.B, pl.R, pl.P, pl.O, s));
    else if (!pl.fast) HIPCHK(ctx, tk::launch_simulate(pl.B, pl.R, pl.EM, pl.QM, pl.IM, pl.P, pl.O, pl.n_wgs, pl.wpw, s));
    else {
        FastRun fr(pl);
        TRY(fr.prepare());
        TRY(fr.init());
        TRY(fr.rounds());
        TRY(fr.finish(ms));
    }
    if (T) HIPCHK(ctx, hipEventRecord(ctx->ev[2], s));
    return close_run(pl, ms, res, overflow);
}

extern "C" {

int tksmseq_run(tksmseq_ctx* ctx, const tksmseq_batch* batch, const tksmseq_run_params* p, tksmseq_result* result) {
    if (!ctx || !batch || !p || !result) return TKSMSEQ_EINVAL;
    HIPCHK(ctx, hipSetDevice(ctx->device));
    memset(result, 0, sizeof(*result));
    if (p->mode != TKSMSEQ_MODE_PERFECT && p->mode != TKSMSEQ_MODE_BADREAD) { ctx->err = "unknown mode"; return TKSMSEQ_EINVAL; }
    if (p->mode == TKSMSEQ_MODE_BADREAD) {
        if (ctx->em.type < 0) { ctx->err = "no error model loaded"; return TKSMSEQ_ESTATE; }
        if (!ctx->idm.set) { ctx->err = "identity distribution not set"; return TKSMSEQ_ESTATE; }
        if (p->compute_qual && p->fastq && ctx->qm.n_slots == 0) { ctx->err = "no q-score model loaded"; return TKSMSEQ_ESTATE; }
    }
    if (ctx->n_declared) { ctx->err = "the reference holds contigs declared without bases (tksmseq_reference_declare_contig): there is nothing to sequence from"; return TKSMSEQ_ESTATE; }
    tksmseq_batch* b = const_cast<tksmseq_batch*>(batch);
    bool overflow = false;
// ... 22 lines not shown
```

Measured before the change: 15.50 million reads/s.

## Cache hottest q-score keys and guide rows in LDS for k_err probes

Builds a small hot table on the host holding the 32 most frequent q-score k-mers (by model count), with their slots, row offsets and 64-byte guide rows. k_err copies that table into LDS and checks it before falling back to the global hash-table probe and global guide lookup. To make room, the per-wave fragment is no longer staged in LDS up front; it is read straight from global memory and copied into the aux area only before join_out. The hot table is dropped when it would reduce workgroups per CU by LDS, at the cost of an extra block-wide copy and barrier per workgroup.

```diff
diff --git a/tksm_amd/csrc/api.cpp b/tksm_amd/csrc/api.cpp
--- a/tksm_amd/csrc/api.cpp
+++ b/tksm_amd/csrc/api.cpp
@@ -11,6 +11,7 @@
 
 #include "ctx.h"
 #include "loop_filter.h"
+#include "qs_hot.h"
 
 static thread_local std::string g_create_error;
 void set_contextless_error(const std::string& e) { g_create_error = e; }
@@ -76,7 +77,7 @@
     c->d_pself.borrow(src->d_pself); c->d_pseg.borrow(src->d_pseg); c->d_pt0.borrow(src->d_pt0); c->d_pt0b.borrow(src->d_pt0b); c->d_cdf32.borrow(src->d_cdf32); c->d_cdf.borrow(src->d_cdf); c->d_alts.borrow(src->d_alts); c->d_altenc.borrow(src->d_altenc);
     c->d_nalts.borrow(src->d_nalts); c->d_qkeys.borrow(src->d_qkeys); c->d_qoff.borrow(src->d_qoff); c->d_qcnt.borrow(src->d_qcnt);
     c->d_qcdf.borrow(src->d_qcdf); c->d_qq.borrow(src->d_qq); c->d_qtab.borrow(src->d_qtab); c->d_qent.borrow(src->d_qent);
-    c->d_qpairs.borrow(src->d_qpairs); c->d_qguide.borrow(src->d_qguide);
+    c->d_qpairs.borrow(src->d_qpairs); c->d_qguide.borrow(src->d_qguide); c->d_qhot.borrow(src->d_qhot);
     c->tail = src->tail; c->tail_version = src->tail_version; c->host_threads = src->host_threads;
     c->d_tail_lx.borrow(src->d_tail_lx); c->d_tail_ly.borrow(src->d_tail_ly); c->d_tail_cdf.borrow(src->d_tail_cdf); c->d_tail_chain.borrow(src->d_tail_chain);
     return TKSMSEQ_OK;
@@ -317,35 +318,17 @@
     if ((rc = upload(ctx, ctx->d_qcnt, ctx->qm.row_cnt))) return rc;
     if ((rc = upload(ctx, ctx->d_qcdf, ctx->qm.cdf_pool))) return rc;
     if ((rc = upload(ctx, ctx->d_qq, ctx->qm.q_pool))) return rc;
-    {
-        const QScoreModelHost& m2 = ctx->qm;
-        const size_t ns = (size_t)m2.n_slots;
-        std::vector<uint32_t> ent(ns * 4, 0), pairs(m2.q_pool.size() * 2, 0);
-        std::vector<uint8_t> guide(ns * 64, 0);
-        bool direct = true;
-        for (size_t s2 = 0; s2 < ns; s2++) if (m2.keys[s2] && m2.row_cnt[s2] > 128) direct = false;
-        for (uint8_t qv : m2.q_pool) if (qv > 127) direct = false;
-        for (size_t i = 0; i < m2.q_pool.size(); i++) { pairs[2 * i] = m2.cdf_pool[i]; pairs[2 * i + 1] = m2.q_pool[i]; }
-        for (size_t s2 = 0; s2 < ns; s2++) {
-            ent[4 * s2] = (uint32_t)m2.keys[s2]; ent[4 * s2 + 1] = (uint32_t)(m2.keys[s2] >> 32);
-            ent[4 * s2 + 2] = m2.row_off[s2]; ent[4 * s2 + 3] = m2.row_cnt[s2];
-            if (!m2.keys[s2]) continue;
-            const uint32_t off = m2.row_off[s2], cnt = m2.row_cnt[s2];
-            if (cnt > 255) { ctx->err = "q-score rows with more than 255 entries are not supported"; return TKSMSEQ_ELIMIT; }
-            uint32_t a = 0;
-            for (uint32_t bkt = 0; bkt < 64; bkt++) {
-                const uint32_t wmin = bkt << 26, wmax = wmin | 0x3ffffffu;
-                while (a + 1 < cnt && m2.cdf_pool[off + a] <= wmin) a++;
-                uint32_t ah = a;
-                while (ah + 1 < cnt && m2.cdf_pool[off + ah] <= wmax) ah++;
-                guide[s2 * 64 + bkt] = (direct && ah == a) ? (uint8_t)(0x80u | m2.q_pool[off + a]) : (uint8_t)a;
-            }
-        }
-        ctx->qm.guide_direct = direct;
-        if ((rc = upload(ctx, ctx->d_qent, ent))) return rc;
-        if ((rc = upload(ctx, ctx->d_qpairs, pairs))) return rc;
-        return upload(ctx, ctx->d_qguide, guide);
-    }
+    std::vector<uint32_t> ent, pairs;
+    std::vector<uint8_t> guide;
+    if (!build_qscore_tables(ctx->qm, ent, pairs, guide, ctx->err)) return TKSMSEQ_ELIMIT;
+    std::vector<tkqh::QsHotEntry> hot(tkqh::QS_HOT_U4);
+    std::vector<uint32_t> seen(ctx->qm.row_slot.size());
+    (void)tkqh::qs_hot_build(ctx->qm.keys.data(), ctx->qm.occ.data(), ctx->qm.row_off.data(), ctx->qm.row_cnt.data(), ctx->qm.row_slot.data(),
+                             ctx->qm.row_slot.size(), ctx->qm.kmer_size, guide.data(), seen.data(), hot.data());
+    if ((rc = upload(ctx, ctx->d_qent, ent))) return rc;
+    if ((rc = upload(ctx, ctx->d_qpairs, pairs))) return rc;
+    if ((rc = upload(ctx, ctx->d_qhot, hot))) return rc;
+    return upload(ctx, ctx->d_qguide, guide);
 }
 
 static int install_tail_model(tksmseq_ctx* ctx, TailModelHost&& m) {
diff --git a/tksm_amd/csrc/ctx.h b/tksm_amd/csrc/ctx.h
--- a/tksm_amd/csrc/ctx.h
+++ b/tksm_amd/csrc/ctx.h
@@ -228,7 +228,7 @@
     bool em_uniform = false, em_alt0 = false;
     TailModelHost tail; uint64_t tail_version = 0;
     DevBuf d_tail_lx, d_tail_ly, d_tail_cdf, d_tail_chain;
-    DevBuf d_pself, d_pseg, d_pt0, d_pt0b, d_cdf32, d_cdf, d_alts, d_altenc, d_nalts, d_qkeys, d_qoff, d_qcnt, d_qcdf, d_qq, d_qtab, d_qent, d_qpairs, d_qguide;
+    DevBuf d_pself, d_pseg, d_pt0, d_pt0b, d_cdf32, d_cdf, d_alts, d_altenc, d_nalts, d_qkeys, d_qoff, d_qcnt, d_qcdf, d_qq, d_qtab, d_qent, d_qpairs, d_qguide, d_qhot;
 
     DevBuf w_rawlen, w_slotcap, w_slotoff, w_outlen, w_ident, w_reclen, w_recoff, w_status, w_scan, w_trace, w_counter,
         w_scratch, w_records, w_istats, w_dstats, w_sums, w_fullpool, w_biglist, w_bigscratch, w_bigtrace;
diff --git a/tksm_amd/csrc/host.h b/tksm_amd/csrc/host.h
--- a/tksm_amd/csrc/host.h
+++ b/tksm_amd/csrc/host.h
@@ -21,7 +21,11 @@
     std::vector<uint64_t> keys;
     std::vector<uint32_t> row_off, row_cnt, cdf_pool;
     std::vector<uint8_t> q_pool;
+    std::vector<uint64_t> occ;
+    std::vector<uint32_t> row_slot;
 };
+
+bool build_qscore_tables(QScoreModelHost& m, std::vector<uint32_t>& ent, std::vector<uint32_t>& pairs, std::vector<uint8_t>& guide, std::string& err);
 
 struct IdentityHost {
     bool set = false, constant = true;
diff --git a/tksm_amd/csrc/kernels.h b/tksm_amd/csrc/kernels.h
--- a/tksm_amd/csrc/kernels.h
+++ b/tksm_amd/csrc/kernels.h
@@ -54,6 +54,8 @@
     const uint2* pairs;
     const uint8_t* guide;
     int guide_direct;
+    const uint4* hot;
+    int hot_u4;
 };
 
 struct IdentView {
@@ -148,6 +150,8 @@
     CNT_FAIL_LIST = 25,
     CNT_EARLY_SLOW = 26,
     CNT_EARLY = 27,
+    CNT_QS_PROBES = 28,
+    CNT_QS_HOT = 29,
     CNT_WORDS = 32
 };
 enum ExitCause { EXIT_BAND_LOOP = 0, EXIT_SHIFT_LOOP = 1, EXIT_SHIFT_ERR = 2, EXIT_BAND_ERR = 3 };
@@ -199,7 +203,8 @@
                                const IdentView& im, const SimParams& p, const SimBuffers& o, int n_waves, hipStream_t s);
 hipError_t launch_init(const BatchView& b, const RefView& r, const ErrModelView& em, const IdentView& im, const SimParams& p,
                        const SimBuffers& o, const FastBuffers& fb, int waves_per_wg, hipStream_t s);
-int err_lds_bytes(int lcap, int ncap, int waves_per_wg, bool state_in_hbm);
+int err_lds_bytes(int lcap, int ncap, int waves_per_wg, bool state_in_hbm, int hot_u4);
+int err_hot_u4(int lcap, int ncap, int waves_per_wg, bool state_in_hbm, int hot_u4);
 int loop_lds_words(int lcap);
 hipError_t launch_loopw(const ErrModelView& em, const SimParams& p, const FastBuffers& fb, const uint32_t* order, uint32_t begin,
                         uint32_t count, int lcap, int from_jobs, uint32_t c0, uint32_t c1, hipStream_t s);
diff --git a/tksm_amd/csrc/kernels.hip b/tksm_amd/csrc/kernels.hip
--- a/tksm_amd/csrc/kernels.hip
+++ b/tksm_amd/csrc/kernels.hip
@@ -1,5 +1,6 @@
 #include "kernels.h"
 #include "loop_filter.h"
+#include "qs_hot.h"
 #include <type_traits>
 
 namespace tk {
@@ -1654,9 +1655,10 @@
 #endif
     const int lane = threadIdx.x & 63, wave = __builtin_amdgcn_readfirstlane(threadIdx.x >> 6), wpw = blockDim.x >> 6;
     const uint32_t widx = blockIdx.x * (uint32_t)wpw + (uint32_t)wave;
-    if (widx >= count) return;
-    uint64_t r; uint32_t pos;
-    if (!from_jobs) { pos = begin + widx; r = (uint64_t)__builtin_amdgcn_readfirstlane((int)order[pos]) & 0xffffffffull; }
+    const bool live = widx < count;
+    uint64_t r = 0; uint32_t pos = 0;
+    if (!live) {}
+    else if (!from_jobs) { pos = begin + widx; r = (uint64_t)__builtin_amdgcn_readfirstlane((int)order[pos]) & 0xffffffffull; }
     else if (from_jobs == 2) {
         const uint2 e = FB.defer_list[widx];
         r = (uint64_t)__builtin_amdgcn_readfirstlane((int)e.x) & 0xffffffffull;
@@ -1670,14 +1672,22 @@
         pos = lo2 * FB.rs;
     }
     ReadState S = FB.state[r];
+    const int per_wave = STATE_IN_HBM ? lds_ncap + 128 : lds_lcap * 2 + lds_ncap + 128;
+    const int hot_n = QM.hot_u4;
+    uint4* hot_w = reinterpret_cast<uint4*>(lds_raw + (((size_t)wpw * per_wave + 15) & ~(size_t)15));
+    const tkqh::QsHotEntry* hot = reinterpret_cast<const tkqh::QsHotEntry*>(hot_w);
+    if (hot_n) {
+        for (int t = threadIdx.x; t < hot_n; t += blockDim.x) hot_w[t] = QM.hot[t];
+        __syncthreads();
+    }
+    if (!live) return;
     if (S.stage == 2 || S.slow) return;
     if (S.stage == 0) return;
     uint16_t* gnb = nb_row(FB, r);
-    const int per_wave = STATE_IN_HBM ? lds_ncap + 128 : lds_lcap * 3 + lds_ncap + 128;
     uint8_t* lds_wave = lds_raw + (size_t)wave * per_wave;
-    uint8_t* frag = STATE_IN_HBM ? frag_row(FB, r) : lds_wave;
-    uint16_t* nb = STATE_IN_HBM ? gnb : reinterpret_cast<uint16_t*>(lds_wave + lds_lcap);
-    uint8_t* aux = STATE_IN_HBM ? lds_wave : lds_wave + 3 * (size_t)lds_lcap;
+    const uint8_t* frag = frag_row(FB, r);
+    uint16_t* nb = STATE_IN_HBM ? gnb : reinterpret_cast<uint16_t*>(lds_wave);
+    uint8_t* aux = STATE_IN_HBM ? lds_wave : lds_wave + 2 * (size_t)lds_lcap;
     const int k = EM.k;
     const uint64_t g = P.first_read + r * P.stride;
     const int raw_len = __builtin_amdgcn_readfirstlane(S.raw_len);
@@ -1687,8 +1697,6 @@
     uint8_t* out_seq = O.scratch + slot;
     uint8_t* out_qual = out_seq + cap;
     if (!STATE_IN_HBM) {
-        const uint8_t* gfrag0 = frag_row(FB, r);
-        for (int t = lane * 4; t < L; t += 256) *reinterpret_cast<uint32_t*>(frag + t) = *reinterpret_cast<const uint32_t*>(gfrag0 + t);
         for (int t = lane * 2; t < L; t += 128) *reinterpret_cast<uint32_t*>(nb + t) = *reinterpret_cast<const uint32_t*>(gnb + t);
     }
     wave_sync();
@@ -1732,10 +1740,30 @@
             const int d = max(0, max(margins - i2, i2 + margins - (m - 1)));
             int row = -1; uint32_t roff = 0, rcnt = 0;
             auto probe = [&](uint64_t key) {
-                uint32_t sl = (uint32_t)qs_hash(key) & hmask;
+                const uint64_t hh = qs_hash(key);
+                uint32_t sl = (uint32_t)hh & hmask;
 #ifdef TKSM_ABLATE
                 if (P.ablate == 41) { row = (int)(sl & 1023u); roff = 0u; rcnt = 1u; return; }
 #endif
+#ifdef TKSM_ABLATE
+                if (P.ablate != 46)
+#endif
+                if (hot_n) {
+                    const tkqh::QsHotEntry he = tkqh::qs_hot_find(hot, hh);
+#ifdef TKSM_ABLATE
+                    if (P.ablate == 47) {
+                        const unsigned long long act = __ballot(1), hm = __ballot(tkqh::qs_hot_is(he, key));
+                        if (lane == (int)__ffsll((long long)act) - 1) {
+                            atomicAdd(&FB.counters[CNT_QS_PROBES], (uint32_t)__popcll(act)); atomicAdd(&FB.counters[CNT_QS_HOT], (uint32_t)__popcll(hm));
+                        }
+                    }
+#endif
+                    if (tkqh::qs_hot_is(he, key)) {
+                        row = (int)tkqh::qs_hot_slot(he); roff = tkqh::qs_hot_row_off(he);
+                        rcnt = tkqh::qs_hot_row_cnt(he) | ((tkqh::qs_hot_guide_row(he) + 1u) << 8);
+                        return;
+                    }
+                }
                 for (;;) {
                     const uint4 e = QM.ent[sl];
                     const uint64_t kk = ((uint64_t)e.y << 32) | e.x;
@@ -1793,6 +1821,8 @@
                     s0++; e0--;
                 }
             }
+            const uint32_t hrow1 = rcnt >> 8;
+            rcnt &= 0xffu;
             uint8_t q = 0;
 #ifdef TKSM_ABLATE
             if (P.ablate == 42) { out_qual[i2 - lo] = (uint8_t)(33 + (row & 31)); continue; }
@@ -1804,7 +1834,7 @@
 #endif
             if (row >= 0) {
                 const uint32_t w = philox(P.seed, g, ST_QUAL, (uint32_t)i2).x;
-                uint32_t a2 = QM.guide[(size_t)row * 64 + (w >> 26)];
+                uint32_t a2 = hrow1 ? tkqh::qs_hot_guide(hot, hrow1 - 1u, w >> 26) : QM.guide[(size_t)row * 64 + (w >> 26)];
                 if (QM.guide_direct && (a2 & 0x80u)) q = (uint8_t)(a2 & 0x7fu);
                 else {
                     uint2 pr = QM.pairs[roff + a2];
@@ -1816,6 +1846,12 @@
         }
     } else {
         identity = 1.0 - errors / frag_len;
+    }
+    if (!STATE_IN_HBM) {
+        wave_sync();
+        for (int t = lane * 4; t < L; t += 256) *reinterpret_cast<uint32_t*>(aux + t) = *reinterpret_cast<const uint32_t*>(frag + t);
+        wave_sync();
+        frag = aux;
     }
     join_out(frag, nb, L, out_seq, lo, hi, lane);
     if (P.quirk_perfect) identity = 1.0;
@@ -2695,16 +2731,25 @@
     hipLaunchKernelGGL(k_init, dim3((unsigned)((b.n_reads + wpw - 1) / wpw)), dim3(64 * wpw), lds, s, b, r, em, im, p, o, fb);
     return hipGetLastError();
 }
-int err_lds_bytes(int lcap, int ncap, int wpw, bool state_in_hbm) { return wpw * ((state_in_hbm ? 0 : lcap * 3) + ncap + 128); }
+int err_lds_bytes(int lcap, int ncap, int wpw, bool state_in_hbm, int hot_u4) {
+    return ((wpw * ((state_in_hbm ? 0 : lcap * 2) + ncap + 128) + 15) & ~15) + hot_u4 * 16;
+}
+int err_hot_u4(int lcap, int ncap, int wpw, bool state_in_hbm, int hot_u4) {
+    auto resident = [&](int lds) { return std::min(32 / wpw, 160 * 1024 / std::max(lds, 1)); };
+    const int before = resident(wpw * ((state_in_hbm ? 0 : lcap * 3) + ncap + 128));
+    return resident(err_lds_bytes(lcap, ncap, wpw, state_in_hbm, hot_u4)) < before ? 0 : hot_u4;
+}
 hipError_t launch_err(const BatchView& b, const ErrModelView& em, const QsModelView& qm, const SimParams& p, const SimBuffers& o,
                       const FastBuffers& fb, const uint32_t* order, uint32_t begin, uint32_t count, int lds_lcap, int lds_ncap,
                       int from_jobs, uint32_t c0, uint32_t c1, int wpw, bool state_in_hbm, hipStream_t s) {
     if (!count) return hipSuccess;
-    const int lds = err_lds_bytes(lds_lcap, lds_ncap, wpw, state_in_hbm);
+    QsModelView qv = qm;
+    qv.hot_u4 = err_hot_u4(lds_lcap, lds_ncap, wpw, state_in_hbm, qm.hot_u4);
+    const int lds = err_lds_bytes(lds_lcap, lds_ncap, wpw, state_in_hbm, qv.hot_u4);
     auto kern = state_in_hbm ? k_err<true> : k_err<false>;
     hipError_t e = hipFuncSetAttribute(reinterpret_cast<const void*>(kern), hipFuncAttributeMaxDynamicSharedMemorySize, 160 * 1024);
     if (e != hipSuccess) return e;
-    hipLaunchKernelGGL(kern, dim3((count + wpw - 1) / wpw), dim3(64 * wpw), lds, s, b, em, qm, p, o, fb, order, begin, count, lds_lcap,
+    hipLaunchKernelGGL(kern, dim3((count + wpw - 1) / wpw), dim3(64 * wpw), lds, s, b, em, qv, p, o, fb, order, begin, count, lds_lcap,
                        lds_ncap, from_jobs, c0, c1);
     return hipGetLastError();
 }
diff --git a/tksm_amd/csrc/models.cpp b/tksm_amd/csrc/models.cpp
--- a/tksm_amd/csrc/models.cpp
+++ b/tksm_amd/csrc/models.cpp
@@ -222,7 +222,7 @@
 
 static bool parse_qscore_model(const std::string& name_or_path, QScoreModelHost& m, std::string& err) {
     m = QScoreModelHost();
-    struct Row { std::string cigar; std::vector<int> scores; std::vector<double> probs; };
+    struct Row { std::string cigar; std::vector<int> scores; std::vector<double> probs; uint64_t count = 0; };
     std::vector<Row> rows;
     m.kmer_size = 1;
     auto uniform = [&](const std::string& c, int lo, int hi) {
@@ -255,6 +255,12 @@
             int kk = 0;
             for (char c : r.cigar) kk += c != 'D';
             m.kmer_size = std::max(m.kmer_size, kk);
+            {
+                const std::string& c = parts[1];
+                bool digits = !c.empty() && c.size() <= 19;
+                for (char ch : c) digits = digits && ch >= '0' && ch <= '9';
+                r.count = digits ? strtoull(c.c_str(), nullptr, 10) : 0;
+            }
             split(parts[2], ',', sp);
             for (auto& x : sp) {
                 if (x.empty()) continue;
@@ -274,7 +280,7 @@
     size_t n_slots = 1;
     while (n_slots < 2 * rows.size()) n_slots *= 2;
     m.n_slots = (int)n_slots;
-    m.keys.assign(n_slots, 0); m.row_off.assign(n_slots, 0); m.row_cnt.assign(n_slots, 0);
+    m.keys.assign(n_slots, 0); m.row_off.assign(n_slots, 0); m.row_cnt.assign(n_slots, 0); m.occ.assign(n_slots, 0);
     for (auto& r : rows) {
         uint64_t key;
         if (!encode_key(r.cigar, key)) { err = "q-score key not representable (longer than 29 ops): " + r.cigar; return false; }
@@ -283,9 +289,37 @@
         m.keys[s] = key;
         m.row_off[s] = (uint32_t)m.q_pool.size();
         m.row_cnt[s] = (uint32_t)r.scores.size();
+        m.occ[s] = r.count;
+        m.row_slot.push_back((uint32_t)s);
         cdf_thresholds(r.probs, false, m.cdf_pool);
         for (int q : r.scores) m.q_pool.push_back((uint8_t)q);
     }
+    return true;
+}
+
+bool build_qscore_tables(QScoreModelHost& m, std::vector<uint32_t>& ent, std::vector<uint32_t>& pairs, std::vector<uint8_t>& guide, std::string& err) {
+    const size_t ns = (size_t)m.n_slots;
+    ent.assign(ns * 4, 0); pairs.assign(m.q_pool.size() * 2, 0); guide.assign(ns * 64, 0);
+    bool direct = true;
+    for (size_t s2 = 0; s2 < ns; s2++) if (m.keys[s2] && m.row_cnt[s2] > 128) direct = false;
+    for (uint8_t qv : m.q_pool) if (qv > 127) direct = false;
+    for (size_t i = 0; i < m.q_pool.size(); i++) { pairs[2 * i] = m.cdf_pool[i]; pairs[2 * i + 1] = m.q_pool[i]; }
+    for (size_t s2 = 0; s2 < ns; s2++) {
+        ent[4 * s2] = (uint32_t)m.keys[s2]; ent[4 * s2 + 1] = (uint32_t)(m.keys[s2] >> 32);
+        ent[4 * s2 + 2] = m.row_off[s2]; ent[4 * s2 + 3] = m.row_cnt[s2];
+        if (!m.keys[s2]) continue;
+        const uint32_t off = m.row_off[s2], cnt = m.row_cnt[s2];
+        if (cnt > 255) { err = "q-score rows with more than 255 entries are not supported"; return false; }
+        uint32_t a = 0;
+        for (uint32_t bkt = 0; bkt < 64; bkt++) {
+            const uint32_t wmin = bkt << 26, wmax = wmin | 0x3ffffffu;
+            while (a + 1 < cnt && m.cdf_pool[off + a] <= wmin) a++;
+            uint32_t ah = a;
+            while (ah + 1 < cnt && m.cdf_pool[off + ah] <= wmax) ah++;
+            guide[s2 * 64 + bkt] = (direct && ah == a) ? (uint8_t)(0x80u | m.q_pool[off + a]) : (uint8_t)a;
+        }
+    }
+    m.guide_direct = direct;
     return true;
 }
 
diff --git a/tksm_amd/csrc/qs_hot.h b/tksm_amd/csrc/qs_hot.h
--- /dev/null
+++ b/tksm_amd/csrc/qs_hot.h
@@ -0,0 +1,75 @@
+#pragma once
+#include <stddef.h>
+#include <stdint.h>
+
+#if defined(__HIPCC__)
+#define TKQH_HD __host__ __device__ inline
+#else
+#define TKQH_HD inline
+#endif
+
+namespace tkqh {
+
+constexpr uint32_t QS_HOT_KEYS = 32;
+constexpr uint32_t QS_HOT_SLOTS = 128;
+constexpr uint32_t QS_HOT_U4 = QS_HOT_SLOTS + QS_HOT_KEYS * 4u;
+constexpr uint32_t QS_HOT_BYTES = QS_HOT_U4 * 16u;
+
+typedef uint32_t QsHotEntry __attribute__((vector_size(16)));
+TKQH_HD uint64_t qs_hot_key(const QsHotEntry& e) { return ((uint64_t)e[1] << 32) | e[0]; }
+
+TKQH_HD uint64_t qs_hash(uint64_t k) {
+    k ^= k >> 33; k *= 0xff51afd7ed558ccdull; k ^= k >> 33; k *= 0xc4ceb9fe1a85ec53ull; k ^= k >> 33;
+    return k;
+}
+
+TKQH_HD uint32_t qs_hot_index(uint64_t h) { return (uint32_t)(h >> 32) & (QS_HOT_SLOTS - 1u); }
+
+TKQH_HD uint32_t qs_hot_slot(const QsHotEntry& e) { return e[2] & 0x3ffffffu; }
+TKQH_HD uint32_t qs_hot_guide_row(const QsHotEntry& e) { return e[2] >> 26; }
+TKQH_HD uint32_t qs_hot_row_off(const QsHotEntry& e) { return e[3] & 0xffffffu; }
+TKQH_HD uint32_t qs_hot_row_cnt(const QsHotEntry& e) { return e[3] >> 24; }
+TKQH_HD uint8_t qs_hot_guide(const QsHotEntry* block, uint32_t guide_row, uint32_t bkt) {
+    return reinterpret_cast<const uint8_t*>(block + QS_HOT_SLOTS)[guide_row * 64u + bkt];
+}
+
+TKQH_HD QsHotEntry qs_hot_find(const QsHotEntry* block, uint64_t h) { return block[qs_hot_index(h)]; }
+TKQH_HD bool qs_hot_is(const QsHotEntry& e, uint64_t key) { return (qs_hot_key(e) == key) & (key != 0); }
+
+inline int qs_key_ops(uint64_t key) {
+    const int len = (int)(key >> 58);
+    int n = 0;
+    for (int i = 0; i < len; i++) n += ((key >> (2 * i)) & 3u) != 3u;
+    return n;
+}
+
+inline uint32_t qs_hot_build(const uint64_t* keys, const uint64_t* occ, const uint32_t* row_off, const uint32_t* row_cnt, const uint32_t* row_slot,
+                             size_t n_rows, int kmer_size, const uint8_t* guide, uint32_t* seen, QsHotEntry* out) {
+    for (uint32_t i = 0; i < QS_HOT_U4; i++) out[i] = QsHotEntry{0u, 0u, 0u, 0u};
+    for (size_t i = 0; i < n_rows; i++) seen[i] = 0u;
+    uint32_t placed = 0;
+    uint8_t* rows_out = reinterpret_cast<uint8_t*>(out + QS_HOT_SLOTS);
+    for (int wide = 1; wide >= 0 && placed < QS_HOT_KEYS; wide--) {
+        for (;;) {
+            size_t best = n_rows;
+            for (size_t i = 0; i < n_rows; i++) {
+                if (seen[i]) continue;
+                const uint32_t s = row_slot[i];
+                if ((qs_key_ops(keys[s]) == kmer_size) != (wide == 1)) continue;
+                if (best == n_rows || occ[s] > occ[row_slot[best]]) best = i;
+            }
+            if (best == n_rows) break;
+            seen[best] = 1u;
+            const uint32_t s = row_slot[best];
+            QsHotEntry& e = out[qs_hot_index(qs_hash(keys[s]))];
+            if (qs_hot_key(e)) continue;
+            if (s > 0x3ffffffu || row_off[s] > 0xffffffu || row_cnt[s] > 0xffu) continue;
+            e = QsHotEntry{(uint32_t)keys[s], (uint32_t)(keys[s] >> 32), s | (placed << 26), row_off[s] | (row_cnt[s] << 24)};
+            for (uint32_t b = 0; b < 64; b++) rows_out[placed * 64u + b] = guide[(size_t)s * 64 + b];
+            if (++placed == QS_HOT_KEYS) break;
+        }
+    }
+    return placed;
+}
+
+}
diff --git a/tksm_amd/csrc/run.cpp b/tksm_amd/csrc/run.cpp
--- a/tksm_amd/csrc/run.cpp
+++ b/tksm_amd/csrc/run.cpp
@@ -9,6 +9,7 @@
 #include <string>
 
 #include "ctx.h"
+#include "qs_hot.h"
 
 #define TRY(call) do { const int rc_ = (call); if (rc_ != TKSMSEQ_OK) return rc_; } while (0)
 
@@ -123,12 +124,14 @@
         EM = tk::ErrModelView{ctx->em.type, k, ctx->em.max_alts, ctx->em_alt0 ? 1 : 0, ctx->em_uniform ? 1 : 0, ctx->d_cdf.as<uint32_t>(), ctx->d_alts.as<uint64_t>(), ctx->d_nalts.as<uint8_t>(), ctx->d_pself.as<uint2>(), ctx->d_cdf32.as<uint32_t>(), ctx->d_pseg.as<uint4>(), ctx->d_pt0.as<uint32_t>(), ctx->d_pt0b.as<uint4>(), ctx->d_altenc.as<uint4>()};
         QM = tk::QsModelView{ctx->qm.n_slots, ctx->qm.kmer_size, ctx->d_qkeys.as<uint64_t>(), ctx->d_qoff.as<uint32_t>(),
                              ctx->d_qcnt.as<uint32_t>(), ctx->d_qcdf.as<uint32_t>(), ctx->d_qq.as<uint8_t>(), ctx->d_qent.as<uint4>(),
-                             ctx->d_qpairs.as<uint2>(), ctx->d_qguide.as<uint8_t>(), ctx->qm.guide_direct ? 1 : 0};
+                             ctx->d_qpairs.as<uint2>(), ctx->d_qguide.as<uint8_t>(), ctx->qm.guide_direct ? 1 : 0, ctx->d_qhot.as<uint4>(),
+                             0};
         IM = tk::IdentView{ctx->idm.constant ? 1 : 0, ctx->idm.value, ctx->d_qtab.as<double>()};
         P.seed = p->seed; P.first_read = p->first_read_index; P.stride = p->read_index_stride ? p->read_index_stride : 1;
         P.mode = badread ? 1 : 0; P.fastq = p->fastq ? 1 : 0;
         P.quirk_perfect = (badread && p->perfect_of_badread) ? 1 : 0;
         P.compute_q = (badread && p->compute_qual && p->fastq && !P.quirk_perfect) ? 1 : 0;
+        QM.hot_u4 = (P.compute_q && ctx->qm.n_slots) ? (int)tkqh::QS_HOT_U4 : 0;
 #ifdef TKSM_ABLATE
         P.ablate = getenv("TKSMSEQ_ABLATE") ? atoi(getenv("TKSMSEQ_ABLATE")) : 0;
 #endif
@@ -301,7 +304,7 @@
             bk.lcap = (int)((mx + 2 * pl.k + 7) & ~7u); bk.ncap = (int)pl.capf(mx);
             bk.hbm = bk.lcap > ctx->hbm_state_len;
             bk.wpw = tk::WAVES_PER_WG;
-            while (bk.wpw > 1 && tk::err_lds_bytes(bk.lcap, bk.ncap, bk.wpw, bk.hbm) > 64 * 1024) bk.wpw >>= 1;
+            while (bk.wpw > 1 && tk::err_lds_bytes(bk.lcap, bk.ncap, bk.wpw, bk.hbm, 0) > 64 * 1024) bk.wpw >>= 1;
             buckets.push_back(bk);
             i0 = i1;
         }
@@ -493,6 +496,18 @@
                     (unsigned long long)n, n_rounds, cnt[tk::CNT_SLOW], ex[tk::EXIT_BAND_LOOP], ex[tk::EXIT_BAND_ERR], ex[tk::EXIT_SHIFT_LOOP], ex[tk::EXIT_SHIFT_ERR], cc[tk::CNT_REDO_JOBS], cc[tk::CNT_REDO_WAVES], n_early);
             fprintf(stderr, "[tksmseq] fused alignment failures: %u, reasons or-ed 0x%x, last 0x%x (n %u, m %u)\n", cc[tk::CNT_FAIL], cc[tk::CNT_FAIL_OR], cc[tk::CNT_FAIL_LAST], cc[tk::CNT_FAIL_NM] & 0xffffu, cc[tk::CNT_FAIL_NM] >> 16);
             fprintf(stderr, "[tksmseq]   per reason: queue / reservoir overflow %u no pool rows %u - shift>31 %u shift>14 %u end cell %u walk %u | q-score jobs %u, list pass %u\n", why[tk::FAIL_QUEUE], why[tk::FAIL_NOROW], why[tk::FAIL_SHIFT31], why[tk::FAIL_SHIFT14], why[tk::FAIL_END_CELL], why[tk::FAIL_WALK], cc[tk::CNT_FAIL_QJOB], cc[tk::CNT_FAIL_LIST]);
+#ifdef TKSM_ABLATE
+            if (pl.P.ablate == 47) fprintf(stderr, "[tksmseq] k_err q-score probes %u, answered by a hot key in LDS %u (%.4f)\n", cc[tk::CNT_QS_PROBES], cc[tk::CNT_QS_HOT], cc[tk::CNT_QS_HOT] / std::max(1.0, (double)cc[tk::CNT_QS_PROBES]));
+#endif
+            for (const Bucket& bk : buckets) {
+                int wpw0 = tk::WAVES_PER_WG;
+                auto staged = [&](int w) { return w * ((bk.hbm ? 0 : bk.lcap * 3) + bk.ncap + 128); };
+                while (wpw0 > 1 && staged(wpw0) > 64 * 1024) wpw0 >>= 1;
+                const int hot1 = tk::err_hot_u4(bk.lcap, bk.ncap, bk.wpw, bk.hbm, pl.QM.hot_u4), lds1 = tk::err_lds_bytes(bk.lcap, bk.ncap, bk.wpw, bk.hbm, hot1);
+                fprintf(stderr, "[tksmseq]   k_err bucket: %u reads, lcap %d ncap %d %s, hot keys %s: %d waves, %d B LDS, %d workgroups / CU by LDS (fragment staged, no hot keys: %d waves, %d B, %d)\n",
+                        bk.count, bk.lcap, bk.ncap, bk.hbm ? "state in HBM" : "slot codes in LDS", hot1 ? "in LDS" : "not held", bk.wpw, lds1, 160 * 1024 / std::max(lds1, 1), wpw0, staged(wpw0),
+                        160 * 1024 / std::max(staged(wpw0), 1));
+            }
         }
         for (HelperStream& h : ctx->side) if (h.used) HIPCHK(ctx, h.join_into(s));
         if (cnt[tk::CNT_SLOW] > n_side) {
```

Result: no change. 15.58 million reads/s, median of 5 (+0.5%).
